# yjh0410/YOLO-Nano

Measured on NVIDIA B200. Metric: images/sec YOLO-Nano-1.0x 416 bs256 fp32-parity e2e (backbone+neck+head+decode+NMS), higher is better.
Workload: dtype f32 (tcgen05 3xTF32 split, fp32 accumulate)

## Files before the change

yolo_nano_b200/csrc/gemm_tc.cuh:

```cuda
#pragma once
#include <cuda.h>

#include <cstring>

#include "common.cuh"
#include "ptx_sm100.cuh"

namespace ynb {

constexpr int kTcThreads = 512;
constexpr int kTcSplitWarp0 = 8, kTcProducerWarp = 12, kTcMmaWarp = 13;
constexpr int kTcProducers = 3;
constexpr int kTcBM = 128;
constexpr int kTcBK = 32;
constexpr int kTcAStageBytes = kTcBM * 128;
constexpr int kTcMaxStages = 8;
constexpr int kTcSmemBudget = 232448;
constexpr int kTcMaxMain = 4;

struct TcGemmParams {
  int num_steps;
  int chunks_per_tap;
  int is3x3;
  int mode;
  int bf16_in;
  int out_bf16;
  int num_stages;
  int w_resident;
  int64_t M;
  int64_t num_tiles;
  int H, W, TH, TW, tiles_x, tiles_y;
  int N, Npad;
  int nmain;
  int nacc;
  int merge_corr;
  int ksub;
  int presplit;
  int a2_step;
  int stack_b;
  int acc_stages;
  uint32_t tmem_cols;
  uint32_t a_box_bytes;
  float* out;
  int out_ld, out_off, out_step;
  ChanMap omap;
  const float* bias;
  int act;
  const float* pass;
  int pass_ld;
  int tma_store;
  struct Decode {
    float* boxes;
    float* scores;
    int32_t* cls;
    int G, HW;
    float stride, input_size;
    float aw[3], ah[3];
    int64_t Ntot, level_off;
  } dec;
  int* err_flag;
  long long* trace;
  int trace_cap;
};

#define YNB_TRACE(role, a, b)                                                                        \
  do {                                                                                               \
    if (p.trace != nullptr && blockIdx.x == 0) {                                                     \
      const int _lt = (int)(((long long)(a) - (long long)blockIdx.x) / (long long)gridDim.x) & 63;   \
      long long* _e = p.trace + 1 + (long long)((((role) * 64 + _lt) * 32) + ((int)(b) & 31)) * 4;   \
      _e[0] = (role); _e[1] = (a); _e[2] = (b); _e[3] = clock64();                                   \
    }                                                                                                \
  } while (0)

struct TcSmemLayout {
  uint32_t stage_bytes;
  uint32_t w_chunk_bytes;
  uint32_t w_res_off;
  uint32_t bias_off;
  uint32_t stg_off;
  uint32_t bar_off;
  uint32_t total;
};
constexpr int kTcStgBytes = 8 * 4096;

__host__ __device__ inline TcSmemLayout tc_smem_layout(int Npad, int num_steps, int num_stages, bool w_resident,
                                                       bool split) {
  TcSmemLayout L;
  L.w_chunk_bytes = (uint32_t)Npad * 128;
  uint32_t a_bytes = kTcAStageBytes * (split ? 2 : 1);
  uint32_t w_bytes = w_resident ? 0 : L.w_chunk_bytes * (split ? 2 : 1);
  L.stage_bytes = a_bytes + w_bytes;
  L.w_res_off = L.stage_bytes * num_stages;
  uint32_t w_res = w_resident ? L.w_chunk_bytes * (split ? 2 : 1) * num_steps : 0;
  L.bias_off = L.w_res_off + w_res;
  L.stg_off = L.bias_off + 1024;
  L.bar_off = L.stg_off + kTcStgBytes;
  L.total = L.bar_off + 256 + 1024;
  return L;
}

__host__ __device__ __forceinline__ uint32_t rn_tf32_bits(uint32_t u) { return (u + 0x1000u) & 0xffffe000u; }

template <bool kPass, int kDecC>
__global__ void __launch_bounds__(kTcThreads, 1)
tc_gemm_kernel(const __grid_constant__ CUtensorMap tmA, const __grid_constant__ CUtensorMap tmAlo,
               const __grid_constant__ CUtensorMap tmWhi, const __grid_constant__ CUtensorMap tmWlo,
               const __grid_constant__ CUtensorMap tmOut, const TcGemmParams p) {
  extern __shared__ __align__(16) uint8_t smem_raw[];
  uint8_t* smem = smem_raw + ((1024u - (ptx::smem_u32(smem_raw) & 1023u)) & 1023u);

  const bool split = p.mode == YNB_GEMM_TC_3XTF32;
  const int kchunk = p.bf16_in ? 64 : kTcBK;
  const int box_alo = p.presplit ? 1 : -1;
  const int box_whi = p.w_resident ? -1 : 1 + (p.presplit ? 1 : 0);
  const int box_wlo = (p.w_resident || !split) ? -1 : box_whi + 1;
  const int nboxes = 1 + (box_alo >= 0) + (box_whi >= 0) + (box_wlo >= 0);
  const int nprod = nboxes < kTcProducers ? nboxes : kTcProducers;
  const TcSmemLayout lay = tc_smem_layout(p.Npad, p.num_steps, p.num_stages, p.w_resident != 0, split);
  const uint32_t w_chunk_bytes = lay.w_chunk_bytes;
  const uint32_t a_bytes = kTcAStageBytes * (split ? 2 : 1);
  const uint32_t stage_bytes = lay.stage_bytes;
  const uint32_t w_res_bytes = lay.bias_off - lay.w_res_off;
  float* s_bias = reinterpret_cast<float*>(smem + lay.bias_off);
  uint64_t* bars = reinterpret_cast<uint64_t*>(smem + lay.bar_off);
  uint64_t* full = bars;
  uint64_t* ready = bars + kTcMaxStages;
  uint64_t* empty = bars + 2 * kTcMaxStages;
  uint64_t* tmem_full = bars + 3 * kTcMaxStages;
  uint64_t* tmem_empty = bars + 3 * kTcMaxStages + 2;
  uint64_t* w_full = bars + 3 * kTcMaxStages + 4;
  uint32_t* tmem_ptr = reinterpret_cast<uint32_t*>(bars + 3 * kTcMaxStages + 5);

  const int warp = threadIdx.x >> 5, lane = threadIdx.x & 31;
  pdl_trigger();

  if (warp == kTcProducerWarp && lane == 0) {
    ptx::prefetch_tmap(&tmA);
    if (p.presplit || p.a2_step > 0) ptx::prefetch_tmap(&tmAlo);
    ptx::prefetch_tmap(&tmWhi);
    if (split) ptx::prefetch_tmap(&tmWlo);
    if (p.tma_store) ptx::prefetch_tmap(&tmOut);
    for (int s = 0; s < p.num_stages; ++s) {
      ptx::mbar_init(&full[s], nprod);
      ptx::mbar_init(&ready[s], 4);
      ptx::mbar_init(&empty[s], 1);
    }
    for (int a = 0; a < 2; ++a) {
      ptx::mbar_init(&tmem_full[a], 1);
      ptx::mbar_init(&tmem_empty[a], 4);
    }
    ptx::mbar_init(w_full, 1);
    ptx::fence_barrier_init();
  }
  if (warp == kTcMmaWarp) {
    ptx::tmem_alloc(tmem_ptr, p.tmem_cols);
    ptx::tmem_relinquish();
  }
  if (warp < 4) {
    for (int i = threadIdx.x; i < p.Npad; i += 128) s_bias[i] = i < p.N ? __ldg(p.bias + i) : 0.0f;
  }
  ptx::tc_fence_before_sync();
  __syncthreads();
  ptx::tc_fence_after_sync();
  const uint32_t tmem_base = *tmem_ptr;

  auto stage_a = [&](int s) { return smem + (size_t)s * stage_bytes; };
  auto stage_alo = [&](int s) { return smem + (size_t)s * stage_bytes + kTcAStageBytes; };
  auto w_hi_ptr = [&](int s, int step) {
    return p.w_resident ? smem + lay.w_res_off + (size_t)step * w_chunk_bytes * (split ? 2 : 1)
                        : smem + (size_t)s * stage_bytes + a_bytes;
  };
  auto w_lo_ptr = [&](int s, int step) { return w_hi_ptr(s, step) + w_chunk_bytes; };

  const int acc_cols = p.Npad * p.nacc;
  const uint32_t step_tx = p.a_box_bytes * (p.presplit ? 2 : 1) + (p.w_resident ? 0 : w_chunk_bytes * (split ? 2 : 1));
  const bool splitters_on = split && !p.presplit;

  if (warp == kTcProducerWarp && p.w_resident && ptx::elect_one()) {
    ptx::mbar_arrive_expect_tx(w_full, w_res_bytes);
    for (int st = 0; st < p.num_steps; ++st) {
      ptx::tma_load_2d(w_hi_ptr(0, st), &tmWhi, w_full, st * kchunk, 0);
      if (split) ptx::tma_load_2d(w_lo_ptr(0, st), &tmWlo, w_full, st * kchunk, 0);
    }
  }
  pdl_wait();

  const int prole = warp == kTcProducerWarp ? 0 : (warp == 14 ? 1 : (warp == 15 ? 2 : -1));
  if (prole >= 0) {
    if (prole < nprod && ptx::elect_one()) {
      const bool do_a = 0 % nprod == prole;
      const bool do_alo = box_alo >= 0 && box_alo % nprod == prole;
      const bool do_whi = box_whi >= 0 && box_whi % nprod == prole;
      const bool do_wlo = box_wlo >= 0 && box_wlo % nprod == prole;
      const uint32_t my_tx = (do_a ? p.a_box_bytes : 0u) + (do_alo ? p.a_box_bytes : 0u) +
                             (do_whi ? w_chunk_bytes : 0u) + (do_wlo ? w_chunk_bytes : 0u);
      int s = 0;
      uint32_t ph = 0;
      bool ok = true;
      for (int64_t tile = blockIdx.x; tile < p.num_tiles && ok; tile += gridDim.x) {
        int b = 0, y0 = 0, x0 = 0;
        if (p.is3x3) {
          int per_img = p.tiles_x * p.tiles_y;
          b = (int)(tile / per_img);
          int r = (int)(tile - (int64_t)b * per_img);
          y0 = (r / p.tiles_x) * p.TH;
          x0 = (r % p.tiles_x) * p.TW;
        }
        for (int st = 0; st < p.num_steps; ++st) {
          ok = ptx::mbar_wait(&empty[s], ph ^ 1, p.err_flag, 1);
          if (!ok) break;
          ptx::mbar_arrive_expect_tx(&full[s], my_tx);
          if (p.is3x3) {
            int tap = st / p.chunks_per_tap, kc = st - tap * p.chunks_per_tap;
            int dy = tap / 3, dx = tap - dy * 3;
            if (do_a) ptx::tma_load_4d(stage_a(s), &tmA, &full[s], kc * kchunk, x0 + dx - 1, y0 + dy - 1, b);
            if (do_alo) ptx::tma_load_4d(stage_alo(s), &tmAlo, &full[s], kc * kchunk, x0 + dx - 1, y0 + dy - 1, b);
          } else {
            if (do_a) {
              const bool second = p.a2_step > 0 && st >= p.a2_step;
              ptx::tma_load_2d(stage_a(s), second ? &tmAlo : &tmA, &full[s], (second ? st - p.a2_step : st) * kchunk,
                               (int)(tile * kTcBM));
            }
          }
          if (do_whi) ptx::tma_load_2d(w_hi_ptr(s, st), &tmWhi, &full[s], st * kchunk, 0);
          if (do_wlo) ptx::tma_load_2d(w_lo_ptr(s, st), &tmWlo, &full[s], st * kchunk, 0);
          if (prole == 0) YNB_TRACE(1, tile, st);
          if (++s == p.num_stages) { s = 0; ph ^= 1; }
        }
      }
    }
  } else if (warp == kTcMmaWarp) {
    if (ptx::elect_one()) {
      const uint32_t idesc = ptx::make_idesc(2 , kTcBM, p.Npad);
      const uint32_t idesc2 = ptx::make_idesc(2, kTcBM, 2 * p.Npad);
      const uint32_t idesc_bf = ptx::make_idesc(1 , kTcBM, p.Npad);
      int s = 0;
      uint32_t ph = 0;
      int acc = 0;
      uint32_t acc_ph = 0;
      bool ok = true;
      if (p.w_resident) ok = ptx::mbar_wait(w_full, 0, p.err_flag, 2);
      for (int64_t tile = blockIdx.x; tile < p.num_tiles && ok; tile += gridDim.x) {
        ok = ptx::mbar_wait(&tmem_empty[acc], acc_ph ^ 1, p.err_flag, 3);
        if (!ok) break;
        ptx::tc_fence_after_sync();
        const uint32_t d_tmem = tmem_base + (uint32_t)(acc * acc_cols);
        const uint32_t c_tmem = p.merge_corr ? d_tmem : d_tmem + (uint32_t)(p.nmain * p.Npad);
        int t = 0;
        for (int st = 0; st < p.num_steps; ++st) {
          ok = ptx::mbar_wait(splitters_on ? &ready[s] : &full[s], ph, p.err_flag, 4);
          if (!ok) break;
          ptx::tc_fence_after_sync();
          const uint32_t a_hi = ptx::smem_u32(stage_a(s));
          const uint32_t a_lo = ptx::smem_u32(stage_alo(s));
          const uint32_t b_hi = ptx::smem_u32(w_hi_ptr(s, st));
          const uint32_t b_lo = ptx::smem_u32(w_lo_ptr(s, st));
          const int nk = p.ksub > 0 ? min(kTcBK / 8, p.ksub - st * (kTcBK / 8)) : kTcBK / 8;
          if (p.bf16_in) {
#pragma unroll
            for (int k = 0; k < kTcBK / 8; ++k, ++t) {
              if (k >= nk) break;
              ptx::mma_bf16_ss(d_tmem, ptx::make_sw128_kmajor_desc(a_hi + k * 32), ptx::make_sw128_kmajor_desc(b_hi + k * 32),
                               idesc_bf, t != 0);
            }
          } else if (p.stack_b) {
#pragma unroll
            for (int k = 0; k < kTcBK / 8; ++k, ++t) {
              if (k >= nk) break;
              const uint64_t db = ptx::make_sw128_kmajor_desc(b_hi + k * 32);
              ptx::mma_tf32_ss(d_tmem, ptx::make_sw128_kmajor_desc(a_hi + k * 32), db, idesc2, t != 0);
              ptx::mma_tf32_ss(c_tmem, ptx::make_sw128_kmajor_desc(a_lo + k * 32), db, idesc, 1);
            }
          } else {
#pragma unroll
            for (int k = 0; k < kTcBK / 8; ++k, ++t) {
              if (k >= nk) break;
              const uint32_t ko = k * 32;
              const uint64_t da = ptx::make_sw128_kmajor_desc(a_hi + ko);
              const uint64_t db = ptx::make_sw128_kmajor_desc(b_hi + ko);
              const int slot = t % p.nmain;
              if (split) {
                ptx::mma_tf32_ss(c_tmem, ptx::make_sw128_kmajor_desc(a_lo + ko), db, idesc, t != 0);
                ptx::mma_tf32_ss(c_tmem, da, ptx::make_sw128_kmajor_desc(b_lo + ko), idesc, 1);
              }
              ptx::mma_tf32_ss(d_tmem + (uint32_t)(slot * p.Npad), da, db, idesc,
                               (split && p.merge_corr) ? 1 : (t >= p.nmain));
            }
          }
          YNB_TRACE(3, tile, st);
          ptx::mma_commit(&empty[s]);
          if (st == p.num_steps - 1) ptx::mma_commit(&tmem_full[acc]);
          if (++s == p.num_stages) { s = 0; ph ^= 1; }
        }
        if (++acc == p.acc_stages) { acc = 0; acc_ph ^= 1; }
      }
    }
  } else if (warp >= kTcSplitWarp0 && warp < kTcSplitWarp0 + 4) {
    if (splitters_on) {
      const int t = threadIdx.x - kTcSplitWarp0 * 32;
      int s = 0;
      uint32_t ph = 0;
      bool ok = true;
      for (int64_t tile = blockIdx.x; tile < p.num_tiles && ok; tile += gridDim.x) {
        for (int st = 0; st < p.num_steps; ++st) {
          ok = ptx::mbar_wait(&full[s], ph, p.err_flag, 5);
          if (!ok) break;
          uint4* a = reinterpret_cast<uint4*>(stage_a(s));
          uint4* lo = reinterpret_cast<uint4*>(stage_alo(s));
#pragma unroll
          for (int i = 0; i < kTcAStageBytes / 16 / 128; ++i) {
            const uint4 v = a[t + i * 128];
            uint4 h, l;
            h.x = rn_tf32_bits(v.x); h.y = rn_tf32_bits(v.y); h.z = rn_tf32_bits(v.z); h.w = rn_tf32_bits(v.w);
            l.x = rn_tf32_bits(__float_as_uint(__uint_as_float(v.x) - __uint_as_float(h.x)));
            l.y = rn_tf32_bits(__float_as_uint(__uint_as_float(v.y) - __uint_as_float(h.y)));
            l.z = rn_tf32_bits(__float_as_uint(__uint_as_float(v.z) - __uint_as_float(h.z)));
            l.w = rn_tf32_bits(__float_as_uint(__uint_as_float(v.w) - __uint_as_float(h.w)));
            a[t + i * 128] = h;
            lo[t + i * 128] = l;
          }
          ptx::fence_proxy_async_smem();
          __syncwarp();
          if (lane == 0) ptx::mbar_arrive(&ready[s]);
          if (t == 0) YNB_TRACE(2, tile, st);
          if (++s == p.num_stages) { s = 0; ph ^= 1; }
        }
      }
    }
  } else if (warp < 8) {
    const int group = warp >> 2;
    const int q = warp & 3;
    const int row = q * 32 + lane;
    const bool vec = p.out_step == 1 && p.omap.gap == 0;
    const float slope = p.act == YNB_ACT_RELU ? 0.0f : (p.act == YNB_ACT_LEAKY ? 0.1f : 1.0f);
    uint8_t* sbox = smem + lay.stg_off + warp * 4096;
    const int sw = lane & 7;
    const int nloc = (int64_t)blockIdx.x < p.num_tiles
                         ? (int)((p.num_tiles - blockIdx.x + gridDim.x - 1) / gridDim.x) : 0;
    const bool share_last = kDecC == 0;
    const int col_split = min(p.Npad, ((p.Npad / 2 + 31) / 32) * 32);
    bool ok = true;
    for (int lt = 0; lt < nloc && ok; ++lt) {
      const int64_t tile = blockIdx.x + (int64_t)lt * gridDim.x;
      const int acc = p.acc_stages == 2 ? (lt & 1) : 0;
      const bool shared = share_last && lt == nloc - 1 && col_split < p.Npad;
      if (!shared && group != acc) {
        if (p.acc_stages == 1 && share_last) ok = ptx::mbar_wait(&tmem_full[0], (uint32_t)(lt & 1), p.err_flag, 7);
        continue;
      }
      const int col_begin = shared && group == 1 ? col_split : 0;
      const int col_end = shared && group == 0 ? col_split : p.Npad;
      const uint32_t acc_ph = (uint32_t)((lt / p.acc_stages) & 1);
      int64_t m;
      bool valid;
      if (p.is3x3) {
        int per_img = p.tiles_x * p.tiles_y;
        int b = (int)(tile / per_img);
        int r = (int)(tile - (int64_t)b * per_img);
        int y = (r / p.tiles_x) * p.TH + row / p.TW;
        int x = (r % p.tiles_x) * p.TW + row % p.TW;
        valid = row < p.TH * p.TW && y < p.H && x < p.W;
        m = ((int64_t)b * p.H + y) * p.W + x;
      } else {
        m = tile * kTcBM + row;
        valid = m < p.M;
      }
      const int64_t m_base = tile * kTcBM + q * 32;
      float xa[16], xb[16];
      const int rows_left = (int)min((int64_t)32, p.M - m_base);
      auto fetch_x1 = [&](int c0, int r0, float (&x)[16]) {
        const int i = c0 + lane;
        const bool col_ok = kPass && i < p.N;
        const float* src = p.pass + (m_base + r0) * (int64_t)p.pass_ld + i;
        const int nr = col_ok ? rows_left - r0 : 0;
#pragma unroll
        for (int r = 0; r < 16; ++r) x[r] = r < nr ? __ldg(src + r * p.pass_ld) : 0.0f;
      };
      if (kPass) {
        fetch_x1(col_begin, 0, xa);
        fetch_x1(col_begin, 16, xb);
      }
      if (lane == 0 && q == 0) YNB_TRACE(4, tile, group);
      ok = ptx::mbar_wait(&tmem_full[acc], acc_ph, p.err_flag, 6);
      if (!ok) break;
      ptx::tc_fence_after_sync();
      if (lane == 0 && q == 0) YNB_TRACE(6, tile, group);
      const uint32_t t_base = tmem_base + ((uint32_t)(q * 32) << 16) + (uint32_t)(acc * acc_cols);
      if constexpr (kDecC > 0) {
        constexpr int A = 3, C = kDecC, CB = (C + 15) / 16;
        auto ld16 = [&](int c0, float (&v)[16]) {
          uint32_t r[16];
          ptx::tmem_ld_32x16(t_base + c0, r);
          if (p.nacc > 1) {
            for (int a2 = 1; a2 < p.nacc; ++a2) {
              uint32_t r2[16];
              ptx::tmem_ld_32x16(t_base + (uint32_t)(a2 * p.Npad) + c0, r2);
              ptx::tmem_ld_wait();
#pragma unroll
              for (int jj = 0; jj < 16; ++jj) r[jj] = __float_as_uint(__uint_as_float(r[jj]) + __uint_as_float(r2[jj]));
            }
          }
          ptx::tmem_ld_wait();
#pragma unroll
          for (int jj = 0; jj < 16; ++jj) v[jj] = __uint_as_float(r[jj]);
        };
        float objl[A], mx[A], sum[A], tb[4 * A];
        int am[A];
        {
          float v[16];
          ld16(0, v);
#pragma unroll
          for (int a = 0; a < A; ++a) objl[a] = v[a] + s_bias[a];
          constexpr int NPADC = (A * (1 + C + 4) + 15) / 16 * 16;
          constexpr int B0 = (A + A * C) < (NPADC - 16) ? (A + A * C) : (NPADC - 16);
          constexpr int BOFF = A + A * C - B0;
          ld16(B0, v);
#pragma unroll
          for (int k = 0; k < 4 * A; ++k) tb[k] = v[BOFF + k] + s_bias[A + A * C + k];
        }
#pragma unroll
        for (int a = 0; a < A; ++a) {
          const int cbase = A + a * C;
          float m = -INFINITY;
          int arg = 0;
#pragma unroll 1
          for (int blk = 0; blk < CB; ++blk) {
            float v[16];
            ld16(cbase + blk * 16, v);
            const float* bb = s_bias + cbase + blk * 16;
#pragma unroll
            for (int jj = 0; jj < 16; ++jj) {
              const int c = blk * 16 + jj;
              const float x = v[jj] + bb[jj];
              if ((C % 16 == 0 || c < C) && x > m) { m = x; arg = c; }
            }
          }
          float sm = 0.0f;
#pragma unroll 1
          for (int blk = 0; blk < CB; ++blk) {
            float v[16];
            ld16(cbase + blk * 16, v);
            const float* bb = s_bias + cbase + blk * 16;
#pragma unroll
            for (int jj = 0; jj < 16; ++jj) {
              const int c = blk * 16 + jj;
              if (C % 16 == 0 || c < C) sm += softmax_exp((v[jj] + bb[jj]) - m);
            }
          }
          mx[a] = m; am[a] = arg; sum[a] = sm;
        }
        (void)mx;
        {
          ptx::tc_fence_before_sync();
          __syncwarp();
          if (lane == 0) ptx::mbar_arrive(&tmem_empty[acc]);
        }
        if (valid) {
          const int b = (int)(m / p.dec.HW);
          const int pix = (int)(m - (int64_t)b * p.dec.HW);
          const int gy = pix / p.dec.G, gx = pix - gy * p.dec.G;
          const int64_t o0 = (int64_t)b * p.dec.Ntot + p.dec.level_off + (int64_t)pix * A;
#pragma unroll
          for (int a = 0; a < A; ++a) {
            const float obj = 1.0f / (1.0f + expf(-objl[a]));
            const float score = class_score(sum[a], obj);
            const float tx = tb[4 * a], ty = tb[4 * a + 1], tw = tb[4 * a + 2], th = tb[4 * a + 3];
            float cx = __fmul_rn(__fadd_rn(1.0f / (1.0f + expf(-tx)), (float)gx), p.dec.stride);
            float cy = __fmul_rn(__fadd_rn(1.0f / (1.0f + expf(-ty)), (float)gy), p.dec.stride);
            float w = __fmul_rn(expf(tw), p.dec.aw[a]);
            float h = __fmul_rn(expf(th), p.dec.ah[a]);
            float hw = __fmul_rn(w, 0.5f), hh = __fmul_rn(h, 0.5f);
            float x1 = __fdiv_rn(__fsub_rn(cx, hw), p.dec.input_size);
            float y1 = __fdiv_rn(__fsub_rn(cy, hh), p.dec.input_size);
            float x2 = __fdiv_rn(__fadd_rn(cx, hw), p.dec.input_size);
            float y2 = __fdiv_rn(__fadd_rn(cy, hh), p.dec.input_size);
            reinterpret_cast<float4*>(p.dec.boxes)[o0 + a] =
                make_float4(fminf(fmaxf(x1, 0.f), 1.f), fminf(fmaxf(y1, 0.f), 1.f), fminf(fmaxf(x2, 0.f), 1.f),
                            fminf(fmaxf(y2, 0.f), 1.f));
            p.dec.scores[o0 + a] = score;
            p.dec.cls[o0 + a] = am[a];
          }
        }
        if (lane == 0 && q == 0) YNB_TRACE(5, tile, group);
        continue;
      }
      auto box_free = [&]() {
        if (p.tma_store) {
          if (ptx::elect_one()) ptx::bulk_wait_read<0>();
          __syncwarp();
        }
      };
      auto drain16 = [&](int c0, int jc) {
        uint32_t r[16];
        ptx::tmem_ld_32x16(t_base + c0, r);
        if (p.nacc == 2) {
          uint32_t r2[16];
          ptx::tmem_ld_32x16(t_base + (uint32_t)p.Npad + c0, r2);
          ptx::tmem_ld_wait();
#pragma unroll
          for (int j = 0; j < 16; ++j) r[j] = __float_as_uint(__uint_as_float(r[j]) + __uint_as_float(r2[j]));
        } else if (p.nacc > 2) {
          for (int a = 1; a < p.nacc; ++a) {
            uint32_t r2[16];
            ptx::tmem_ld_32x16(t_base + (uint32_t)(a * p.Npad) + c0, r2);
            ptx::tmem_ld_wait();
#pragma unroll
            for (int j = 0; j < 16; ++j) r[j] = __float_as_uint(__uint_as_float(r[j]) + __uint_as_float(r2[j]));
          }
        } else {
          ptx::tmem_ld_wait();
        }
        if (jc == 0) box_free();
#pragma unroll
        for (int j = 0; j < 4; ++j) {
          const float4 b4 = *reinterpret_cast<const float4*>(s_bias + c0 + 4 * j);
          float x0 = __uint_as_float(r[4 * j]) + b4.x, x1 = __uint_as_float(r[4 * j + 1]) + b4.y;
          float x2 = __uint_as_float(r[4 * j + 2]) + b4.z, x3 = __uint_as_float(r[4 * j + 3]) + b4.w;
          *reinterpret_cast<float4*>(sbox + lane * 128 + (((jc + j) ^ sw) << 4)) =
              make_float4(fmaxf(x0, x0 * slope), fmaxf(x1, x1 * slope), fmaxf(x2, x2 * slope), fmaxf(x3, x3 * slope));
        }
      };
      auto staged = [&](int r, int l) {
        return *reinterpret_cast<const float*>(sbox + r * 128 + ((((l >> 2) ^ (r & 7)) << 4) | ((l & 3) << 2)));
      };

      auto drain16_bf16 = [&](int c0, int half) {
        uint32_t r[16];
        ptx::tmem_ld_32x16(t_base + c0, r);
        ptx::tmem_ld_wait();
        if (half == 0) box_free();
        uint32_t w[8];
#pragma unroll
        for (int j = 0; j < 8; ++j) {
          float x0 = __uint_as_float(r[2 * j]) + s_bias[c0 + 2 * j], x1 = __uint_as_float(r[2 * j + 1]) + s_bias[c0 + 2 * j + 1];
          w[j] = pack_bf16x2(fmaxf(x0, x0 * slope), fmaxf(x1, x1 * slope));
        }
        uint4* dst = reinterpret_cast<uint4*>(sbox + lane * 64 + half * 32);
        dst[0] = make_uint4(w[0], w[1], w[2], w[3]);
        dst[1] = make_uint4(w[4], w[5], w[6], w[7]);
      };
      const bool bf16_box = p.out_bf16 && p.tma_store && !kPass;
      bf16* const out_bf = reinterpret_cast<bf16*>(p.out);

      for (int c0 = col_begin; c0 < col_end; c0 += 32) {
        if (bf16_box) {
          drain16_bf16(c0, 0);
          if (c0 + 16 < col_end) drain16_bf16(c0 + 16, 1);
        } else {
          drain16(c0, 0);
          if (c0 + 16 < col_end) drain16(c0 + 16, 4);
        }
        if (c0 + 32 >= col_end && !shared) {
          ptx::tc_fence_before_sync();
          __syncwarp();
          if (lane == 0) ptx::mbar_arrive(&tmem_empty[acc]);
        }
        if (!kPass && p.tma_store) {
          ptx::fence_proxy_async_smem();
          __syncwarp();
          if (ptx::elect_one()) {
            ptx::tma_store_2d(&tmOut, sbox, c0, (int)m_base);
            ptx::bulk_commit();
          }
          continue;
        }
        __syncwarp();
        const int i = c0 + lane;
        const bool col_ok = i < p.N;
        if (kPass) {
          const int nrow = col_ok ? (int)min((int64_t)32, p.M - m_base) : 0;
          float* o = p.out + m_base * p.out_ld + p.omap.slot(2 * (col_ok ? i : 0));
#pragma unroll
          for (int r = 0; r < 16; ++r, o += p.out_ld)
            if (r < nrow) *reinterpret_cast<float2*>(o) = make_float2(xa[r], staged(r, lane));
          if (c0 + 32 < col_end) fetch_x1(c0 + 32, 0, xa);
#pragma unroll
          for (int r = 16; r < 32; ++r, o += p.out_ld)
            if (r < nrow) *reinterpret_cast<float2*>(o) = make_float2(xb[r - 16], staged(r, lane));
          if (c0 + 32 < col_end) fetch_x1(c0 + 32, 16, xb);
        } else {
          const int col = vec ? p.out_off + i : p.omap.slot(p.out_off + (col_ok ? i : 0) * p.out_step);
          if (!p.is3x3) {
            const int nrow = col_ok ? (int)min((int64_t)32, p.M - m_base) : 0;
            if (p.out_bf16) {
              bf16* o = out_bf + m_base * p.out_ld + col;
#pragma unroll 8
              for (int r = 0; r < 32; ++r, o += p.out_ld)
                if (r < nrow) *o = __float2bfloat16_rn(staged(r, lane));
            } else {
              float* o = p.out + m_base * p.out_ld + col;
#pragma unroll 8
              for (int r = 0; r < 32; ++r, o += p.out_ld)
                if (r < nrow) *o = staged(r, lane);
            }
          } else {
            const int64_t off = valid ? m * p.out_ld : -1;
#pragma unroll 8
            for (int r = 0; r < 32; ++r) {
              const int64_t offr = __shfl_sync(0xffffffffu, off, r);
              if (col_ok && offr >= 0) {
                if (p.out_bf16) out_bf[offr + col] = __float2bfloat16_rn(staged(r, lane));
                else p.out[offr + col] = staged(r, lane);
              }
            }
          }
        }
        __syncwarp();
      }
      if (lane == 0 && q == 0) YNB_TRACE(5, tile, group);
    }
    __syncwarp();
    if (p.tma_store && ptx::elect_one()) ptx::bulk_wait<0>();
  }

  ptx::tc_fence_before_sync();
  __syncthreads();
  if (warp == kTcMmaWarp) {
    ptx::tc_fence_after_sync();
    ptx::tmem_dealloc(tmem_base, p.tmem_cols);
  }
}

typedef CUresult (*PFN_encodeTiled)(CUtensorMap*, CUtensorMapDataType, cuuint32_t, void*, const cuuint64_t*,
                                    const cuuint64_t*, const cuuint32_t*, const cuuint32_t*,
                                    CUtensorMapInterleave, CUtensorMapSwizzle, CUtensorMapL2promotion,
                                    CUtensorMapFloatOOBfill);

inline PFN_encodeTiled get_encode_tiled() {
  static PFN_encodeTiled fn = nullptr;
  if (!fn) {
    void* p = nullptr;
    cudaDriverEntryPointQueryResult qres;
    if (cudaGetDriverEntryPoint("cuTensorMapEncodeTiled", &p, cudaEnableDefault, &qres) == cudaSuccess &&
        qres == cudaDriverEntryPointSuccess)
      fn = reinterpret_cast<PFN_encodeTiled>(p);
  }
  return fn;
}

inline bool make_tmap_2d(CUtensorMap* m, const void* base, uint64_t k, uint64_t rows, uint64_t row_stride_elems,
                         uint32_t box_rows, bool bf16 = false) {
  PFN_encodeTiled enc = get_encode_tiled();
  if (!enc) return false;
  const uint64_t es = bf16 ? 2 : 4;
  cuuint64_t dims[2] = {k, rows};
  cuuint64_t strides[1] = {row_stride_elems * es};
  cuuint32_t box[2] = {(cuuint32_t)(128 / es), box_rows};
  cuuint32_t estr[2] = {1, 1};
  return enc(m, bf16 ? CU_TENSOR_MAP_DATA_TYPE_BFLOAT16 : CU_TENSOR_MAP_DATA_TYPE_FLOAT32, 2, const_cast<void*>(base), dims,
             strides, box, estr, CU_TENSOR_MAP_INTERLEAVE_NONE, CU_TENSOR_MAP_SWIZZLE_128B,
             CU_TENSOR_MAP_L2_PROMOTION_L2_128B, CU_TENSOR_MAP_FLOAT_OOB_FILL_NONE) == CUDA_SUCCESS;
}

inline bool make_tmap_nhwc(CUtensorMap* m, const void* base, int C, int W, int H, int B, int ld, int box_w,
                           int box_h, bool bf16 = false, bool swizzle = true) {
  PFN_encodeTiled enc = get_encode_tiled();
  if (!enc) return false;
  const uint64_t es = bf16 ? 2 : 4;
  cuuint64_t dims[4] = {(cuuint64_t)C, (cuuint64_t)W, (cuuint64_t)H, (cuuint64_t)B};
  cuuint64_t strides[3] = {(cuuint64_t)ld * es, (cuuint64_t)ld * es * W, (cuuint64_t)ld * es * W * H};
  cuuint32_t box[4] = {(cuuint32_t)(128 / es), (cuuint32_t)box_w, (cuuint32_t)box_h, 1};
  cuuint32_t estr[4] = {1, 1, 1, 1};
  return enc(m, bf16 ? CU_TENSOR_MAP_DATA_TYPE_BFLOAT16 : CU_TENSOR_MAP_DATA_TYPE_FLOAT32, 4, const_cast<void*>(base), dims,
             strides, box, estr, CU_TENSOR_MAP_INTERLEAVE_NONE,
             swizzle ? CU_TENSOR_MAP_SWIZZLE_128B : CU_TENSOR_MAP_SWIZZLE_NONE,
             CU_TENSOR_MAP_L2_PROMOTION_L2_128B, CU_TENSOR_MAP_FLOAT_OOB_FILL_NONE) == CUDA_SUCCESS;
}

inline bool make_tmap_stem_input(CUtensorMap* m, const float* x, int S, int B) {
  PFN_encodeTiled enc = get_encode_tiled();
  if (!enc || (reinterpret_cast<uintptr_t>(x) & 15u) || (S & 3)) return false;
  cuuint64_t dims[4] = {(cuuint64_t)S, (cuuint64_t)S, 3, (cuuint64_t)B};
  cuuint64_t strides[3] = {(cuuint64_t)S * 4, (cuuint64_t)S * S * 4, (cuuint64_t)S * S * 12};
  cuuint32_t box[4] = {40, 35, 3, 1};
  cuuint32_t estr[4] = {1, 1, 1, 1};
  return enc(m, CU_TENSOR_MAP_DATA_TYPE_FLOAT32, 4, const_cast<float*>(x), dims, strides, box, estr,
             CU_TENSOR_MAP_INTERLEAVE_NONE, CU_TENSOR_MAP_SWIZZLE_NONE, CU_TENSOR_MAP_L2_PROMOTION_L2_128B,
             CU_TENSOR_MAP_FLOAT_OOB_FILL_NONE) == CUDA_SUCCESS;
}

inline bool make_tmap_out(CUtensorMap* m, void* base, uint64_t cols, uint64_t rows, uint64_t ld, bool bf16 = false) {
  PFN_encodeTiled enc = get_encode_tiled();
  if (!enc) return false;
  const uint64_t es = bf16 ? 2 : 4;
  cuuint64_t dims[2] = {cols, rows};
  cuuint64_t strides[1] = {ld * es};
  cuuint32_t box[2] = {32, 32};
  cuuint32_t estr[2] = {1, 1};
  return enc(m, bf16 ? CU_TENSOR_MAP_DATA_TYPE_BFLOAT16 : CU_TENSOR_MAP_DATA_TYPE_FLOAT32, 2, base, dims, strides, box,
             estr, CU_TENSOR_MAP_INTERLEAVE_NONE, bf16 ? CU_TENSOR_MAP_SWIZZLE_NONE : CU_TENSOR_MAP_SWIZZLE_128B,
             CU_TENSOR_MAP_L2_PROMOTION_NONE, CU_TENSOR_MAP_FLOAT_OOB_FILL_NONE) == CUDA_SUCCESS;
}

struct TcWeights {
  float* hi = nullptr;
  float* lo = nullptr;
  bf16* bw = nullptr;
  int N = 0, Npad = 0, Kpad = 0;
  CUtensorMap tm_hi, tm_lo;
};

inline void split_tf32_host(float v, float* hi, float* lo) {
  uint32_t u;
  memcpy(&u, &v, 4);
  uint32_t h = rn_tf32_bits(u);
  float hf;
  memcpy(&hf, &h, 4);
  float l = v - hf;
  uint32_t lu;
  memcpy(&lu, &l, 4);
  lu = rn_tf32_bits(lu);
  memcpy(lo, &lu, 4);
  *hi = hf;
}

struct TcGemmLaunch {
  CUtensorMap tmA;
  CUtensorMap tmOut;
  const TcWeights* w = nullptr;
  CUtensorMap tmAlo;
  TcGemmParams p;
  uint32_t smem = 0;
  unsigned grid = 0;
  int dec_classes = 0;
};

inline void tc_plan_tmem(TcGemmParams& p, bool allow_merge = false) {
  const bool split = p.mode == YNB_GEMM_TC_3XTF32;
  p.merge_corr = 0;
  static const bool merge_all = getenv("YNB_TC_MERGE_ALL") != nullptr;
  if (split && ((allow_merge && p.num_steps * (kTcBK / 8) <= 16) || merge_all) && 2 * p.Npad <= 512) {
    p.merge_corr = 1;
    p.stack_b = 0;
    p.nmain = 1; p.nacc = 1; p.acc_stages = 2;
    p.tmem_cols = 32;
    while ((int)p.tmem_cols < 2 * p.Npad) p.tmem_cols <<= 1;
    return;
  }
  const int corr = split ? 1 : 0;
  int want = 1;
  if (split) {
    const int ksteps = p.num_steps * (kTcBK / 8);
    want = ksteps >= 64 ? 4 : (ksteps >= 24 ? 3 : (ksteps >= 12 ? 2 : 1));
    static const int nmain_cap = getenv("YNB_TC_NMAIN_MAX") ? atoi(getenv("YNB_TC_NMAIN_MAX")) : 1;
    if (want > nmain_cap) want = nmain_cap;
  }
  p.nmain = want;
  while (p.nmain > 1 && (p.nmain + corr) * p.Npad > 512) p.nmain--;
  p.nacc = p.nmain + corr;
  p.acc_stages = 2 * p.nacc * p.Npad <= 512 ? 2 : 1;
  if (p.acc_stages == 1 && want <= 2 && p.nmain > 1 && 2 * (p.nmain - 1 + corr) * p.Npad <= 512) {
    p.nmain--;
    p.nacc--;
    p.acc_stages = 2;
  }
  p.tmem_cols = 32;
  while ((int)p.tmem_cols < p.acc_stages * p.nacc * p.Npad) p.tmem_cols <<= 1;
  static const bool no_stack = getenv("YNB_TC_NO_STACK") != nullptr;
  p.stack_b = (split && !no_stack && p.nmain == 1 && p.nacc == 2 && 2 * p.Npad <= 256 && (2 * p.Npad) % 16 == 0) ? 1 : 0;
}

inline bool tc_plan_smem(TcGemmLaunch& L) {
  TcGemmParams& p = L.p;
  const bool split = p.mode == YNB_GEMM_TC_3XTF32;
  for (int resident = 1; resident >= 0; --resident) {
    for (int stages = kTcMaxStages; stages >= 2; --stages) {
      if (stages > p.num_steps * 4 && stages > 2) continue;
      TcSmemLayout lay = tc_smem_layout(p.Npad, p.num_steps, stages, resident != 0, split);
      static const bool res2 = getenv("YNB_TC_RES2") != nullptr;
      if (lay.total <= (uint32_t)kTcSmemBudget && (resident == 0 || stages >= 3 || p.num_steps <= 2 || res2)) {
        p.num_stages = stages;
        p.w_resident = resident;
        L.smem = lay.total;
        return true;
      }
    }
  }
  return false;
}

inline cudaError_t launch_tc_gemm(const TcGemmLaunch& L, cudaStream_t st) {
  using KernelT = void (*)(CUtensorMap, CUtensorMap, CUtensorMap, CUtensorMap, CUtensorMap, TcGemmParams);
  static const KernelT kernels[4] = {tc_gemm_kernel<false, 0>, tc_gemm_kernel<true, 0>, tc_gemm_kernel<false, 80>,
                                     tc_gemm_kernel<false, 20>};
  static bool attr_set = false;
  if (!attr_set) {
    for (KernelT k : kernels) {
      cudaError_t e = cudaFuncSetAttribute(k, cudaFuncAttributeMaxDynamicSharedMemorySize, kTcSmemBudget);
      if (e != cudaSuccess) return e;
    }
    attr_set = true;
  }
  const CUtensorMap& tmo = L.p.tma_store ? L.tmOut : L.tmA;
  KernelT kern = L.dec_classes == 80 ? kernels[2] : (L.dec_classes == 20 ? kernels[3] : kernels[L.p.pass != nullptr ? 1 : 0]);
  const CUtensorMap& tmalo = (L.p.presplit || L.p.a2_step > 0) ? L.tmAlo : L.tmA;
  cudaError_t r = launch_pdl(kern, dim3(L.grid), dim3(kTcThreads), (size_t)L.smem, st, L.tmA, tmalo, L.w->tm_hi,
                             L.w->tm_lo, tmo, L.p);
  YNB_COUNT_LAUNCH();
  return r;
}

inline void tc_pick_tile(int H, int W, int* TH, int* TW) {
  double best = -1;
  for (int tw = 4; tw <= 64 && tw <= W + 3; ++tw) {
    int th = 128 / tw;
    if (th < 1) continue;
    if (th > H) th = H;
    double eff = (double)H * W / ((double)((W + tw - 1) / tw) * ((H + th - 1) / th) * 128.0);
    if (eff > best + 1e-9) { best = eff; *TH = th; *TW = tw; }
  }
}

}
```

yolo_nano_b200/csrc/unit_tc.cuh:

```cuda
#pragma once
#include "gemm_tc.cuh"

namespace ynb {

constexpr int kDpThreads = 640;
constexpr int kDpEpiWarps = 8;
constexpr int kDpDwWarp0 = 8, kDpDwWarps = 8;
constexpr int kDpRawWarp = 16, kDpMmaWarp = 17, kDpWWarp = 18;
constexpr int kDpMaxAStages = 4, kDpMaxRawStages = 4;
constexpr int kDpStgBytes = kDpEpiWarps * 4096;

struct DwPwParams {
  int H, W, lgTW, tiles_x, tiles_y;
  int64_t num_tiles;
  int C4;
  int num_chunks;
  int ksub;
  int N, Npad;
  int mode;
  int w_resident, a_stages, raw_stages;
  int prefetch_tiles;
  int pass_blocks;
  int tma_out;
  uint32_t tmem_cols;
  const float* dw_w;
  const float* dw_b;
  int dw_act;
  float* out;
  int out_ld, out_off;
  ChanMap omap;
  const float* bias;
  int act;
  const float* pass;
  int pass_ld;
  int* err_flag;
  long long* trace;
};

#define YNB_DP_TRACE(role, lt, kc)                                                              \
  do {                                                                                           \
    if (p.trace != nullptr && blockIdx.x == 0 && (lt) < 16)                                      \
      p.trace[((role) * 16 + (lt)) * 8 + ((kc) & 7)] = clock64();                               \
  } while (0)

struct DpSmemLayout {
  uint32_t raw_stride, a_off, a_stride, w_chunk_bytes, w_res_off, dww_off, bias_off, stg_off, bar_off, total;
};

__host__ __device__ inline DpSmemLayout dp_smem_layout(int Npad, int num_chunks, int lgTW, int a_stages, int raw_stages,
                                                       bool w_resident, bool split, int chunk_ch = 32) {
  DpSmemLayout L;
  const int TW = 1 << lgTW, TH = kTcBM >> lgTW;
  L.w_chunk_bytes = (uint32_t)Npad * 128;
  L.raw_stride = ((uint32_t)((TW + 2) * (TH + 2) * 128) + 1023u) & ~1023u;
  L.a_off = L.raw_stride * raw_stages;
  L.a_stride = kTcAStageBytes * (split ? 2 : 1) + (w_resident ? 0 : L.w_chunk_bytes * (split ? 2 : 1));
  L.w_res_off = L.a_off + L.a_stride * a_stages;
  const uint32_t w_res = w_resident ? L.w_chunk_bytes * (split ? 2 : 1) * num_chunks : 0;
  L.dww_off = L.w_res_off + w_res;
  L.bias_off = L.dww_off + (((uint32_t)(10 * num_chunks * chunk_ch * 4) + 1023u) & ~1023u);
  L.stg_off = L.bias_off + 1024;
  L.bar_off = L.stg_off + kDpStgBytes;
  L.total = L.bar_off + 256 + 1024;
  return L;
}

__device__ __forceinline__ float cvt_rna_tf32(float x) {
  uint32_t r;
  asm("cvt.rna.tf32.f32 %0, %1;" : "=r"(r) : "f"(x));
  return __uint_as_float(r);
}

template <bool kPass, typename E>
__global__ void __launch_bounds__(kDpThreads, 1)
dwpw_tc_kernel(const __grid_constant__ CUtensorMap tmIn, const __grid_constant__ CUtensorMap tmWhi,
               const __grid_constant__ CUtensorMap tmWlo, const __grid_constant__ CUtensorMap tmPass,
               const __grid_constant__ CUtensorMap tmOut, const DwPwParams p) {
  extern __shared__ __align__(16) uint8_t smem_raw[];
  uint8_t* smem = smem_raw + ((1024u - (ptx::smem_u32(smem_raw) & 1023u)) & 1023u);

  constexpr bool kBf16 = sizeof(E) == 2;
  constexpr int CH = 128 / (int)sizeof(E);
  constexpr int CGS = CH / 4;
  const bool split = !kBf16 && p.mode == YNB_GEMM_TC_3XTF32;
  const DpSmemLayout lay = dp_smem_layout(p.Npad, p.num_chunks, p.lgTW, p.a_stages, p.raw_stages, p.w_resident != 0, split, CH);
  const uint32_t w_chunk_bytes = lay.w_chunk_bytes;
  const int KC = p.num_chunks * CH;
  const int TW = 1 << p.lgTW, TH = kTcBM >> p.lgTW;
  float* s_dww = reinterpret_cast<float*>(smem + lay.dww_off);
  float* s_bias = reinterpret_cast<float*>(smem + lay.bias_off);
  uint64_t* bars = reinterpret_cast<uint64_t*>(smem + lay.bar_off);
  uint64_t* raw_full = bars;
  uint64_t* raw_empty = bars + 4;
  uint64_t* a_ready = bars + 8;
  uint64_t* a_empty = bars + 12;
  uint64_t* w_full = bars + 16;
  uint64_t* tmem_full = bars + 20;
  uint64_t* tmem_empty = bars + 22;
  uint32_t* tmem_ptr = reinterpret_cast<uint32_t*>(bars + 24);

  const int warp = threadIdx.x >> 5, lane = threadIdx.x & 31;
  pdl_trigger();

  if (warp == kDpRawWarp && lane == 0) {
    ptx::prefetch_tmap(&tmIn);
    ptx::prefetch_tmap(&tmWhi);
    if (split) ptx::prefetch_tmap(&tmWlo);
    if (p.pass_blocks) ptx::prefetch_tmap(&tmPass);
    if (p.tma_out) ptx::prefetch_tmap(&tmOut);
    for (int s = 0; s < kDpMaxRawStages; ++s) {
      ptx::mbar_init(&raw_full[s], 1);
      ptx::mbar_init(&raw_empty[s], kBf16 ? kDpDwWarps : kDpDwWarps / 2);
    }
    for (int s = 0; s < kDpMaxAStages; ++s) {
      ptx::mbar_init(&a_ready[s], kBf16 ? kDpDwWarps : kDpDwWarps / 2);
      ptx::mbar_init(&a_empty[s], 1);
      ptx::mbar_init(&w_full[s], 1);
    }
    for (int a = 0; a < 2; ++a) {
      ptx::mbar_init(&tmem_full[a], 1);
      ptx::mbar_init(&tmem_empty[a], 4);
    }
    ptx::fence_barrier_init();
  }
  if (warp == kDpMmaWarp) {
    ptx::tmem_alloc(tmem_ptr, p.tmem_cols);
    ptx::tmem_relinquish();
  }
  for (int i = threadIdx.x; i < 10 * KC; i += kDpThreads) {
    const int tap = i / KC, c = i - tap * KC;
    float v = 0.0f;
    if (c < p.C4) v = tap < 9 ? __ldg(p.dw_w + tap * p.C4 + c) : __ldg(p.dw_b + c);
    s_dww[i] = v;
  }
  for (int i = threadIdx.x; i < p.Npad; i += kDpThreads) s_bias[i] = i < p.N ? __ldg(p.bias + i) : 0.0f;
  ptx::tc_fence_before_sync();
  __syncthreads();
  ptx::tc_fence_after_sync();
  const uint32_t tmem_base = *tmem_ptr;

  const int nacc = split ? 2 : 1;
  const int acc_cols = p.Npad * nacc;
  const int per_img = p.tiles_x * p.tiles_y;
  auto a_stage = [&](int s) { return smem + lay.a_off + (size_t)s * lay.a_stride; };
  auto w_hi_ptr = [&](int s, int kc) {
    return p.w_resident ? smem + lay.w_res_off + (size_t)kc * w_chunk_bytes * (split ? 2 : 1)
                        : a_stage(s) + kTcAStageBytes * (split ? 2 : 1);
  };

  if (warp == kDpRawWarp && p.w_resident && ptx::elect_one()) {
    ptx::mbar_arrive_expect_tx(&w_full[0], w_chunk_bytes * (split ? 2 : 1) * p.num_chunks);
    for (int kc = 0; kc < p.num_chunks; ++kc) {
      ptx::tma_load_2d(w_hi_ptr(0, kc), &tmWhi, &w_full[0], kc * CH, 0);
      if (split) ptx::tma_load_2d(w_hi_ptr(0, kc) + w_chunk_bytes, &tmWlo, &w_full[0], kc * CH, 0);
    }
  }
  pdl_wait();

  if (warp == kDpRawWarp) {
    if (ptx::elect_one()) {
      const uint32_t raw_bytes = (uint32_t)((TW + 2) * (TH + 2) * 128);
      int r = 0;
      uint32_t ph = 0;
      bool ok = true;
      for (int64_t tile = blockIdx.x; tile < p.num_tiles && ok; tile += gridDim.x) {
        const int b = (int)(tile / per_img);
        const int rr = (int)(tile - (int64_t)b * per_img);
        const int y0 = (rr / p.tiles_x) * TH, x0 = (rr % p.tiles_x) * TW;
#pragma unroll 1
        for (int cb = 0; cb < p.pass_blocks; ++cb) ptx::tma_prefetch_4d(&tmPass, cb * CH, x0, y0, b);
        if (p.prefetch_tiles > 0) {
          const int64_t tp = tile + (int64_t)p.prefetch_tiles * gridDim.x;
          if (tp < p.num_tiles) {
            const int bp = (int)(tp / per_img);
            const int rp = (int)(tp - (int64_t)bp * per_img);
            const int yp = (rp / p.tiles_x) * TH, xp = (rp % p.tiles_x) * TW;
#pragma unroll 1
            for (int kc = 0; kc < p.num_chunks; ++kc) ptx::tma_prefetch_4d(&tmIn, kc * CH, xp - 1, yp - 1, bp);
          }
        }
        for (int kc = 0; kc < p.num_chunks; ++kc) {
          ok = ptx::mbar_wait(&raw_empty[r], ph ^ 1, p.err_flag, 1);
          if (!ok) break;
          ptx::mbar_arrive_expect_tx(&raw_full[r], raw_bytes);
          ptx::tma_load_4d(smem + (size_t)r * lay.raw_stride, &tmIn, &raw_full[r], kc * CH, x0 - 1, y0 - 1, b);
          YNB_DP_TRACE(0, (int)((tile - blockIdx.x) / gridDim.x), kc);
          if (++r == p.raw_stages) { r = 0; ph ^= 1; }
        }
      }
    }
  } else if (warp == kDpWWarp) {
    if (!p.w_resident && ptx::elect_one()) {
      int s = 0;
      uint32_t ph = 0;
      bool ok = true;
      for (int64_t tile = blockIdx.x; tile < p.num_tiles && ok; tile += gridDim.x) {
        for (int kc = 0; kc < p.num_chunks; ++kc) {
          ok = ptx::mbar_wait(&a_empty[s], ph ^ 1, p.err_flag, 2);
          if (!ok) break;
          ptx::mbar_arrive_expect_tx(&w_full[s], w_chunk_bytes * (split ? 2 : 1));
          ptx::tma_load_2d(w_hi_ptr(s, kc), &tmWhi, &w_full[s], kc * CH, 0);
          if (split) ptx::tma_load_2d(w_hi_ptr(s, kc) + w_chunk_bytes, &tmWlo, &w_full[s], kc * CH, 0);
          if (++s == p.a_stages) { s = 0; ph ^= 1; }
        }
      }
    }
  } else if (warp == kDpMmaWarp) {
    if (ptx::elect_one()) {
      const uint32_t idesc = ptx::make_idesc(kBf16 ? 1 : 2 , kTcBM, p.Npad);
      const uint32_t idesc2 = ptx::make_idesc(2, kTcBM, 2 * p.Npad);
      const bool stack_b = split && 2 * p.Npad <= 256;
      int s = 0, acc = 0;
      uint32_t ph = 0, acc_ph = 0;
      bool ok = true;
      if (p.w_resident) ok = ptx::mbar_wait(&w_full[0], 0, p.err_flag, 3);
      for (int64_t tile = blockIdx.x; tile < p.num_tiles && ok; tile += gridDim.x) {
        ok = ptx::mbar_wait(&tmem_empty[acc], acc_ph ^ 1, p.err_flag, 4);
        if (!ok) break;
        ptx::tc_fence_after_sync();
        const uint32_t d_tmem = tmem_base + (uint32_t)(acc * acc_cols);
        const uint32_t c_tmem = d_tmem + (uint32_t)p.Npad;
        for (int kc = 0; kc < p.num_chunks; ++kc) {
          ok = ptx::mbar_wait(&a_ready[s], ph, p.err_flag, 5);
          if (ok && !p.w_resident) ok = ptx::mbar_wait(&w_full[s], ph, p.err_flag, 6);
          if (!ok) break;
          ptx::tc_fence_after_sync();
          const uint32_t a_hi = ptx::smem_u32(a_stage(s));
          const uint32_t a_lo = a_hi + kTcAStageBytes;
          const uint32_t b_hi = ptx::smem_u32(w_hi_ptr(s, kc));
          const uint32_t b_lo = b_hi + w_chunk_bytes;
          const int nk = min(kTcBK / 8, p.ksub - kc * (kTcBK / 8));
#pragma unroll
          for (int k = 0; k < kTcBK / 8; ++k) {
            if (k >= nk) break;
            const uint32_t ko = k * 32;
            const uint32_t accum = (kc | k) != 0;
            const uint64_t da = ptx::make_sw128_kmajor_desc(a_hi + ko);
            const uint64_t db = ptx::make_sw128_kmajor_desc(b_hi + ko);
            if (kBf16) {
              ptx::mma_bf16_ss(d_tmem, da, db, idesc, accum);
            } else if (stack_b) {
              ptx::mma_tf32_ss(d_tmem, da, db, idesc2, accum);
              ptx::mma_tf32_ss(c_tmem, ptx::make_sw128_kmajor_desc(a_lo + ko), db, idesc, 1);
            } else if (split) {
              ptx::mma_tf32_ss(c_tmem, ptx::make_sw128_kmajor_desc(a_lo + ko), db, idesc, accum);
              ptx::mma_tf32_ss(c_tmem, da, ptx::make_sw128_kmajor_desc(b_lo + ko), idesc, 1);
              ptx::mma_tf32_ss(d_tmem, da, db, idesc, accum);
            } else {
              ptx::mma_tf32_ss(d_tmem, da, db, idesc, accum);
            }
          }
          YNB_DP_TRACE(3, (int)((tile - blockIdx.x) / gridDim.x), kc);
          ptx::mma_commit(&a_empty[s]);
          if (kc == p.num_chunks - 1) ptx::mma_commit(&tmem_full[acc]);
          if (++s == p.a_stages) { s = 0; ph ^= 1; }
        }
        if (++acc == 2) { acc = 0; acc_ph ^= 1; }
      }
    }
  } else if (warp >= kDpDwWarp0 && warp < kDpDwWarp0 + kDpDwWarps) {
    constexpr int NGROUPS = kBf16 ? 1 : 2;
    constexpr int GTHREADS = 256 / NGROUPS;
    const int t = (threadIdx.x - kDpDwWarp0 * 32) % GTHREADS;
    const int grp = (threadIdx.x - kDpDwWarp0 * 32) / GTHREADS;
    const int cg = t & (CGS - 1);
    const int IW = TW + 2;
    const bool has_act = p.dw_act != YNB_ACT_NONE;
    const float slope = p.dw_act == YNB_ACT_RELU ? 0.0f : 0.1f;
    const int nloc = (int64_t)blockIdx.x < p.num_tiles
                         ? (int)((p.num_tiles - blockIdx.x + gridDim.x - 1) / gridDim.x) : 0;
    const int total_chunks = nloc * p.num_chunks;
    bool ok = true;
    {
      for (int gc = grp; gc < total_chunks && ok; gc += NGROUPS) {
        const int lt_ = gc / p.num_chunks, kc = gc - lt_ * p.num_chunks;
        const int r = gc % p.raw_stages, s = gc % p.a_stages;
        const uint32_t rph = (uint32_t)((gc / p.raw_stages) & 1), sph = (uint32_t)((gc / p.a_stages) & 1);
        const float* wv = s_dww + kc * CH + cg * 4;
        const float4 bv = *reinterpret_cast<const float4*>(wv + 9 * KC);
        ok = ptx::mbar_wait(&raw_full[r], rph, p.err_flag, 7);
        if (ok) ok = ptx::mbar_wait(&a_empty[s], sph ^ 1, p.err_flag, 8);
        if (!ok) break;
        if (t == 0) YNB_DP_TRACE(1, lt_, kc);
        const uint8_t* raw = smem + (size_t)r * lay.raw_stride;
        uint8_t* a_hi = a_stage(s);
        uint8_t* a_lo = a_hi + kTcAStageBytes;
        constexpr int ROWS = 2;
        const int bidx = t / CGS;
        const int nsx = TW >> 2;
        const int sx = bidx % nsx, sy = (bidx / nsx) * ROWS;
        float4 acc[ROWS][4];
#pragma unroll
        for (int o = 0; o < ROWS; ++o)
#pragma unroll
          for (int q = 0; q < 4; ++q) acc[o][q] = bv;
#pragma unroll
        for (int ir = 0; ir < ROWS + 2; ++ir) {
          const int r0 = (sy + ir) * IW + sx * 4;
          float4 v[6];
#pragma unroll
          for (int j = 0; j < 6; ++j) {
            const int rr = r0 + j;
            if (!kBf16) v[j] = load4(reinterpret_cast<const E*>(raw + rr * 128 + (cg << 4)));
            else v[j] = load4(reinterpret_cast<const E*>(raw + rr * 128 + (cg << 3)));
          }
#pragma unroll
          for (int o = 0; o < ROWS; ++o) {
            const int ky = ir - o;
            if (ky < 0 || ky > 2) continue;
#pragma unroll
            for (int kx = 0; kx < 3; ++kx) {
              const float4 k = *reinterpret_cast<const float4*>(wv + (ky * 3 + kx) * KC);
#pragma unroll
              for (int q = 0; q < 4; ++q) {
                const float4 u = v[q + kx];
                const float2 lo = __ffma2_rn(make_float2(u.x, u.y), make_float2(k.x, k.y), make_float2(acc[o][q].x, acc[o][q].y));
                const float2 hi = __ffma2_rn(make_float2(u.z, u.w), make_float2(k.z, k.w), make_float2(acc[o][q].z, acc[o][q].w));
                acc[o][q] = make_float4(lo.x, lo.y, hi.x, hi.y);
              }
            }
          }
        }
        __syncwarp();
        if (lane == 0) ptx::mbar_arrive(&raw_empty[r]);
#pragma unroll
        for (int o = 0; o < ROWS; ++o) {
          const int row0 = (sy + o) * TW + sx * 4;
#pragma unroll
          for (int q = 0; q < 4; ++q) {
            const int row = row0 + q;
            float4 a = acc[o][q];
            if (has_act) {
              a.x = fmaxf(a.x, a.x * slope); a.y = fmaxf(a.y, a.y * slope);
              a.z = fmaxf(a.z, a.z * slope); a.w = fmaxf(a.w, a.w * slope);
            }
            if (kBf16) {
              const uint32_t o2 = (uint32_t)row * 128 + ((uint32_t)((cg >> 1) ^ (row & 7)) << 4) + ((uint32_t)(cg & 1) << 3);
              *reinterpret_cast<uint2*>(a_hi + o2) = make_uint2(pack_bf16x2(a.x, a.y), pack_bf16x2(a.z, a.w));
            } else {
              const uint32_t o2 = (uint32_t)row * 128 + ((uint32_t)(cg ^ (row & 7)) << 4);
              if (split) {
                float4 h, l;
                h.x = cvt_rna_tf32(a.x); h.y = cvt_rna_tf32(a.y); h.z = cvt_rna_tf32(a.z); h.w = cvt_rna_tf32(a.w);
                l.x = cvt_rna_tf32(a.x - h.x); l.y = cvt_rna_tf32(a.y - h.y);
                l.z = cvt_rna_tf32(a.z - h.z); l.w = cvt_rna_tf32(a.w - h.w);
                *reinterpret_cast<float4*>(a_hi + o2) = h;
                *reinterpret_cast<float4*>(a_lo + o2) = l;
              } else {
                *reinterpret_cast<float4*>(a_hi + o2) = a;
              }
            }
          }
        }
        ptx::fence_proxy_async_smem();
        __syncwarp();
        if (lane == 0) ptx::mbar_arrive(&a_ready[s]);
        if (t == 0) YNB_DP_TRACE(2, lt_, kc);
      }
    }
  } else if (warp < kDpEpiWarps) {
    const int group = warp >> 2, q = warp & 3;
    const int row = q * 32 + lane;
    const float slope = p.act == YNB_ACT_RELU ? 0.0f : (p.act == YNB_ACT_LEAKY ? 0.1f : 1.0f);
    uint8_t* sbox = smem + lay.stg_off + warp * 4096;
    const int sw = lane & 7;
    const int yy = row >> p.lgTW, xx = row & (TW - 1);
    const bool gap = p.omap.gap != 0;
    constexpr int BOX = 128 / (int)sizeof(E);
    constexpr int CPB = kPass ? BOX / 2 : BOX;
    constexpr int EPC = 16 / (int)sizeof(E);
    const int nbox = (p.Npad + CPB - 1) / CPB;
    const int out_cols = kPass ? 2 * p.N : ((p.N + EPC - 1) / EPC) * EPC;
    E* const outp = reinterpret_cast<E*>(p.out);
    const E* const passp = reinterpret_cast<const E*>(p.pass);
    const int acc = group;
    bool ok = true;
    int lt = group;
    for (int64_t tile = blockIdx.x + (int64_t)group * gridDim.x; tile < p.num_tiles && ok; tile += 2 * (int64_t)gridDim.x, lt += 2) {
      const uint32_t acc_ph = (uint32_t)((lt >> 1) & 1);
      const int b = (int)(tile / per_img);
      const int rr = (int)(tile - (int64_t)b * per_img);
      const int y = (rr / p.tiles_x) * TH + yy, x = (rr % p.tiles_x) * TW + xx;
      const bool valid = y < p.H && x < p.W;
      const int pix = (b * p.H + y) * p.W + x;
      const int ooff = valid ? pix * p.out_ld : -1;
      const E* prow = passp + (valid ? (size_t)pix * p.pass_ld : 0);
      uint4 x1v[4];
      auto fetch_x1 = [&](int c0) {
#pragma unroll
        for (int j = 0; j < 4; ++j)
          x1v[j] = (kPass && valid && c0 + EPC * j < p.N) ? __ldg(reinterpret_cast<const uint4*>(prow + c0) + j)
                                                         : make_uint4(0u, 0u, 0u, 0u);
      };
      if (kPass) fetch_x1(0);
      ok = ptx::mbar_wait(&tmem_full[acc], acc_ph, p.err_flag, 9);
      if (!ok) break;
      ptx::tc_fence_after_sync();
      if (q == 0 && lane == 0) YNB_DP_TRACE(4, lt, 0);
      const uint32_t t_base = tmem_base + ((uint32_t)(q * 32) << 16) + (uint32_t)(acc * acc_cols);
      auto drain16 = [&](int c0, float (&v)[16]) {
        uint32_t r1[16];
        ptx::tmem_ld_32x16(t_base + c0, r1);
        if (nacc == 2) {
          uint32_t r2[16];
          ptx::tmem_ld_32x16(t_base + (uint32_t)p.Npad + c0, r2);
          ptx::tmem_ld_wait();
#pragma unroll
          for (int j = 0; j < 16; ++j) v[j] = __uint_as_float(r1[j]) + __uint_as_float(r2[j]);
        } else {
          ptx::tmem_ld_wait();
#pragma unroll
          for (int j = 0; j < 16; ++j) v[j] = __uint_as_float(r1[j]);
        }
#pragma unroll
        for (int j = 0; j < 4; ++j) {
          const float4 b4 = *reinterpret_cast<const float4*>(s_bias + c0 + 4 * j);
          v[4 * j] += b4.x; v[4 * j + 1] += b4.y; v[4 * j + 2] += b4.z; v[4 * j + 3] += b4.w;
        }
        if (p.act == YNB_ACT_RELU) {
#pragma unroll
          for (int j = 0; j < 16; ++j) v[j] = fmaxf(v[j], 0.0f);
        } else {
#pragma unroll
          for (int j = 0; j < 16; ++j) v[j] = fmaxf(v[j], v[j] * slope);
        }
      };
      auto put_chunk = [&](int j, uint4 val) {
        *reinterpret_cast<uint4*>(sbox + lane * 128 + ((j ^ sw) << 4)) = val;
      };
      const bool tma_out = p.tma_out != 0;
      for (int bx = 0; bx < nbox; ++bx) {
        const int c0 = bx * CPB;
        auto box_free = [&]() {
          if (tma_out) {
            if (ptx::elect_one()) ptx::bulk_wait_read<0>();
            __syncwarp();
          }
        };
        if (!kBf16 && kPass) {
          float v[16];
          drain16(c0, v);
          box_free();
          const uint32_t xw[16] = {x1v[0].x, x1v[0].y, x1v[0].z, x1v[0].w, x1v[1].x, x1v[1].y, x1v[1].z, x1v[1].w,
                                   x1v[2].x, x1v[2].y, x1v[2].z, x1v[2].w, x1v[3].x, x1v[3].y, x1v[3].z, x1v[3].w};
#pragma unroll
          for (int j = 0; j < 8; ++j)
            put_chunk(j, make_uint4(xw[2 * j], __float_as_uint(v[2 * j]), xw[2 * j + 1], __float_as_uint(v[2 * j + 1])));
        } else if (!kBf16) {
          float v[16];
          drain16(c0, v);
          box_free();
#pragma unroll
          for (int j = 0; j < 4; ++j)
            put_chunk(j, make_uint4(__float_as_uint(v[4 * j]), __float_as_uint(v[4 * j + 1]), __float_as_uint(v[4 * j + 2]),
                                    __float_as_uint(v[4 * j + 3])));
          if (c0 + 16 < p.Npad) {
            drain16(c0 + 16, v);
#pragma unroll
            for (int j = 0; j < 4; ++j)
              put_chunk(4 + j, make_uint4(__float_as_uint(v[4 * j]), __float_as_uint(v[4 * j + 1]),
                                          __float_as_uint(v[4 * j + 2]), __float_as_uint(v[4 * j + 3])));
          }
        } else if (kPass) {
          box_free();
          const uint32_t xw[16] = {x1v[0].x, x1v[0].y, x1v[0].z, x1v[0].w, x1v[1].x, x1v[1].y, x1v[1].z, x1v[1].w,
                                   x1v[2].x, x1v[2].y, x1v[2].z, x1v[2].w, x1v[3].x, x1v[3].y, x1v[3].z, x1v[3].w};
#pragma unroll
          for (int h = 0; h < 2; ++h) {
            if (h == 0 || c0 + 16 < p.Npad) {
              float v[16];
              drain16(c0 + 16 * h, v);
              uint32_t w[16];
#pragma unroll
              for (int i = 0; i < 16; ++i) {
                const uint32_t xs = xw[8 * h + (i >> 1)];
                const uint32_t x1bits = (i & 1) ? (xs >> 16) : (xs & 0xffffu);
                w[i] = x1bits | (pack_bf16x2(0.0f, v[i]) & 0xffff0000u);
              }
#pragma unroll
              for (int j = 0; j < 4; ++j) put_chunk(4 * h + j, make_uint4(w[4 * j], w[4 * j + 1], w[4 * j + 2], w[4 * j + 3]));
            }
          }
        } else {
          box_free();
#pragma unroll
          for (int h = 0; h < 4; ++h) {
            if (h == 0 || c0 + 16 * h < p.Npad) {
              float v[16];
              drain16(c0 + 16 * h, v);
              put_chunk(2 * h, make_uint4(pack_bf16x2(v[0], v[1]), pack_bf16x2(v[2], v[3]), pack_bf16x2(v[4], v[5]),
                                          pack_bf16x2(v[6], v[7])));
              put_chunk(2 * h + 1, make_uint4(pack_bf16x2(v[8], v[9]), pack_bf16x2(v[10], v[11]), pack_bf16x2(v[12], v[13]),
                                              pack_bf16x2(v[14], v[15])));
            }
          }
        }
        if (kPass && bx + 1 < nbox) fetch_x1((bx + 1) * CPB);
        if (bx == nbox - 1) {
          ptx::tc_fence_before_sync();
          __syncwarp();
          if (lane == 0) ptx::mbar_arrive(&tmem_empty[acc]);
        }
        __syncwarp();
        const int j0 = bx * BOX;
        if (tma_out) {
          ptx::fence_proxy_async_smem();
          __syncwarp();
          if (ptx::elect_one()) {
            ptx::tma_store_4d(&tmOut, sbox, j0, (rr % p.tiles_x) * TW, (rr / p.tiles_x) * TH + q * (32 >> p.lgTW), b);
            ptx::bulk_commit();
          }
          continue;
        }
        if (!gap) {
          const int ch = lane & 7;
          const int jc = j0 + EPC * ch;
#pragma unroll
          for (int k = 0; k < 8; ++k) {
            const int r = (lane >> 3) + 4 * k;
            const int oo = __shfl_sync(0xffffffffu, ooff, r);
            const uint4 val = *reinterpret_cast<const uint4*>(sbox + r * 128 + ((ch ^ (r & 7)) << 4));
            if (oo >= 0 && jc < out_cols) *reinterpret_cast<uint4*>(outp + oo + p.out_off + jc) = val;
          }
        } else if (!kBf16) {
          const int pr = lane & 15;
          const int jc = j0 + 2 * pr;
          const int col = p.omap.slot(p.out_off + jc);
#pragma unroll
          for (int k = 0; k < 16; ++k) {
            const int r = (lane >> 4) + 2 * k;
            const int oo = __shfl_sync(0xffffffffu, ooff, r);
            const uint2 val =
                *reinterpret_cast<const uint2*>(sbox + r * 128 + ((((pr >> 1) ^ (r & 7)) << 4) | ((pr & 1) << 3)));
            if (oo >= 0 && jc < out_cols) *reinterpret_cast<uint2*>(outp + oo + col) = val;
          }
        } else {
          const int jc = j0 + 2 * lane;
          const int col = p.omap.slot(p.out_off + jc);
#pragma unroll 8
          for (int r = 0; r < 32; ++r) {
            const int oo = __shfl_sync(0xffffffffu, ooff, r);
            const uint32_t val =
                *reinterpret_cast<const uint32_t*>(sbox + r * 128 + ((((lane >> 2) ^ (r & 7)) << 4) | ((lane & 3) << 2)));
            if (oo >= 0 && jc < out_cols) *reinterpret_cast<uint32_t*>(outp + oo + col) = val;
          }
        }
        __syncwarp();
      }
      if (q == 0 && lane == 0) YNB_DP_TRACE(5, lt, 0);
    }
    if (p.tma_out && ptx::elect_one()) ptx::bulk_wait<0>();
  }

  ptx::tc_fence_before_sync();
  __syncthreads();
  if (warp == kDpMmaWarp) {
    ptx::tc_fence_after_sync();
    ptx::tmem_dealloc(tmem_base, p.tmem_cols);
  }
}

struct DwPwLaunch {
  CUtensorMap tmIn;
  CUtensorMap tmOut;
  CUtensorMap tmPass;
  const TcWeights* w = nullptr;
  DwPwParams p;
  uint32_t smem = 0;
  unsigned grid = 0;
};

inline bool plan_dwpw(DwPwLaunch& L, const void* in, int in_ld, int B, int H, int W, int C, int C4, const TcWeights* w,
                      int mode) {
  DwPwParams& p = L.p;
  const bool split = mode == YNB_GEMM_TC_3XTF32;
  const bool is_bf16 = mode == YNB_GEMM_TC_BF16;
  const int es = is_bf16 ? 2 : 4, chunk_ch = 128 / es;
  if (2 * (split ? 2 : 1) * w->Npad > 512 || (reinterpret_cast<uintptr_t>(in) & 15u) || ((in_ld * es) & 15)) return false;
  if ((int64_t)B * H * W * std::max(p.out_ld, std::max(p.pass_ld, 1)) >= (1LL << 31)) return false;
  p.H = H; p.W = W;
  {
    const int t16 = ((W + 15) / 16) * ((H + 7) / 8), t32 = ((W + 31) / 32) * ((H + 3) / 4);
    p.lgTW = t32 < t16 ? 5 : 4;
    static const int force = getenv("YNB_DP_LGTW") ? atoi(getenv("YNB_DP_LGTW")) : 0;
    if (force == 4 || force == 5) p.lgTW = force;
  }
  const int TW = 1 << p.lgTW, TH = kTcBM >> p.lgTW;
  p.tiles_x = (W + TW - 1) / TW;
  p.tiles_y = (H + TH - 1) / TH;
  p.num_tiles = (int64_t)B * p.tiles_x * p.tiles_y;
  p.C4 = C4;
  p.num_chunks = w->Kpad / chunk_ch;
  p.ksub = (C * es + 31) / 32;
  p.N = w->N; p.Npad = w->Npad;
  p.mode = mode;
  p.tmem_cols = 32;
  while ((int)p.tmem_cols < 2 * (split ? 2 : 1) * p.Npad) p.tmem_cols <<= 1;
  bool found = false;
  static const int wres = getenv("YNB_DP_WRES") ? atoi(getenv("YNB_DP_WRES")) : -1;
  for (int raw = kDpMaxRawStages; raw >= 2 && !found; --raw)
    for (int resident = 1; resident >= 0 && !found; --resident) {
      if (wres >= 0 && resident != wres) continue;
      DpSmemLayout lay = dp_smem_layout(p.Npad, p.num_chunks, p.lgTW, 2, raw, resident != 0, split, chunk_ch);
      if (lay.total <= (uint32_t)kTcSmemBudget) {
        p.a_stages = 2; p.raw_stages = raw; p.w_resident = resident; L.smem = lay.total;
        found = true;
      }
    }
  if (!found) return false;
  {
    static const int pf = getenv("YNB_DP_PREFETCH") ? atoi(getenv("YNB_DP_PREFETCH")) : 0;
    p.prefetch_tiles = pf;
  }
  const int epc = 16 / es;
  if ((reinterpret_cast<uintptr_t>(p.out) & 15u) || (p.out_ld % epc) || (p.out_off % epc)) return false;
  p.pass_blocks = 0;
  if (p.pass) {
    if ((reinterpret_cast<uintptr_t>(p.pass) & 15u) || (p.pass_ld % epc)) return false;
    if (make_tmap_nhwc(&L.tmPass, p.pass, (p.N + epc - 1) / epc * epc, W, H, B, p.pass_ld, TW, TH, is_bf16))
      p.pass_blocks = (p.N + chunk_ch - 1) / chunk_ch;
  }
  if (!make_tmap_nhwc(&L.tmIn, in, C4, W, H, B, in_ld, TW + 2, TH + 2, is_bf16, false)) return false;
  p.tma_out = 0;
  {
    static const bool no_ts = getenv("YNB_DP_NO_TMA_STORE") != nullptr;
    const int out_cols = p.pass ? 2 * p.N : (p.N + epc - 1) / epc * epc;
    if (!no_ts && p.omap.gap == 0 && p.out_off == 0 &&
        make_tmap_nhwc(&L.tmOut, p.out, out_cols, W, H, B, p.out_ld, TW, 32 / TW, is_bf16))
      p.tma_out = 1;
  }
  L.w = w;
  L.grid = (unsigned)std::min<int64_t>(p.num_tiles, kNumSMs);
  return true;
}

inline cudaError_t launch_dwpw_tc(const DwPwLaunch& L, cudaStream_t st) {
  using KernelT = void (*)(CUtensorMap, CUtensorMap, CUtensorMap, CUtensorMap, CUtensorMap, DwPwParams);
  static const KernelT kernels[4] = {dwpw_tc_kernel<false, float>, dwpw_tc_kernel<true, float>,
                                     dwpw_tc_kernel<false, bf16>, dwpw_tc_kernel<true, bf16>};
  static bool attr_set = false;
  if (!attr_set) {
    for (KernelT k : kernels) {
      cudaError_t e = cudaFuncSetAttribute(k, cudaFuncAttributeMaxDynamicSharedMemorySize, kTcSmemBudget);
      if (e != cudaSuccess) return e;
    }
    attr_set = true;
  }
  const int ki = (L.p.mode == YNB_GEMM_TC_BF16 ? 2 : 0) + (L.p.pass != nullptr ? 1 : 0);
  cudaError_t r = launch_pdl(kernels[ki], dim3(L.grid), dim3(kDpThreads), (size_t)L.smem, st,
                             L.tmIn, L.w->tm_hi, L.w->tm_lo, L.p.pass_blocks ? L.tmPass : L.tmIn,
                             L.p.tma_out ? L.tmOut : L.tmIn, L.p);
  YNB_COUNT_LAUNCH();
  return r;
}

}
```

yolo_nano_b200/csrc/ynb_api.cu:

```cuda
#include <cuda.h>
#include <cuda_runtime.h>

#include <cmath>
#include <cstdio>
#include <cstdlib>
#include <cstring>
#include <deque>
#include <functional>
#include <map>
#include <memory>
#include <string>
#include <tuple>
#include <vector>

#include "yolonano_b200.h"

#include "common.cuh"
#include "decode_nms.cuh"
#include "nms_grid.cuh"
#include "gemm_ffma.cuh"
#include "gemm_tc.cuh"
#include "unit_tc.cuh"
#include "kernels_basic.cuh"
#include "train_ops.cuh"
#include "wgrad_tc.cuh"
#include "topology.h"

#define YNB_EXPORT extern "C" __attribute__((visibility("default")))

namespace ynb {

thread_local LaunchCounter* g_counter = nullptr;
static thread_local std::string g_create_error;

struct Tensor {
  float* p = nullptr;
  int es = 4;
  int C = 0;
  int ld = 0;
  int H = 0, W = 0;
  ChanMap map = {INT_MAX, 0};
  size_t floats_per_image() const { return (size_t)H * W * ld; }
  void* at(int off = 0) const { return reinterpret_cast<char*>(p) + (size_t)off * es; }
};

struct InLayout {
  int ktot;
  ChanMap map;
};

struct PackedConv {
  bool loaded = false;
  std::vector<float> w_host, b_host;
  float* w_dev = nullptr;
  float* b_dev = nullptr;
  int n = 0, ktot = 0;
  TcWeights tc;
};

struct Op {
  std::string name, kind;
  double bytes = 0, flops = 0;
  std::function<cudaError_t(cudaStream_t)> fn;
  bool mark = false;
  bool side = false;
  bool join = false;
};

struct ProfEntry {
  std::string name, kind;
  double bytes, flops;
  float ms;
};

struct Plan {
  int batch = 0;
  std::vector<Op> net;
  std::vector<Op> raw_tail;
  std::vector<Op> decode;
  std::vector<Op> fused_tail;
  bool fused = false;
};

}

using namespace ynb;

struct ynb_engine {
  ynb_config cfg;
  int S = 0;
  std::string err;
  std::vector<ConvSpec> table;
  std::map<std::string, int> index;
  std::vector<PackedConv> convs;
  struct CatConv { PackedConv pc; int n0 = 0, k1p = 0, k2p = 0; };
  std::vector<CatConv> cat[3];
  StemWeights stem_w;
  PreLut prelut;
  PreLut* d_prelut = nullptr;
  struct StemMap { CUtensorMap tm; int ok; };
  std::map<std::tuple<const float*, int, int>, StemMap> stem_maps;
  bool committed = false;

  char* ws = nullptr;
  size_t ws_bytes = 0;
  int ws_batch = 0, ws_S = 0;
  std::map<std::string, Tensor> taps;
  Tensor raw[3];
  float* d_boxes = nullptr;
  float* d_scores = nullptr;
  int32_t* d_cls = nullptr;
  void* d_nms_ws = nullptr;
  int64_t nms_ws_bytes = 0;
  float* d_x = nullptr;
  struct HostSlot {
    float* x = nullptr; float* boxes = nullptr; float* scores = nullptr; int32_t* cls = nullptr;
    int32_t* counts = nullptr;
    uint8_t* img_u8 = nullptr;
    int32_t* rects = nullptr;
    cudaEvent_t h2d = nullptr, done = nullptr;
    bool busy = false;
    int batch = 0;
    float* ob = nullptr; float* os = nullptr; int32_t* oc = nullptr; int32_t* on = nullptr;
    int* flag_host = nullptr;
  } slot[2];
  cudaStream_t s_copy = nullptr;
  cudaStream_t s_copy2 = nullptr;
  cudaEvent_t ev_copy2 = nullptr;
  cudaStream_t s_d2h = nullptr;
  const float* d_x_bound = nullptr;
  float* d_out_boxes = nullptr;
  float* d_out_scores = nullptr;
  int32_t* d_out_cls = nullptr;
  int32_t* d_out_counts = nullptr;
  int* d_err = nullptr;

  std::map<int, std::unique_ptr<Plan>> plans;
  std::deque<std::deque<TcGemmLaunch>> tc_store;
  std::deque<std::deque<DwPwLaunch>> dp_store;
  std::deque<CUtensorMap> dw_maps;

  cudaStream_t s_main = nullptr, s_side = nullptr;
  std::vector<cudaEvent_t> events;
  size_t ev_next = 0;
  cudaEvent_t ev_in = nullptr, ev_out = nullptr;
  struct GraphKey {
    int batch; const void* x; const void* ob; const void* os; const void* oc; const void* on;
    float conf, thr; int diou, mode, S;
    bool operator<(const GraphKey& o) const {
      return std::tie(batch, x, ob, os, oc, on, conf, thr, diou, mode, S) <
             std::tie(o.batch, o.x, o.ob, o.os, o.oc, o.on, o.conf, o.thr, o.diou, o.mode, o.S);
    }
  };
  std::map<GraphKey, cudaGraphExec_t> graphs;
  std::map<GraphKey, int> graph_seen;
  bool use_graphs = true;
  std::map<int, int64_t> graph_launches;
  LaunchCounter counter;
  bool profiling = false;
  std::vector<ProfEntry> prof;

  int64_t N() const {
    int64_t n = 0;
    for (int s : {8, 16, 32}) n += (int64_t)cfg.num_anchors * (S / s) * (S / s);
    return n;
  }
};

namespace ynb {
inline bool is_bf16(const ynb_engine* e) { return e->cfg.gemm_mode == YNB_GEMM_TC_BF16; }
}

namespace {

int fail(ynb_engine* e, int code, const std::string& msg) {
  if (e) e->err = msg; else g_create_error = msg;
  return code;
}
#define CUDA_TRY(e, call)                                                                 \
  do {                                                                                    \
    cudaError_t _st = (call);                                                             \
    if (_st != cudaSuccess)                                                               \
      return fail(e, YNB_ERR_CUDA, std::string(#call) + ": " + cudaGetErrorString(_st));  \
  } while (0)

struct CounterScope {
  explicit CounterScope(ynb_engine* e) { g_counter = &e->counter; }
  ~CounterScope() { g_counter = nullptr; }
};

struct StageLayout { int ld; ChanMap map; };
static bool dense_stage2() {
  static const bool off = getenv("YNB_GAP_STAGE2") != nullptr;
  return !off;
}
StageLayout stage_layout(bool bf, int si) {
  const int cout = stage_channels()[si + 1], h = cout / 2, a = bf ? 8 : 4;
  const int hp = round_up(h, a);
  if (hp == h) return {cout, dense_map()};
  if (dense_stage2()) return {round_up(cout, a), dense_map()};
  return {2 * hp, ChanMap{h, hp - h}};
}
struct X2Window { int off, shift; };
X2Window x2_window(const StageLayout& sl, int h, int a) {
  if (sl.map.gap != 0) return {sl.map.slot(h), 0};
  return {h - h % a, h % a};
}

InLayout in_layout(const ConvSpec& c, bool bf) {
  const std::string& n = c.name;
  if (c.kind == kDense3x3) return {c.cin == 3 ? 27 : 9 * c.cin, dense_map()};
  bool reads_c3 = n == "backbone.stage3.0.branch1.0" || n == "backbone.stage3.0.branch1.2" ||
                  n == "backbone.stage3.0.branch2.0" || n == "conv1x1_0.convs.0";
  bool reads_c4 = n == "backbone.stage4.0.branch1.0" || n == "backbone.stage4.0.branch1.2" ||
                  n == "backbone.stage4.0.branch2.0" || n == "conv1x1_1.convs.0";
  if (reads_c3) { StageLayout L = stage_layout(bf, 0); return {L.ld, L.map}; }
  if (reads_c4) { StageLayout L = stage_layout(bf, 1); return {L.ld, L.map}; }
  for (int si = 0; si < 3; ++si) {
    const std::string pre = "backbone.stage" + std::to_string(si + 2) + ".";
    if (n.compare(0, pre.size(), pre) == 0 && n.size() > pre.size() + 2 && n[pre.size()] != '0' &&
        n.compare(n.size() - 10, 10, ".branch2.0") == 0) {
      const int a = bf ? 8 : 4;
      const X2Window w = x2_window(stage_layout(bf, si), c.cin, a);
      if (w.shift) return {round_up(c.cin + w.shift, a), ChanMap{0, w.shift}};
    }
  }
  return {round_up(c.cin, bf ? 8 : 4), dense_map()};
}

int pack_tc_matrix(ynb_engine* e, TcWeights& t, const float* w, int n, int ktot, int taps, const std::string& name) {
  const bool bf = is_bf16(e);
  t.N = n;
  t.Npad = round_up(n, 16);
  if (t.hi) cudaFree(t.hi);
  if (t.lo) cudaFree(t.lo);
  if (t.bw) cudaFree(t.bw);
  t.hi = t.lo = nullptr; t.bw = nullptr;
  if (bf) {
    const int kin = ktot / taps, kin_pad = round_up(kin, 64);
    t.Kpad = taps * kin_pad;
    std::vector<bf16> bw((size_t)t.Npad * t.Kpad, __float2bfloat16(0.0f));
    for (int r = 0; r < n; ++r)
      for (int tp = 0; tp < taps; ++tp)
        for (int k = 0; k < kin; ++k)
          bw[(size_t)r * t.Kpad + (size_t)tp * kin_pad + k] = __float2bfloat16_rn(w[(size_t)r * ktot + (size_t)tp * kin + k]);
    CUDA_TRY(e, cudaMalloc(&t.bw, bw.size() * 2));
    CUDA_TRY(e, cudaMemcpy(t.bw, bw.data(), bw.size() * 2, cudaMemcpyHostToDevice));
    if (!make_tmap_2d(&t.tm_hi, t.bw, t.Kpad, t.Npad, t.Kpad, t.Npad, true))
      return fail(e, YNB_ERR_CUDA, "cuTensorMapEncodeTiled failed for weights of " + name);
    t.tm_lo = t.tm_hi;
    return YNB_OK;
  }
  t.Kpad = round_up(ktot, kTcBK);
  std::vector<float> hi((size_t)t.Npad * t.Kpad, 0.f), lo((size_t)t.Npad * t.Kpad, 0.f);
  for (int r = 0; r < n; ++r)
    for (int k = 0; k < ktot; ++k)
      split_tf32_host(w[(size_t)r * ktot + k], &hi[(size_t)r * t.Kpad + k], &lo[(size_t)r * t.Kpad + k]);
  CUDA_TRY(e, cudaMalloc(&t.hi, hi.size() * 4));
  CUDA_TRY(e, cudaMalloc(&t.lo, lo.size() * 4));
  CUDA_TRY(e, cudaMemcpy(t.hi, hi.data(), hi.size() * 4, cudaMemcpyHostToDevice));
  CUDA_TRY(e, cudaMemcpy(t.lo, lo.data(), lo.size() * 4, cudaMemcpyHostToDevice));
  if (!make_tmap_2d(&t.tm_hi, t.hi, t.Kpad, t.Npad, t.Kpad, t.Npad) ||
      !make_tmap_2d(&t.tm_lo, t.lo, t.Kpad, t.Npad, t.Kpad, t.Npad))
    return fail(e, YNB_ERR_CUDA, "cuTensorMapEncodeTiled failed for weights of " + name);
  return YNB_OK;
}

int pack_cat(ynb_engine* e, int si) {
  const bool bf = is_bf16(e);
  const std::string bk = "backbone.stage" + std::to_string(si + 2) + ".0.";
  const int i1 = e->index.at(bk + "branch1.2"), i2 = e->index.at(bk + "branch2.5");
  const ConvSpec& c1 = e->table[i1];
  const ConvSpec& c2 = e->table[i2];
  const PackedConv& p1 = e->convs[i1];
  const PackedConv& p2 = e->convs[i2];
  const InLayout il1 = in_layout(c1, bf), il2 = in_layout(c2, bf);
  const StageLayout sl = stage_layout(bf, si);
  const int ch = bf ? 64 : kTcBK;
  const int k1p = round_up(il1.ktot, ch), k2p = round_up(il2.ktot, ch), ktot = k1p + k2p;
  const int h = c1.cout;
  std::vector<float> w((size_t)sl.ld * ktot, 0.f), b((size_t)sl.ld, 0.f);
  for (int i = 0; i < h; ++i) {
    const int r1 = sl.map.slot(2 * i), r2 = sl.map.slot(2 * i + 1);
    for (int k = 0; k < c1.cin; ++k) w[(size_t)r1 * ktot + il1.map.slot(k)] = p1.w_host[(size_t)i * c1.cin + k];
    for (int k = 0; k < c2.cin; ++k) w[(size_t)r2 * ktot + k1p + il2.map.slot(k)] = p2.w_host[(size_t)i * c2.cin + k];
    b[r1] = p1.b_host[i];
    b[r2] = p2.b_host[i];
  }
  const int parts = (sl.ld + 239) / 240;
  const int npart = round_up((sl.ld + parts - 1) / parts, bf ? 8 : 4);
  for (auto& cc : e->cat[si]) {
    if (cc.pc.b_dev) cudaFree(cc.pc.b_dev);
    if (cc.pc.tc.hi) cudaFree(cc.pc.tc.hi);
    if (cc.pc.tc.lo) cudaFree(cc.pc.tc.lo);
    if (cc.pc.tc.bw) cudaFree(cc.pc.tc.bw);
  }
  e->cat[si].clear();
  e->cat[si].resize(parts);
  for (int pi = 0; pi < parts; ++pi) {
    ynb_engine::CatConv& cc = e->cat[si][pi];
    cc.n0 = pi * npart;
    const int n = std::min(npart, sl.ld - cc.n0);
    cc.k1p = k1p; cc.k2p = k2p;
    cc.pc.n = n; cc.pc.ktot = ktot; cc.pc.loaded = true;
    CUDA_TRY(e, cudaMalloc(&cc.pc.b_dev, round_up(n, 4) * 4));
    CUDA_TRY(e, cudaMemset(cc.pc.b_dev, 0, round_up(n, 4) * 4));
    CUDA_TRY(e, cudaMemcpy(cc.pc.b_dev, b.data() + cc.n0, n * 4, cudaMemcpyHostToDevice));
    int rc = pack_tc_matrix(e, cc.pc.tc, w.data() + (size_t)cc.n0 * ktot, n, ktot, 1, bk + "cat");
    if (rc) return rc;
  }
  return YNB_OK;
}

int pack_conv(ynb_engine* e, int i) {
  const ConvSpec& c = e->table[i];
  PackedConv& pc = e->convs[i];
  const bool bf = is_bf16(e);
  InLayout il = in_layout(c, bf);
  std::vector<float> w, b;
  if (c.kind == kDense3x3 && c.cin == 3) {
    w.assign(27 * 24, 0.f);
    for (int co = 0; co < 24; ++co)
      for (int ci = 0; ci < 3; ++ci)
        for (int t = 0; t < 9; ++t) w[(ci * 9 + t) * 24 + co] = pc.w_host[(co * 3 + ci) * 9 + t];
    b = pc.b_host;
    pc.n = 24; pc.ktot = 27;
    memcpy(e->stem_w.w, w.data(), sizeof(e->stem_w.w));
    memcpy(e->stem_w.b, b.data(), sizeof(e->stem_w.b));
  } else if (c.kind == kDw3x3) {
    int c4 = il.ktot;
    w.assign(9 * c4, 0.f);
    b.assign(c4, 0.f);
    for (int ch = 0; ch < c.cin; ++ch) {
      int s = il.map.slot(ch);
      for (int t = 0; t < 9; ++t) w[t * c4 + s] = pc.w_host[ch * 9 + t];
      b[s] = pc.b_host[ch];
    }
    pc.n = c4; pc.ktot = 9;
  } else if (c.kind == kPw1x1) {
    w.assign((size_t)c.cout * il.ktot, 0.f);
    for (int n = 0; n < c.cout; ++n)
      for (int k = 0; k < c.cin; ++k) w[(size_t)n * il.ktot + il.map.slot(k)] = pc.w_host[(size_t)n * c.cin + k];
    b = pc.b_host;
    pc.n = c.cout; pc.ktot = il.ktot;
  } else {
    w.assign((size_t)c.cout * 9 * c.cin, 0.f);
    for (int n = 0; n < c.cout; ++n)
      for (int ci = 0; ci < c.cin; ++ci)
        for (int t = 0; t < 9; ++t)
          w[((size_t)n * 9 + t) * c.cin + ci] = pc.w_host[((size_t)n * c.cin + ci) * 9 + t];
    b = pc.b_host;
    pc.n = c.cout; pc.ktot = 9 * c.cin;
  }
  if (pc.w_dev) cudaFree(pc.w_dev);
  if (pc.b_dev) cudaFree(pc.b_dev);
  pc.w_dev = pc.b_dev = nullptr;
  CUDA_TRY(e, cudaMalloc(&pc.w_dev, w.size() * 4));
  CUDA_TRY(e, cudaMalloc(&pc.b_dev, round_up((int)b.size(), 4) * 4));
  CUDA_TRY(e, cudaMemcpy(pc.w_dev, w.data(), w.size() * 4, cudaMemcpyHostToDevice));
  CUDA_TRY(e, cudaMemset(pc.b_dev, 0, round_up((int)b.size(), 4) * 4));
  CUDA_TRY(e, cudaMemcpy(pc.b_dev, b.data(), b.size() * 4, cudaMemcpyHostToDevice));

  if ((c.kind == kPw1x1) || (c.kind == kDense3x3 && c.cin != 3)) {
    int rc = pack_tc_matrix(e, pc.tc, w.data(), pc.n, pc.ktot, c.kind == kDense3x3 ? 9 : 1, c.name);
    if (rc) return rc;
  }
  return YNB_OK;
}

struct Bump {
  size_t off = 0;
  size_t take(size_t bytes) {
    size_t o = off;
    off += (bytes + 1023) & ~(size_t)1023;
    return o;
  }
};

size_t layout_workspace(ynb_engine* e, int batch, int S, char* base) {
  Bump bump;
  const bool bf = is_bf16(e);
  const int es_act = bf ? 2 : 4, al = bf ? 8 : 4;
  auto tensor = [&](const std::string& name, int C, int ld, int H, ChanMap map = dense_map(), int es = 0) {
    Tensor t;
    t.es = es ? es : es_act;
    t.C = C; t.ld = ld; t.H = H; t.W = H; t.map = map;
    size_t o = bump.take((size_t)batch * H * H * ld * t.es);
    t.p = base ? reinterpret_cast<float*>(base + o) : nullptr;
    e->taps[name] = t;
    return t;
  };
  e->taps.clear();
  const int H1 = S / 4;
  tensor("pool", 24, 24, H1);
  int hin = H1;
  int ld_in = 24;
  ChanMap map_in = dense_map();
  for (int si = 0; si < 3; ++si) {
    int cout = stage_channels()[si + 1], h = cout / 2, cin = stage_channels()[si];
    int hout = hin / 2;
    std::string st = "stage" + std::to_string(si + 2);
    const StageLayout sl = stage_layout(bf, si);
    int ld_h = round_up(h, al);
    tensor(st + ".b1dw", cin, ld_in, hout, map_in);
    tensor(st + ".b2pw", h, ld_h, hin);
    tensor(st + ".mid1", h, ld_h, hout);
    tensor(st + ".mid2", h, ld_h, hout);
    for (int bi = 0; bi < stage_repeats()[si]; ++bi) tensor(st + "." + std::to_string(bi), cout, sl.ld, hout, sl.map);
    hin = hout;
    ld_in = sl.ld;
    map_in = sl.map;
  }
  const int H3 = S / 8, H4 = S / 16, H5 = S / 32;
  const int hs[3] = {H3, H4, H5};
  for (int l = 0; l < 3; ++l) tensor("lat" + std::to_string(l + 3), 96, 96, hs[l]);
  tensor("sum4", 96, 96, H4); tensor("sum4.lo", 96, 96, H4); tensor("fpn4", 96, 96, H4);
  tensor("sum3", 96, 96, H3); tensor("sum3.lo", 96, 96, H3); tensor("p3", 96, 96, H3);
  tensor("sum4b", 96, 96, H4); tensor("sum4b.lo", 96, 96, H4); tensor("p4", 96, 96, H4);
  tensor("sum5", 96, 96, H5); tensor("sum5.lo", 96, 96, H5); tensor("p5", 96, 96, H5);
  const int ch = e->cfg.num_anchors * (1 + e->cfg.num_classes + 4);
  const char* pn[3] = {"pred_s", "pred_m", "pred_l"};
  for (int l = 0; l < 3; ++l) {
    tensor("head" + std::to_string(l) + ".a", 96, 96, hs[l]);
    tensor("head" + std::to_string(l) + ".b", 96, 96, hs[l]);
    tensor("head" + std::to_string(l) + ".c", 96, 96, hs[l]);
    e->raw[l] = tensor(pn[l], ch, round_up(ch, 4), hs[l], dense_map(), 4);
  }
  e->taps["c3"] = e->taps["stage2.3"];
  e->taps["c4"] = e->taps["stage3.7"];
  e->taps["c5"] = e->taps["stage4.3"];

  int64_t n = 0;
  for (int s : {8, 16, 32}) n += (int64_t)e->cfg.num_anchors * (S / s) * (S / s);
  auto raw = [&](size_t bytes) { size_t o = bump.take(bytes); return base ? base + o : nullptr; };
  e->d_boxes = (float*)raw((size_t)batch * n * 16);
  e->d_scores = (float*)raw((size_t)batch * n * 4);
  e->d_cls = (int32_t*)raw((size_t)batch * n * 4);
  e->nms_ws_bytes = std::max(nms_workspace_bytes(batch, n), grid_nms_workspace_bytes(batch, n));
  e->d_nms_ws = raw((size_t)e->nms_ws_bytes);
  for (int k = 0; k < 2; ++k) {
    e->slot[k].x = (float*)raw((size_t)batch * 3 * S * S * 4);
    e->slot[k].boxes = (float*)raw((size_t)batch * n * 16);
    e->slot[k].scores = (float*)raw((size_t)batch * n * 4);
    e->slot[k].cls = (int32_t*)raw((size_t)batch * n * 4);
    e->slot[k].counts = (int32_t*)raw((size_t)batch * 4);
    e->slot[k].img_u8 = (uint8_t*)raw((size_t)batch * 3 * S * S);
    e->slot[k].rects = (int32_t*)raw((size_t)batch * 16);
  }
  e->d_x = e->slot[0].x;
  e->d_out_boxes = e->slot[0].boxes;
  e->d_out_scores = e->slot[0].scores;
  e->d_out_cls = e->slot[0].cls;
  e->d_out_counts = e->slot[0].counts;
  e->d_err = (int*)raw(256);
  return bump.off;
}

int ensure_workspace(ynb_engine* e, int batch) {
  if (e->ws && e->ws_batch >= batch && e->ws_S == e->S) return YNB_OK;
  int nb = std::max(batch, std::max(e->ws_batch, (int)e->cfg.max_batch));
  CUDA_TRY(e, cudaDeviceSynchronize());
  e->plans.clear();
  e->tc_store.clear(); e->dp_store.clear(); e->dw_maps.clear(); e->stem_maps.clear();
  for (auto& kv : e->graphs) cudaGraphExecDestroy(kv.second);
  e->graphs.clear();
  e->graph_seen.clear();
  if (e->ws) { cudaFree(e->ws); e->ws = nullptr; }
  size_t bytes = layout_workspace(e, nb, e->S, nullptr);
  CUDA_TRY(e, cudaMalloc(&e->ws, bytes));
  CUDA_TRY(e, cudaMemset(e->ws, 0, bytes));
  layout_workspace(e, nb, e->S, e->ws);
  e->ws_bytes = bytes;
  e->ws_batch = nb;
  e->ws_S = e->S;
  return YNB_OK;
}

struct Planner {
  ynb_engine* e;
  int B;
  Plan* plan;
  std::deque<TcGemmLaunch>* tc;
  std::deque<DwPwLaunch>* dp;
  std::string error;
  std::vector<Op>* dst = nullptr;
  std::vector<Op>& ops() { return dst ? *dst : plan->net; }

  const PackedConv& conv(const std::string& name) const { return e->convs[e->index.at(name)]; }
  const ConvSpec& spec(const std::string& name) const { return e->table[e->index.at(name)]; }
  Tensor T(const std::string& name) const { return e->taps.at(name); }

  void dw(const std::string& name, const Tensor& in, int in_off, const Tensor& out) {
    const PackedConv& pc = conv(name);
    const ConvSpec& c = spec(name);
    int B_ = B, c4 = pc.n, stride = c.stride, act = c.act;
    const float *w = pc.w_dev, *b = pc.b_dev;
    double px_in = (double)B * in.H * in.W, px_out = (double)B * out.H * out.W;
    const bool bf = is_bf16(e);
    const double bytes = (double)in.es * c.cin * (px_in + px_out) + 40.0 * c.cin, flops = 18.0 * c.cin * px_out;
    static const bool no_tma = getenv("YNB_DW_NO_TMA") != nullptr;
    e->dw_maps.emplace_back();
    CUtensorMap* tm = &e->dw_maps.back();
    if ((!no_tma || bf) && make_tmap_dw(tm, in.p, in.ld, in_off, B, in.H, in.W, c4, stride, bf)) {
      plan->net.push_back({name, "dwconv3x3", bytes, flops, [=](cudaStream_t st) {
        return launch_dwconv3x3_tma(*tm, out.p, out.ld, 0, w, b, B_, in.H, in.W, c4, stride, act, st, false, bf);
      }});
      return;
    }
    if (bf) { error = "bf16 depthwise conv needs a 16-byte aligned view: " + name; return; }
    plan->net.push_back({name, "dwconv3x3", bytes, flops, [=](cudaStream_t st) {
      return launch_dwconv3x3(in.p, in.ld, in_off, out.p, out.ld, 0, w, b, B_, in.H, in.W, c4, stride, act, st);
    }});
  }

  void passthrough(const std::string& name, const Tensor& x, const Tensor& out, int half) {
    int64_t M = (int64_t)B * x.H * x.W;
    Tensor ps = x, o = out;
    Op op{name + "+passthrough", "interleave_copy", 8.0 * M * half, 0.0, [=](cudaStream_t st) {
      return launch_interleave_copy(ps.p, ps.ld, o.p, o.ld, o.map, M, half, st);
    }};
    op.side = true;
    plan->net.push_back(op);
  }

  void pw(const std::string& name, const Tensor& in, int in_off, const Tensor& out, int out_off, int out_step,
          bool join = false, const Tensor* pass = nullptr, const TcGemmParams::Decode* dec = nullptr) {
    const PackedConv& pc = conv(name);
    const ConvSpec& c = spec(name);
    int64_t M = (int64_t)B * in.H * in.W;
    const bool tc_mode = e->cfg.gemm_mode != YNB_GEMM_FP32_FFMA;
    const bool bf = is_bf16(e);
    const double abytes = (double)in.es * M * c.cin + (double)out.es * M * (c.cout + (pass && tc_mode ? 2.0 * c.cout : 0.0)) +
                          (bf ? 2.0 : 4.0) * c.cin * c.cout + 4.0 * c.cout;
    const double aflops = 2.0 * M * c.cin * c.cout;
    if (e->cfg.gemm_mode == YNB_GEMM_FP32_FFMA) {
      GemmParams g{};
      g.a = in.p; g.a_ld = in.ld; g.a_off = in_off; g.a2 = nullptr; g.a2_mode = 0;
      g.w = pc.w_dev; g.bias = pc.b_dev; g.out = out.p; g.out_ld = out.ld;
      g.out_off = out_off; g.out_step = out_step; g.omap = out.map;
      g.M = M; g.N = pc.n; g.Ktot = pc.ktot; g.act = c.act;
      if (pass) { g.out_off = 1; g.out_step = 2; }
      Op op{name, "pw_ffma", abytes, aflops, [=](cudaStream_t st) { return launch_gemm_ffma(g, false, st); }};
      op.join = join;
      ops().push_back(op);
      return;
    }
    tc->emplace_back();
    TcGemmLaunch& L = tc->back();
    L.w = &pc.tc;
    TcGemmParams& p = L.p;
    memset(&p, 0, sizeof(p));
    p.mode = e->cfg.gemm_mode;
    p.is3x3 = 0;
    p.bf16_in = bf ? 1 : 0;
    p.out_bf16 = out.es == 2 ? 1 : 0;
    if (bf && pass) { error = "bf16 mode: the pass-through GEMM epilogue is not built (unit tails go through dwpw): " + name; return; }
    p.num_steps = pc.tc.Kpad / (bf ? 64 : kTcBK);
    p.chunks_per_tap = p.num_steps;
    p.ksub = bf ? (pc.ktot + 15) / 16 : (pc.ktot + 7) / 8;
    p.M = M;
    p.num_tiles = (M + kTcBM - 1) / kTcBM;
    p.N = pc.n; p.Npad = pc.tc.Npad;
    tc_plan_tmem(p, name.size() > 2 && name.compare(0, 8, "head_det") == 0 && name.compare(name.size() - 2, 2, ".4") == 0);
    p.a_box_bytes = kTcAStageBytes;
    p.out = out.p; p.out_ld = out.ld; p.out_off = out_off; p.out_step = out_step; p.omap = out.map;
    p.bias = pc.b_dev; p.act = c.act;
    p.pass = pass ? pass->p : nullptr; p.pass_ld = pass ? pass->ld : 0;
    p.err_flag = e->d_err;
    if (dec) {
      p.dec = *dec;
      L.dec_classes = e->cfg.num_classes;
    }
    const int oal = 16 / out.es;
    p.tma_store = (!dec && !pass && out_step == 1 && out.map.gap == 0 && out_off % oal == 0 && out.ld % oal == 0) ? 1 : 0;
    if (p.tma_store && !make_tmap_out(&L.tmOut, out.at(out_off), (uint64_t)round_up(pc.n, oal), (uint64_t)M,
                                      (uint64_t)out.ld, out.es == 2)) {
      error = "cuTensorMapEncodeTiled failed for output of " + name;
      return;
    }
    if (!make_tmap_2d(&L.tmA, in.at(in_off), (uint64_t)pc.ktot, (uint64_t)M, (uint64_t)in.ld, kTcBM, bf)) {
      error = "cuTensorMapEncodeTiled failed for input of " + name;
      return;
    }
    if (!tc_plan_smem(L)) { error = "no smem configuration for " + name; return; }
    L.grid = (unsigned)std::min<int64_t>(p.num_tiles, kNumSMs);
    const TcGemmLaunch* Lp = &L;
    const double obytes = dec ? abytes - (double)out.es * M * c.cout + 24.0 * M * 3 : abytes;
    Op op{dec ? name + "+decode" : name, dec ? "pw_decode_tcgen05" : "pw_tcgen05", obytes, aflops,
          [=](cudaStream_t st) { return launch_tc_gemm(*Lp, st); }};
    op.join = join;
    ops().push_back(op);
  }

  bool catpw(int si, const std::string& unit, const Tensor& b1dw, const Tensor& mid2, const Tensor& out) {
    static const bool off = getenv("YNB_NO_CAT_GEMM") != nullptr;
    if (off || e->cfg.gemm_mode == YNB_GEMM_FP32_FFMA || e->cat[si].empty()) return false;
    const bool bf = is_bf16(e);
// ... 194 lines not shown
      std::string u = bk + std::to_string(bi);
      Tensor o = P.T(st + "." + std::to_string(bi));
      const int x2_off = x2_window(stage_layout(is_bf16(e), si), h, is_bf16(e) ? 8 : 4).off;
      const bool ffma = e->cfg.gemm_mode == YNB_GEMM_FP32_FFMA;
      P.pw(u + ".branch2.0", x, x2_off, mid1, 0, 1, ffma && bi > 1);
      if (ffma) {
        plan->net.back().mark = true;
        P.passthrough(u, x, o, h);
      }
      if (!P.dwpw(u + ".branch2.3", u + ".branch2.5", mid1, o, &x)) {
        P.dw(u + ".branch2.3", mid1, 0, mid2);
        P.pw(u + ".branch2.5", mid2, 0, o, 1, 2, false, &x);
      }
      x = o;
    }
  }
  Tensor c3 = P.T("c3"), c4 = P.T("c4"), c5 = P.T("c5");
  Tensor lat3 = P.T("lat3"), lat4 = P.T("lat4"), lat5 = P.T("lat5");
  P.pw("conv1x1_0.convs.0", c3, 0, lat3, 0, 1, true);
  P.pw("conv1x1_1.convs.0", c4, 0, lat4, 0, 1);
  P.pw("conv1x1_2.convs.0", c5, 0, lat5, 0, 1);
  Tensor fpn4 = P.T("fpn4"), p3 = P.T("p3"), p4 = P.T("p4"), p5 = P.T("p5");
  P.conv3("smooth_0.convs.0", lat4, &lat5, 1, P.T("sum4"), P.T("sum4.lo"), fpn4);
  P.conv3("smooth_1.convs.0", lat3, &fpn4, 1, P.T("sum3"), P.T("sum3.lo"), p3);
  P.conv3("smooth_2.convs.0", fpn4, &p3, 2, P.T("sum4b"), P.T("sum4b.lo"), p4);
  P.conv3("smooth_3.convs.0", lat5, &p4, 2, P.T("sum5"), P.T("sum5.lo"), p5);
  Tensor feats[3] = {p3, p4, p5};
  Tensor head_in[3];
  for (int l = 0; l < 3; ++l) {
    std::string hd = "head_det_" + std::to_string(l + 1);
    Tensor ta = P.T("head" + std::to_string(l) + ".a"), tb = P.T("head" + std::to_string(l) + ".b");
    if (!P.dwpw(hd + ".0.convs.0", hd + ".1.convs.0", feats[l], ta, nullptr)) {
      P.dw(hd + ".0.convs.0", feats[l], 0, tb);
      P.pw(hd + ".1.convs.0", tb, 0, ta, 0, 1);
    }
    if (!P.dwpw(hd + ".2.convs.0", hd + ".3.convs.0", ta, tb, nullptr)) {
      Tensor tc2 = P.T("head" + std::to_string(l) + ".c");
      P.dw(hd + ".2.convs.0", ta, 0, tc2);
      P.pw(hd + ".3.convs.0", tc2, 0, tb, 0, 1);
    }
    head_in[l] = tb;
  }
  P.dst = &plan->raw_tail;
  for (int l = 0; l < 3; ++l) P.pw("head_det_" + std::to_string(l + 1) + ".4", head_in[l], 0, e->raw[l], 0, 1);
  plan->fused = e->cfg.gemm_mode != YNB_GEMM_FP32_FFMA && e->cfg.num_anchors == 3 &&
                (e->cfg.num_classes == 80 || e->cfg.num_classes == 20) && !getenv("YNB_NO_FUSED_DECODE");
  if (plan->fused) {
    P.dst = &plan->fused_tail;
    int64_t off = 0;
    for (int l = 0; l < 3; ++l) {
      TcGemmParams::Decode d{};
      const int stride = 8 << l;
      d.boxes = e->d_boxes; d.scores = e->d_scores; d.cls = e->d_cls;
      d.G = S / stride; d.HW = d.G * d.G;
      d.stride = (float)stride; d.input_size = (float)S;
      for (int a = 0; a < 3; ++a) {
        d.aw[a] = e->cfg.anchors[(l * 3 + a) * 2];
        d.ah[a] = e->cfg.anchors[(l * 3 + a) * 2 + 1];
      }
      d.Ntot = e->N(); d.level_off = off;
      off += (int64_t)d.HW * 3;
      P.pw("head_det_" + std::to_string(l + 1) + ".4", head_in[l], 0, e->raw[l], 0, 1, false, nullptr, &d);
    }
  }
  P.dst = nullptr;
  if (!P.error.empty()) return fail(e, YNB_ERR_CUDA, P.error);
  int64_t N = e->N(), off = 0;
  for (int l = 0; l < 3; ++l) {
    DecodeParams d{};
    int stride = 8 << l;
    d.raw = e->raw[l].p; d.ld = e->raw[l].ld;
    d.boxes = e->d_boxes; d.scores = e->d_scores; d.cls = e->d_cls;
    d.batch = B; d.G = S / stride; d.A = e->cfg.num_anchors; d.C = e->cfg.num_classes;
    d.stride = (float)stride; d.input_size = (float)S;
    for (int a = 0; a < d.A; ++a) {
      d.anchor_w[a] = e->cfg.anchors[(l * d.A + a) * 2];
      d.anchor_h[a] = e->cfg.anchors[(l * d.A + a) * 2 + 1];
    }
    d.N = N; d.level_off = off;
    off += (int64_t)d.G * d.G * d.A;
    double cells = (double)B * d.G * d.G;
    plan->decode.push_back({"decode.level" + std::to_string(l), "decode",
                            4.0 * cells * d.A * (1 + d.C + 4) + 24.0 * cells * d.A, 0.0,
                            [=](cudaStream_t st) { return launch_decode_level(d, st); }});
  }
  *out = plan.get();
  e->plans[B] = std::move(plan);
  return YNB_OK;
}

int check_ready(ynb_engine* e, int batch) {
  if (!e) return YNB_ERR_INVALID;
  if (!e->committed) return fail(e, YNB_ERR_STATE, "weights not committed (ynb_load_conv x77, ynb_commit_weights)");
  if (batch <= 0) return fail(e, YNB_ERR_INVALID, "batch must be positive");
  return YNB_OK;
}

cudaEvent_t next_event(ynb_engine* e) {
  cudaEvent_t ev = e->events[e->ev_next];
  e->ev_next = (e->ev_next + 1) % e->events.size();
  return ev;
}

struct SideState {
  cudaEvent_t mark = nullptr, done = nullptr;
};

int run_ops(ynb_engine* e, const std::vector<Op>& ops, SideState* ss = nullptr) {
  cudaStream_t st = e->s_main;
  SideState local;
  if (!ss) ss = &local;
  if (!e->profiling) {
    for (const Op& op : ops) {
      if (op.mark) {
        ss->mark = next_event(e);
        CUDA_TRY(e, cudaEventRecord(ss->mark, st));
      }
      if (op.join && ss->done) {
        CUDA_TRY(e, cudaStreamWaitEvent(st, ss->done, 0));
        ss->done = nullptr;
      }
      cudaError_t r;
      if (op.side) {
        if (!ss->mark) {
          ss->mark = next_event(e);
          CUDA_TRY(e, cudaEventRecord(ss->mark, st));
        }
        CUDA_TRY(e, cudaStreamWaitEvent(e->s_side, ss->mark, 0));
        r = op.fn(e->s_side);
        ss->done = next_event(e);
        CUDA_TRY(e, cudaEventRecord(ss->done, e->s_side));
      } else {
        r = op.fn(st);
      }
      if (r != cudaSuccess)
        return fail(e, YNB_ERR_CUDA, "kernel launch (" + op.name + "): " + cudaGetErrorString(r));
    }
    if (ss == &local && ss->done) CUDA_TRY(e, cudaStreamWaitEvent(st, ss->done, 0));
    return YNB_OK;
  }
  std::vector<cudaEvent_t> ev(ops.size() + 1);
  for (auto& x : ev) CUDA_TRY(e, cudaEventCreate(&x));
  CUDA_TRY(e, cudaEventRecord(ev[0], st));
  for (size_t i = 0; i < ops.size(); ++i) {
    cudaError_t r = ops[i].fn(st);
    if (r != cudaSuccess)
      return fail(e, YNB_ERR_CUDA, "kernel launch (" + ops[i].name + "): " + cudaGetErrorString(r));
    CUDA_TRY(e, cudaEventRecord(ev[i + 1], st));
  }
  CUDA_TRY(e, cudaEventSynchronize(ev.back()));
  for (size_t i = 0; i < ops.size(); ++i) {
    float ms = 0;
    CUDA_TRY(e, cudaEventElapsedTime(&ms, ev[i], ev[i + 1]));
    e->prof.push_back({ops[i].name, ops[i].kind, ops[i].bytes, ops[i].flops, ms});
  }
  for (auto& x : ev) cudaEventDestroy(x);
  return YNB_OK;
}

int enter(ynb_engine* e, cudaStream_t user) {
  CUDA_TRY(e, cudaEventRecord(e->ev_in, user));
  CUDA_TRY(e, cudaStreamWaitEvent(e->s_main, e->ev_in, 0));
  return YNB_OK;
}
int leave(ynb_engine* e, cudaStream_t user) {
  CUDA_TRY(e, cudaEventRecord(e->ev_out, e->s_main));
  CUDA_TRY(e, cudaStreamWaitEvent(user, e->ev_out, 0));
  return YNB_OK;
}

int prepare(ynb_engine* e, int batch, Plan** plan_out) {
  int rc = check_ready(e, batch);
  if (rc) return rc;
  CUDA_TRY(e, cudaSetDevice(e->cfg.device));
  if ((rc = ensure_workspace(e, batch))) return rc;
  return build_plan(e, batch, plan_out);
}

int run_network(ynb_engine* e, const float* x_dev, Plan* plan) {
  e->d_x_bound = x_dev;
  e->prof.clear();
  int rc = run_ops(e, plan->net);
  return rc ? rc : run_ops(e, plan->raw_tail);
}

int run_decoded(ynb_engine* e, const float* x_dev, Plan* plan) {
  if (!plan->fused) {
    int rc = run_network(e, x_dev, plan);
    return rc ? rc : run_ops(e, plan->decode);
  }
  e->d_x_bound = x_dev;
  e->prof.clear();
  int rc = run_ops(e, plan->net);
  return rc ? rc : run_ops(e, plan->fused_tail);
}

int check_device_error(ynb_engine* e) {
  cudaStream_t st = e->s_main;
  int flag = 0;
  CUDA_TRY(e, cudaMemcpyAsync(&flag, e->d_err, 4, cudaMemcpyDeviceToHost, st));
  CUDA_TRY(e, cudaStreamSynchronize(st));
  if (flag != 0) {
    cudaMemsetAsync(e->d_err, 0, 4, st);
    return fail(e, YNB_ERR_CUDA, "tensor-core pipeline timed out waiting on mbarrier (code " +
                                     std::to_string(flag) + ")");
  }
  return YNB_OK;
}

}

static void drop_graphs(ynb_engine* e);

YNB_EXPORT int ynb_abi_version(void) { return YNB_ABI_VERSION; }

YNB_EXPORT const char* ynb_last_error(const ynb_engine* e) { return e ? e->err.c_str() : g_create_error.c_str(); }

YNB_EXPORT int ynb_create(const ynb_config* cfg, ynb_engine** out) {
  if (!cfg || !out) return fail(nullptr, YNB_ERR_INVALID, "null argument");
  *out = nullptr;
  if (cfg->abi_version != YNB_ABI_VERSION) return fail(nullptr, YNB_ERR_INVALID, "ABI version mismatch");
  if (cfg->num_anchors != 3) return fail(nullptr, YNB_ERR_UNSUPPORTED, "num_anchors must be 3");
  if (cfg->num_classes < 1 || cfg->num_classes > 255) return fail(nullptr, YNB_ERR_INVALID, "num_classes out of range");
  if (cfg->input_size < 32 || cfg->input_size % 32 || cfg->input_size > 1024)
    return fail(nullptr, YNB_ERR_INVALID, "input_size must be a multiple of 32 in [32, 1024]");
  if (cfg->gemm_mode < 0 || cfg->gemm_mode > YNB_GEMM_TC_BF16) return fail(nullptr, YNB_ERR_INVALID, "bad gemm_mode");
  int ndev = 0;
  cudaError_t st = cudaGetDeviceCount(&ndev);
  if (st != cudaSuccess || ndev == 0)
    return fail(nullptr, YNB_ERR_NO_DEVICE,
                std::string("no CUDA device: ") + (st != cudaSuccess ? cudaGetErrorString(st) : "count is 0") +
                    " (this library has no CPU path)");
  if (cfg->device < 0 || cfg->device >= ndev) return fail(nullptr, YNB_ERR_INVALID, "device ordinal out of range");
  cudaDeviceProp prop;
  if (cudaGetDeviceProperties(&prop, cfg->device) != cudaSuccess || prop.major != 10)
    return fail(nullptr, YNB_ERR_NO_DEVICE, "device is not compute capability 10.x (built for sm_100a only)");
  if (cudaSetDevice(cfg->device) != cudaSuccess) return fail(nullptr, YNB_ERR_CUDA, "cudaSetDevice failed");
  ynb_engine* e = new ynb_engine();
  e->cfg = *cfg;
  if (e->cfg.max_batch < 1) e->cfg.max_batch = 1;
  e->S = cfg->input_size;
  {
    const float mean[3] = {0.406f, 0.456f, 0.485f}, stdv[3] = {0.225f, 0.224f, 0.229f};
    make_prelut(&e->prelut, mean, stdv);
  }
  e->table = conv_table(cfg->num_classes, cfg->num_anchors);
  e->convs.resize(e->table.size());
  for (size_t i = 0; i < e->table.size(); ++i) e->index[e->table[i].name] = (int)i;
  bool ok = cudaStreamCreateWithFlags(&e->s_main, cudaStreamNonBlocking) == cudaSuccess &&
            cudaStreamCreateWithFlags(&e->s_side, cudaStreamNonBlocking) == cudaSuccess &&
            cudaEventCreateWithFlags(&e->ev_in, cudaEventDisableTiming) == cudaSuccess &&
            cudaEventCreateWithFlags(&e->ev_out, cudaEventDisableTiming) == cudaSuccess;
  ok = ok && cudaStreamCreateWithFlags(&e->s_copy, cudaStreamNonBlocking) == cudaSuccess;
  ok = ok && cudaStreamCreateWithFlags(&e->s_copy2, cudaStreamNonBlocking) == cudaSuccess;
  ok = ok && cudaEventCreateWithFlags(&e->ev_copy2, cudaEventDisableTiming) == cudaSuccess;
  ok = ok && cudaStreamCreateWithFlags(&e->s_d2h, cudaStreamNonBlocking) == cudaSuccess;
  ok = ok && cudaMalloc(&e->d_prelut, sizeof(PreLut)) == cudaSuccess &&
       cudaMemcpy(e->d_prelut, &e->prelut, sizeof(PreLut), cudaMemcpyHostToDevice) == cudaSuccess;
  for (int k = 0; k < 2 && ok; ++k)
    ok = cudaEventCreateWithFlags(&e->slot[k].h2d, cudaEventDisableTiming) == cudaSuccess &&
         cudaEventCreateWithFlags(&e->slot[k].done, cudaEventDisableTiming) == cudaSuccess &&
         cudaHostAlloc(&e->slot[k].flag_host, 64, cudaHostAllocDefault) == cudaSuccess;
  e->events.resize(64);
  for (auto& ev : e->events) ok = ok && cudaEventCreateWithFlags(&ev, cudaEventDisableTiming) == cudaSuccess;
  if (!ok) {
    delete e;
    return fail(nullptr, YNB_ERR_CUDA, "stream / event creation failed");
  }
  *out = e;
  return YNB_OK;
}

static void drop_graphs(ynb_engine* e) {
  for (auto& kv : e->graphs) cudaGraphExecDestroy(kv.second);
  e->graphs.clear();
  e->graph_seen.clear();
}

YNB_EXPORT void ynb_destroy(ynb_engine* e) {
  if (!e) return;
  cudaSetDevice(e->cfg.device);
  cudaDeviceSynchronize();
  drop_graphs(e);
  for (auto ev : e->events) cudaEventDestroy(ev);
  if (e->ev_in) cudaEventDestroy(e->ev_in);
  if (e->ev_out) cudaEventDestroy(e->ev_out);
  for (int k = 0; k < 2; ++k) {
    if (e->slot[k].h2d) cudaEventDestroy(e->slot[k].h2d);
    if (e->slot[k].done) cudaEventDestroy(e->slot[k].done);
    if (e->slot[k].flag_host) cudaFreeHost(e->slot[k].flag_host);
  }
  if (e->s_copy) cudaStreamDestroy(e->s_copy);
  if (e->s_copy2) cudaStreamDestroy(e->s_copy2);
  if (e->ev_copy2) cudaEventDestroy(e->ev_copy2);
  if (e->s_d2h) cudaStreamDestroy(e->s_d2h);
  if (e->d_prelut) cudaFree(e->d_prelut);
  if (e->s_main) cudaStreamDestroy(e->s_main);
  if (e->s_side) cudaStreamDestroy(e->s_side);
  for (PackedConv& pc : e->convs) {
    if (pc.w_dev) cudaFree(pc.w_dev);
    if (pc.b_dev) cudaFree(pc.b_dev);
    if (pc.tc.hi) cudaFree(pc.tc.hi);
    if (pc.tc.lo) cudaFree(pc.tc.lo);
    if (pc.tc.bw) cudaFree(pc.tc.bw);
  }
  for (int si = 0; si < 3; ++si)
    for (auto& cc : e->cat[si]) {
      if (cc.pc.b_dev) cudaFree(cc.pc.b_dev);
      if (cc.pc.tc.hi) cudaFree(cc.pc.tc.hi);
      if (cc.pc.tc.lo) cudaFree(cc.pc.tc.lo);
      if (cc.pc.tc.bw) cudaFree(cc.pc.tc.bw);
    }
  if (e->ws) cudaFree(e->ws);
  delete e;
}

YNB_EXPORT int ynb_set_grid(ynb_engine* e, int32_t input_size) {
  if (!e) return YNB_ERR_INVALID;
  if (input_size < 32 || input_size % 32 || input_size > 1024)
    return fail(e, YNB_ERR_INVALID, "input_size must be a multiple of 32 in [32, 1024]");
  if (input_size != e->S) e->stem_maps.clear();
  e->S = input_size;
  return YNB_OK;
}

YNB_EXPORT int ynb_set_thresholds(ynb_engine* e, float conf, float nms, int32_t diou) {
  if (!e) return YNB_ERR_INVALID;
  e->cfg.conf_thresh = conf; e->cfg.nms_thresh = nms; e->cfg.diou_nms = diou;
  return YNB_OK;
}

YNB_EXPORT int ynb_set_gemm_mode(ynb_engine* e, int32_t mode) {
  if (!e) return YNB_ERR_INVALID;
  if (mode < 0 || mode > YNB_GEMM_TC_BF16) return fail(e, YNB_ERR_INVALID, "bad gemm_mode");
  if ((mode == YNB_GEMM_TC_BF16) != (e->cfg.gemm_mode == YNB_GEMM_TC_BF16))
    return fail(e, YNB_ERR_UNSUPPORTED, "bf16 mode changes the activation storage and the weight packing: create the "
                                        "engine with gemm_mode = YNB_GEMM_TC_BF16 instead of switching");
  if (mode != e->cfg.gemm_mode) {
    cudaDeviceSynchronize();
    e->cfg.gemm_mode = mode; e->plans.clear(); e->tc_store.clear(); e->dp_store.clear(); e->dw_maps.clear(); drop_graphs(e);
  }
  return YNB_OK;
}

YNB_EXPORT int64_t ynb_num_boxes(const ynb_engine* e) { return e ? e->N() : 0; }

YNB_EXPORT int64_t ynb_workspace_bytes(const ynb_engine* e, int32_t batch) {
  if (!e || batch < 1) return 0;
  ynb_engine tmp;
  tmp.cfg = e->cfg;
  return (int64_t)layout_workspace(&tmp, batch, e->S, nullptr);
}

YNB_EXPORT int32_t ynb_num_convs(void) { return 77; }

YNB_EXPORT const char* ynb_conv_name(int32_t i) {
  static const std::vector<ConvSpec> t = conv_table(80, 3);
  return (i >= 0 && i < (int)t.size()) ? t[i].name.c_str() : nullptr;
}

YNB_EXPORT int ynb_conv_shape(int32_t i, int32_t num_classes, int32_t num_anchors, int32_t* cout,
                              int32_t* cin_per_group, int32_t* ksize) {
  std::vector<ConvSpec> t = conv_table(num_classes, num_anchors);
  if (i < 0 || i >= (int)t.size() || !cout || !cin_per_group || !ksize) return YNB_ERR_INVALID;
  *cout = t[i].cout;
  *cin_per_group = t[i].kind == kDw3x3 ? 1 : t[i].cin;
  *ksize = t[i].kind == kPw1x1 ? 1 : 3;
  return YNB_OK;
}

YNB_EXPORT int ynb_load_conv(ynb_engine* e, const char* name, const float* w, int64_t w_elems, const float* b,
                             int64_t b_elems) {
  if (!e || !name || !w || !b) return fail(e, YNB_ERR_INVALID, "null argument");
  auto it = e->index.find(name);
  if (it == e->index.end()) return fail(e, YNB_ERR_INVALID, std::string("unknown conv ") + name);
  const ConvSpec& c = e->table[it->second];
  int64_t expect = (int64_t)c.cout * (c.kind == kDw3x3 ? 1 : c.cin) * (c.kind == kPw1x1 ? 1 : 9);
  if (w_elems != expect || b_elems != c.cout)
    return fail(e, YNB_ERR_INVALID, std::string("shape mismatch for ") + name);
  PackedConv& pc = e->convs[it->second];
  pc.w_host.assign(w, w + w_elems);
  pc.b_host.assign(b, b + b_elems);
  pc.loaded = true;
  e->committed = false;
  return YNB_OK;
}

YNB_EXPORT int ynb_commit_weights(ynb_engine* e) {
  if (!e) return YNB_ERR_INVALID;
  CUDA_TRY(e, cudaSetDevice(e->cfg.device));
  for (size_t i = 0; i < e->convs.size(); ++i)
    if (!e->convs[i].loaded) return fail(e, YNB_ERR_STATE, "conv not loaded: " + e->table[i].name);
  CUDA_TRY(e, cudaDeviceSynchronize());
  e->plans.clear();
  e->tc_store.clear(); e->dp_store.clear(); e->dw_maps.clear();
  drop_graphs(e);
  for (size_t i = 0; i < e->convs.size(); ++i) {
    int rc = pack_conv(e, (int)i);
    if (rc) return rc;
  }
  for (int si = 0; si < 3; ++si) {
    int rc = pack_cat(e, si);
    if (rc) return rc;
  }
  e->committed = true;
  return YNB_OK;
}

YNB_EXPORT int ynb_forward_raw(ynb_engine* e, const float* x_dev, int32_t batch, float* ps, float* pm, float* pl,
                               void* stream) {
  if (!e || !x_dev || !ps || !pm || !pl) return fail(e, YNB_ERR_INVALID, "null argument");
  cudaStream_t user = (cudaStream_t)stream;
  CounterScope cs(e);
  Plan* plan = nullptr;
  int rc = prepare(e, batch, &plan);
  if (rc || (rc = enter(e, user)) || (rc = run_network(e, x_dev, plan))) return rc;
  float* outs[3] = {ps, pm, pl};
  for (int l = 0; l < 3; ++l) {
    const Tensor& t = e->raw[l];
    CUDA_TRY(e, launch_nhwc_to_nchw(t.p, t.ld, t.map, outs[l], batch, t.C, t.H * t.W, e->s_main, t.es == 2));
  }
  if ((rc = leave(e, user))) return rc;
  return e->cfg.gemm_mode == YNB_GEMM_FP32_FFMA ? YNB_OK : check_device_error(e);
}

YNB_EXPORT int ynb_forward_decode(ynb_engine* e, const float* x_dev, int32_t batch, float* boxes, float* scores,
                                  int32_t* cls, void* stream) {
  if (!e || !x_dev || !boxes || !scores || !cls) return fail(e, YNB_ERR_INVALID, "null argument");
  cudaStream_t user = (cudaStream_t)stream;
  CounterScope cs(e);
  Plan* plan = nullptr;
  int rc = prepare(e, batch, &plan);
  if (rc || (rc = enter(e, user)) || (rc = run_decoded(e, x_dev, plan))) return rc;
  int64_t n = e->N();
  cudaStream_t st = e->s_main;
  CUDA_TRY(e, cudaMemcpyAsync(boxes, e->d_boxes, (size_t)batch * n * 16, cudaMemcpyDeviceToDevice, st));
  CUDA_TRY(e, cudaMemcpyAsync(scores, e->d_scores, (size_t)batch * n * 4, cudaMemcpyDeviceToDevice, st));
  CUDA_TRY(e, cudaMemcpyAsync(cls, e->d_cls, (size_t)batch * n * 4, cudaMemcpyDeviceToDevice, st));
  if ((rc = leave(e, user))) return rc;
  return e->cfg.gemm_mode == YNB_GEMM_FP32_FFMA ? YNB_OK : check_device_error(e);
}

static int detect_ops(ynb_engine* e, Plan* plan, const float* x_dev, int batch, float* ob, float* os, int32_t* oc,
                      int32_t* on) {
  int rc = run_decoded(e, x_dev, plan);
  if (rc) return rc;
  const int64_t n = e->N();
  std::vector<Op> nms_ops(1);
  static const bool sorted_nms = getenv("YNB_NMS_SORTED") != nullptr;
  if (!sorted_nms && e->cfg.num_anchors == 3 && n <= 65535 && e->S % 32 == 0) {
    GridNmsWorkspace gw = grid_nms_carve(e->d_nms_ws, batch, n);
    const int S = e->S;
    nms_ops[0] = {"nms(prep+build+resolve+compact)", "nms", 24.0 * batch * n * 2, 0.0, [=](cudaStream_t s2) {
      return launch_nms_grid(e->d_boxes, e->d_scores, e->d_cls, batch, S, e->cfg.num_classes, e->cfg.conf_thresh,
                             e->cfg.nms_thresh, e->cfg.diou_nms, ob, os, oc, on, nullptr, gw, s2);
    }};
    return run_ops(e, nms_ops);
  }
  NmsWorkspace w = nms_carve(e->d_nms_ws, batch, e->N());
  nms_ops[0] = {"nms(keys+sort+greedy+compact)", "nms", 24.0 * batch * n * 2, 0.0, [=](cudaStream_t s2) {
    return launch_nms(e->d_boxes, e->d_scores, e->d_cls, batch, n, e->cfg.num_classes, e->cfg.conf_thresh,
                      e->cfg.nms_thresh, e->cfg.diou_nms, ob, os, oc, on, nullptr, w, s2);
  }};
  return run_ops(e, nms_ops);
}

static int detect_device(ynb_engine* e, const float* x_dev, int batch, float* ob, float* os, int32_t* oc,
                         int32_t* on) {
  Plan* plan = nullptr;
  int rc = prepare(e, batch, &plan);
  if (rc) return rc;
  if (!e->use_graphs || e->profiling) return detect_ops(e, plan, x_dev, batch, ob, os, oc, on);
  ynb_engine::GraphKey key{batch, x_dev, ob, os, oc, on, e->cfg.conf_thresh, e->cfg.nms_thresh,
                           e->cfg.diou_nms, e->cfg.gemm_mode, e->S};
  auto it = e->graphs.find(key);
  if (it == e->graphs.end()) {
    if (e->graph_seen.size() > 256) e->graph_seen.clear();
    if (e->graph_seen[key]++ == 0) return detect_ops(e, plan, x_dev, batch, ob, os, oc, on);
    if (e->graphs.size() >= 32) drop_graphs(e);
    cudaGraph_t graph = nullptr;
    CUDA_TRY(e, cudaStreamBeginCapture(e->s_main, cudaStreamCaptureModeThreadLocal));
    const int64_t l0 = e->counter.n;
    rc = detect_ops(e, plan, x_dev, batch, ob, os, oc, on);
    e->graph_launches[batch] = e->counter.n - l0;
    e->counter.n = l0;
    cudaError_t ce = cudaStreamEndCapture(e->s_main, &graph);
    if (rc) { if (graph) cudaGraphDestroy(graph); return rc; }
    if (ce != cudaSuccess) return fail(e, YNB_ERR_CUDA, std::string("cudaStreamEndCapture: ") + cudaGetErrorString(ce));
    cudaGraphExec_t exec = nullptr;
    ce = cudaGraphInstantiate(&exec, graph, 0);
    cudaGraphDestroy(graph);
    if (ce != cudaSuccess) return fail(e, YNB_ERR_CUDA, std::string("cudaGraphInstantiate: ") + cudaGetErrorString(ce));
    it = e->graphs.emplace(key, exec).first;
  }
  CUDA_TRY(e, cudaGraphLaunch(it->second, e->s_main));
  e->counter.n += e->graph_launches[batch];
  return YNB_OK;
}

YNB_EXPORT int ynb_forward_detect(ynb_engine* e, const float* x_dev, int32_t batch, float* ob, float* os,
                                  int32_t* oc, int32_t* on, void* stream) {
  if (!e || !x_dev || !ob || !os || !oc || !on) return fail(e, YNB_ERR_INVALID, "null argument");
  cudaStream_t user = (cudaStream_t)stream;
  CounterScope cs(e);
  int rc = check_ready(e, batch);
  if (rc || (rc = enter(e, user)) || (rc = detect_device(e, x_dev, batch, ob, os, oc, on))) return rc;
  return leave(e, user);
}

static int submit_host_common(ynb_engine* e, int32_t slot_id, const float* x_host, const uint8_t* img_host,
                              const int32_t* rects_host, int32_t batch, float* ob, float* os, int32_t* oc,
                              int32_t* on, void* stream) {
  if (!e || (!x_host && !img_host) || !ob || !os || !oc || !on) return fail(e, YNB_ERR_INVALID, "null argument");
  if (slot_id < 0 || slot_id > 1) return fail(e, YNB_ERR_INVALID, "slot must be 0 or 1");
  cudaStream_t user = (cudaStream_t)stream;
  CounterScope cs(e);
  Plan* plan = nullptr;
  int rc = prepare(e, batch, &plan);
  if (rc) return rc;
  ynb_engine::HostSlot& sl = e->slot[slot_id];
  if (sl.busy) return fail(e, YNB_ERR_STATE, "slot still in flight: call ynb_wait_host first");
  const size_t px = (size_t)3 * e->S * e->S;
  CUDA_TRY(e, cudaEventRecord(e->ev_in, user));
  CUDA_TRY(e, cudaStreamWaitEvent(e->s_copy, e->ev_in, 0));
  if (x_host) {
    const size_t total = px * 4 * batch, half = (total / 2) & ~(size_t)255;
    CUDA_TRY(e, cudaStreamWaitEvent(e->s_copy2, e->ev_in, 0));
    CUDA_TRY(e, cudaMemcpyAsync(sl.x, x_host, half, cudaMemcpyHostToDevice, e->s_copy));
    CUDA_TRY(e, cudaMemcpyAsync(reinterpret_cast<char*>(sl.x) + half, reinterpret_cast<const char*>(x_host) + half,
                                total - half, cudaMemcpyHostToDevice, e->s_copy2));
    CUDA_TRY(e, cudaEventRecord(e->ev_copy2, e->s_copy2));
    CUDA_TRY(e, cudaStreamWaitEvent(e->s_copy, e->ev_copy2, 0));
  } else {
    CUDA_TRY(e, cudaMemcpyAsync(sl.img_u8, img_host, px * batch, cudaMemcpyHostToDevice, e->s_copy));
    if (rects_host)
      CUDA_TRY(e, cudaMemcpyAsync(sl.rects, rects_host, (size_t)batch * 16, cudaMemcpyHostToDevice, e->s_copy));
  }
  CUDA_TRY(e, cudaEventRecord(sl.h2d, e->s_copy));
  CUDA_TRY(e, cudaStreamWaitEvent(e->s_main, sl.h2d, 0));
  if (!x_host)
    CUDA_TRY(e, launch_preprocess_u8(sl.img_u8, rects_host ? sl.rects : nullptr, sl.x, e->d_prelut, batch, e->S,
                                     e->s_main));
  if ((rc = detect_device(e, sl.x, batch, sl.boxes, sl.scores, sl.cls, sl.counts))) return rc;
  CUDA_TRY(e, cudaMemcpyAsync(on, sl.counts, (size_t)batch * 4, cudaMemcpyDeviceToHost, e->s_main));
  CUDA_TRY(e, cudaMemcpyAsync(sl.flag_host, e->d_err, 4, cudaMemcpyDeviceToHost, e->s_main));
  CUDA_TRY(e, cudaEventRecord(sl.done, e->s_main));
  sl.busy = true; sl.batch = batch; sl.ob = ob; sl.os = os; sl.oc = oc; sl.on = on;
  return YNB_OK;
}

YNB_EXPORT int ynb_submit_host(ynb_engine* e, int32_t slot_id, const float* x_host, int32_t batch, float* ob,
                               float* os, int32_t* oc, int32_t* on, void* stream) {
  if (!x_host) return fail(e, YNB_ERR_INVALID, "null argument");
  return submit_host_common(e, slot_id, x_host, nullptr, nullptr, batch, ob, os, oc, on, stream);
}

YNB_EXPORT int ynb_submit_host_u8(ynb_engine* e, int32_t slot_id, const uint8_t* img_host, const int32_t* rects_host,
                                  int32_t batch, float* ob, float* os, int32_t* oc, int32_t* on, void* stream) {
  if (!img_host) return fail(e, YNB_ERR_INVALID, "null argument");
  return submit_host_common(e, slot_id, nullptr, img_host, rects_host, batch, ob, os, oc, on, stream);
}

YNB_EXPORT int ynb_set_normalization(ynb_engine* e, const float* mean_bgr, const float* std_bgr) {
  if (!e || !mean_bgr || !std_bgr) return fail(e, YNB_ERR_INVALID, "null argument");
  for (int c = 0; c < 3; ++c)
    if (!(std_bgr[c] > 0.0f)) return fail(e, YNB_ERR_INVALID, "std must be positive");
  make_prelut(&e->prelut, mean_bgr, std_bgr);
  CUDA_TRY(e, cudaSetDevice(e->cfg.device));
  CUDA_TRY(e, cudaDeviceSynchronize());
  CUDA_TRY(e, cudaMemcpy(e->d_prelut, &e->prelut, sizeof(PreLut), cudaMemcpyHostToDevice));
  return YNB_OK;
}

YNB_EXPORT int ynb_preprocess_u8(ynb_engine* e, const uint8_t* img_dev, const int32_t* rects_dev, int32_t batch,
                                 float* x_dev, void* stream) {
  if (!e || !img_dev || !x_dev || batch <= 0) return fail(e, YNB_ERR_INVALID, "null argument");
  CUDA_TRY(e, cudaSetDevice(e->cfg.device));
  cudaError_t r = launch_preprocess_u8(img_dev, rects_dev, x_dev, e->d_prelut, batch, e->S, (cudaStream_t)stream);
  if (r != cudaSuccess) return fail(e, YNB_ERR_CUDA, std::string("preprocess_u8: ") + cudaGetErrorString(r));
  return YNB_OK;
}

static_assert(sizeof(ynb_image_desc) == sizeof(ImageDesc), "ynb_image_desc and the kernel's ImageDesc must agree");

YNB_EXPORT int ynb_preprocess_letterbox_u8(ynb_engine* e, const uint8_t* src_dev, const ynb_image_desc* descs_dev,
                                           int32_t batch, float* x_dev, void* stream) {
  if (!e || !src_dev || !descs_dev || !x_dev || batch <= 0) return fail(e, YNB_ERR_INVALID, "null argument");
  CUDA_TRY(e, cudaSetDevice(e->cfg.device));
  cudaError_t r = launch_letterbox_preprocess(src_dev, reinterpret_cast<const ImageDesc*>(descs_dev), x_dev, e->d_prelut,
                                              batch, e->S, (cudaStream_t)stream);
  if (r != cudaSuccess) return fail(e, YNB_ERR_CUDA, std::string("letterbox_preprocess: ") + cudaGetErrorString(r));
  return YNB_OK;
}

YNB_EXPORT int ynb_map_boxes(float* boxes_dev, const int32_t* counts_dev, const double* maps_dev, int32_t batch,
                             int64_t n_per_image, void* stream) {
  if (!boxes_dev || !counts_dev || !maps_dev || batch <= 0 || n_per_image <= 0)
    return fail(nullptr, YNB_ERR_INVALID, "ynb_map_boxes: bad arguments");
  cudaError_t r = launch_map_boxes(boxes_dev, counts_dev, maps_dev, batch, n_per_image, (cudaStream_t)stream);
  if (r != cudaSuccess) return fail(nullptr, YNB_ERR_CUDA, std::string("map_boxes: ") + cudaGetErrorString(r));
  return YNB_OK;
}

YNB_EXPORT int ynb_wait_host(ynb_engine* e, int32_t slot_id) {
  if (!e || slot_id < 0 || slot_id > 1) return fail(e, YNB_ERR_INVALID, "bad slot");
  ynb_engine::HostSlot& sl = e->slot[slot_id];
  if (!sl.busy) return fail(e, YNB_ERR_STATE, "nothing submitted on this slot");
  CUDA_TRY(e, cudaSetDevice(e->cfg.device));
  CUDA_TRY(e, cudaEventSynchronize(sl.done));
  sl.busy = false;
  if (*sl.flag_host != 0) {
    int code = *sl.flag_host;
    cudaMemsetAsync(e->d_err, 0, 4, e->s_main);
    return fail(e, YNB_ERR_CUDA, "tensor-core pipeline timed out waiting on mbarrier (code " + std::to_string(code) + ")");
  }
  const int64_t n = e->N();
  size_t kmax = 0;
  for (int b = 0; b < sl.batch; ++b) kmax = std::max(kmax, (size_t)sl.on[b]);
  if (kmax > 0) {
    CUDA_TRY(e, cudaMemcpy2DAsync(sl.ob, (size_t)n * 16, sl.boxes, (size_t)n * 16, kmax * 16, sl.batch,
                                  cudaMemcpyDeviceToHost, e->s_d2h));
    CUDA_TRY(e, cudaMemcpy2DAsync(sl.os, (size_t)n * 4, sl.scores, (size_t)n * 4, kmax * 4, sl.batch,
                                  cudaMemcpyDeviceToHost, e->s_d2h));
    CUDA_TRY(e, cudaMemcpy2DAsync(sl.oc, (size_t)n * 4, sl.cls, (size_t)n * 4, kmax * 4, sl.batch,
                                  cudaMemcpyDeviceToHost, e->s_d2h));
    CUDA_TRY(e, cudaStreamSynchronize(e->s_d2h));
  }
  return YNB_OK;
}

YNB_EXPORT int ynb_detect_host(ynb_engine* e, const float* x_host, int32_t batch, float* ob, float* os,
                               int32_t* oc, int32_t* on, void* stream) {
  if (!e) return YNB_ERR_INVALID;
  if (e->slot[0].busy) return fail(e, YNB_ERR_STATE, "slot 0 in flight (ynb_submit_host without ynb_wait_host)");
  int rc = ynb_submit_host(e, 0, x_host, batch, ob, os, oc, on, stream);
  return rc ? rc : ynb_wait_host(e, 0);
}

YNB_EXPORT int ynb_tap_shape(const ynb_engine* e, const char* tap, int32_t* c, int32_t* h, int32_t* w) {
  if (!e || !tap || !c || !h || !w) return YNB_ERR_INVALID;
  ynb_engine* me = const_cast<ynb_engine*>(e);
  if (me->taps.empty()) {
    ynb_engine tmp;
    tmp.cfg = e->cfg;
    layout_workspace(&tmp, 1, e->S, nullptr);
    me->taps = tmp.taps;
  }
  auto it = me->taps.find(tap);
  if (it == me->taps.end()) return fail(me, YNB_ERR_INVALID, std::string("unknown tap ") + tap);
  int hh = it->second.H;
  if (me->ws_S != me->S) {
    ynb_engine tmp;
    tmp.cfg = e->cfg;
    layout_workspace(&tmp, 1, e->S, nullptr);
    hh = tmp.taps.at(tap).H;
  }
  *c = it->second.C; *h = hh; *w = hh;
  return YNB_OK;
}

YNB_EXPORT int ynb_read_tap(ynb_engine* e, const char* tap, int32_t batch, float* out_dev, void* stream) {
  if (!e || !tap || !out_dev) return fail(e, YNB_ERR_INVALID, "null argument");
  if (!e->ws || e->ws_S != e->S || batch > e->ws_batch) return fail(e, YNB_ERR_STATE, "run a forward first");
  auto it = e->taps.find(tap);
  if (it == e->taps.end() || !it->second.p) return fail(e, YNB_ERR_INVALID, std::string("unknown tap ") + tap);
  const Tensor& t = it->second;
  CounterScope cs(e);
  int rc = enter(e, (cudaStream_t)stream);
  if (rc) return rc;
  CUDA_TRY(e, launch_nhwc_to_nchw(t.p, t.ld, t.map, out_dev, batch, t.C, t.H * t.W, e->s_main, t.es == 2));
  return leave(e, (cudaStream_t)stream);
}

YNB_EXPORT int64_t ynb_launch_count(const ynb_engine* e) { return e ? e->counter.n : 0; }

YNB_EXPORT int ynb_set_profiling(ynb_engine* e, int32_t on) {
  if (!e) return YNB_ERR_INVALID;
  e->profiling = on != 0;
  return YNB_OK;
}

YNB_EXPORT int32_t ynb_profile_count(const ynb_engine* e) { return e ? (int32_t)e->prof.size() : 0; }

YNB_EXPORT int ynb_profile_entry(const ynb_engine* e, int32_t i, const char** name, const char** kind, float* ms,
                                 double* bytes, double* flops) {
  if (!e || i < 0 || i >= (int32_t)e->prof.size() || !name || !kind || !ms || !bytes || !flops) return YNB_ERR_INVALID;
  const ProfEntry& p = e->prof[i];
  *name = p.name.c_str(); *kind = p.kind.c_str(); *ms = p.ms; *bytes = p.bytes; *flops = p.flops;
  return YNB_OK;
}

static thread_local std::string g_unit_error;
#define UNIT_TRY(call)                                                       \
  do {                                                                       \
    cudaError_t _st = (call);                                                \
    if (_st != cudaSuccess) {                                                \
      g_create_error = std::string(#call) + ": " + cudaGetErrorString(_st);  \
      return YNB_ERR_CUDA;                                                   \
    }                                                                        \
  } while (0)

YNB_EXPORT int ynb_dwconv3x3(const float* in, int32_t in_ld, int32_t in_off, float* out, int32_t out_ld,
                             int32_t out_off, int32_t out_step, const float* w, const float* b, int32_t batch,
                             int32_t h_in, int32_t w_in, int32_t channels, int32_t stride, int32_t act, void* stream) {
  if (!in || !out || !w || !b || channels % 4 || in_ld % 4 || in_off % 4 || out_ld % 4 || out_off % 4 ||
      out_step != 1 || (stride != 1 && stride != 2))
    return fail(nullptr, YNB_ERR_INVALID, "ynb_dwconv3x3: channels/ld/off must be multiples of 4, out_step 1");
  CUtensorMap tm;
  if (!getenv("YNB_DW_NO_TMA") && make_tmap_dw(&tm, in, in_ld, in_off, batch, h_in, w_in, channels, stride)) {
    UNIT_TRY(launch_dwconv3x3_tma(tm, out, out_ld, out_off, w, b, batch, h_in, w_in, channels, stride, act,
                                  (cudaStream_t)stream));
    return YNB_OK;
  }
  UNIT_TRY(launch_dwconv3x3(in, in_ld, in_off, out, out_ld, out_off, w, b, batch, h_in, w_in, channels, stride, act,
                            (cudaStream_t)stream));
  return YNB_OK;
}

YNB_EXPORT int ynb_resize_bilinear(const float* in_dev, int32_t batch, int32_t h_in, int32_t w_in, float* out_dev,
                                   int32_t s_out, int32_t with_flip, void* stream) {
  if (!in_dev || !out_dev || batch <= 0 || h_in <= 0 || w_in <= 0 || s_out <= 0)
    return fail(nullptr, YNB_ERR_INVALID, "ynb_resize_bilinear: bad arguments");
  UNIT_TRY(launch_resize_bilinear(in_dev, out_dev, batch, h_in, w_in, s_out, with_flip, (cudaStream_t)stream));
  return YNB_OK;
}

YNB_EXPORT int ynb_pwconv(const float* in, int32_t in_ld, int32_t in_off, float* out, int32_t out_ld,
                          int32_t out_off, int32_t out_step, const float* w, const float* b, int64_t pixels,
                          int32_t cin, int32_t cout, int32_t act, void* stream) {
  if (!in || !out || !w || !b || cin % 4 || in_ld % 4 || in_off % 4)
    return fail(nullptr, YNB_ERR_INVALID, "ynb_pwconv: cin / in_ld / in_off must be multiples of 4");
  GemmParams g{};
  g.a = in; g.a_ld = in_ld; g.a_off = in_off; g.w = w; g.bias = b; g.out = out; g.out_ld = out_ld;
  g.out_off = out_off; g.out_step = out_step; g.omap = dense_map(); g.M = pixels; g.N = cout; g.Ktot = cin;
  g.act = act;
  UNIT_TRY(launch_gemm_ffma(g, false, (cudaStream_t)stream));
  return YNB_OK;
}

YNB_EXPORT int ynb_pwconv_tc(const float* in, int32_t in_ld, int32_t in_off, float* out, int32_t out_ld,
                             int32_t out_off, int32_t out_step, const float* w_dev, const float* b_dev,
                             int64_t pixels, int32_t cin, int32_t cout, int32_t act, int32_t mode, void* stream) {
  if (!in || !out || !w_dev || !b_dev || cin % 4 || in_ld % 4 || in_off % 4 || out_ld % 4 ||
      (out_step == 1 && out_off % 4) || cout > 256 || (mode != YNB_GEMM_TC_3XTF32 && mode != YNB_GEMM_TC_TF32))
    return fail(nullptr, YNB_ERR_INVALID, "ynb_pwconv_tc: bad arguments");
  cudaStream_t st = (cudaStream_t)stream;
  std::vector<float> w((size_t)cout * cin);
  UNIT_TRY(cudaMemcpy(w.data(), w_dev, w.size() * 4, cudaMemcpyDeviceToHost));
  TcWeights t;
  t.N = cout; t.Npad = round_up(cout, 16); t.Kpad = round_up(cin, kTcBK);
  std::vector<float> hi((size_t)t.Npad * t.Kpad, 0.f), lo((size_t)t.Npad * t.Kpad, 0.f);
  for (int n = 0; n < cout; ++n)
    for (int k = 0; k < cin; ++k)
      split_tf32_host(w[(size_t)n * cin + k], &hi[(size_t)n * t.Kpad + k], &lo[(size_t)n * t.Kpad + k]);
  int* d_err = nullptr;
  UNIT_TRY(cudaMalloc(&t.hi, hi.size() * 4));
  UNIT_TRY(cudaMalloc(&t.lo, lo.size() * 4));
  UNIT_TRY(cudaMalloc(&d_err, 4));
  UNIT_TRY(cudaMemset(d_err, 0, 4));
  UNIT_TRY(cudaMemcpy(t.hi, hi.data(), hi.size() * 4, cudaMemcpyHostToDevice));
  UNIT_TRY(cudaMemcpy(t.lo, lo.data(), lo.size() * 4, cudaMemcpyHostToDevice));
  int rc = YNB_OK;
  TcGemmLaunch L;
  L.w = &t;
  TcGemmParams& p = L.p;
  memset(&p, 0, sizeof(p));
  p.mode = mode; p.num_steps = t.Kpad / kTcBK; p.chunks_per_tap = p.num_steps; p.ksub = (cin + 7) / 8;
  p.M = pixels; p.num_tiles = (pixels + kTcBM - 1) / kTcBM; p.N = cout; p.Npad = t.Npad;
  tc_plan_tmem(p);
  p.a_box_bytes = kTcAStageBytes;
  p.out = out; p.out_ld = out_ld; p.out_off = out_off; p.out_step = out_step; p.omap = dense_map();
  p.bias = b_dev; p.act = act; p.err_flag = d_err;
  long long* d_trace = nullptr;
  const int trace_cap = 8 * 64 * 32;
  const bool want_trace = getenv("YNB_TC_TRACE") != nullptr;
  if (want_trace) {
    UNIT_TRY(cudaMalloc(&d_trace, (1 + 4 * trace_cap) * 8));
    UNIT_TRY(cudaMemset(d_trace, 0, (1 + 4 * trace_cap) * 8));
    p.trace = d_trace; p.trace_cap = trace_cap;
  }
  p.tma_store = (out_step == 1 && out_off % 4 == 0 && getenv("YNB_TC_NO_TMA_STORE") == nullptr) ? 1 : 0;
  if (getenv("YNB_TC_PASS") != nullptr && cin >= cout && out_ld >= 2 * cout) {
    p.pass = in; p.pass_ld = in_ld; p.tma_store = 0; p.out_off = 1; p.out_step = 2;
  }
  if (!make_tmap_2d(&t.tm_hi, t.hi, t.Kpad, t.Npad, t.Kpad, t.Npad) ||
      !make_tmap_2d(&t.tm_lo, t.lo, t.Kpad, t.Npad, t.Kpad, t.Npad) ||
      (p.tma_store && !make_tmap_out(&L.tmOut, out + out_off, (uint64_t)round_up(cout, 4), (uint64_t)pixels,
                                     (uint64_t)out_ld)) ||
      !make_tmap_2d(&L.tmA, in + in_off, cin, pixels, in_ld, kTcBM) || !tc_plan_smem(L)) {
    rc = fail(nullptr, YNB_ERR_CUDA, "ynb_pwconv_tc: tensor map / smem planning failed");
  } else {
    L.grid = (unsigned)std::min<int64_t>(p.num_tiles, kNumSMs);
    cudaError_t r = launch_tc_gemm(L, st);
    if (r == cudaSuccess) r = cudaStreamSynchronize(st);
    int flag = 0;
    if (r == cudaSuccess) r = cudaMemcpy(&flag, d_err, 4, cudaMemcpyDeviceToHost);
    if (r != cudaSuccess) rc = fail(nullptr, YNB_ERR_CUDA, std::string("ynb_pwconv_tc: ") + cudaGetErrorString(r));
    else if (flag) rc = fail(nullptr, YNB_ERR_CUDA, "ynb_pwconv_tc: mbarrier timeout code " + std::to_string(flag));
    if (want_trace && r == cudaSuccess) {
      std::vector<long long> h(1 + 4 * trace_cap);
      cudaMemcpy(h.data(), d_trace, h.size() * 8, cudaMemcpyDeviceToHost);
      int n = 0;
      for (int i = 0; i < trace_cap; ++i) n += h[4 + 4 * i] != 0;
      fprintf(stderr, "YNB_TC_TRACE stages=%d resident=%d nmain=%d acc_stages=%d steps=%d grid=%u events=%d\n",
              p.num_stages, p.w_resident, p.nmain, p.acc_stages, p.num_steps, L.grid, n);
      for (int i = 0; i < trace_cap; ++i)
        if (h[4 + 4 * i] != 0)
          fprintf(stderr, "TRACE %lld %lld %lld %lld\n", h[1 + 4 * i], h[2 + 4 * i], h[3 + 4 * i], h[4 + 4 * i]);
    }
  }
  if (d_trace) cudaFree(d_trace);
  cudaFree(t.hi); cudaFree(t.lo); cudaFree(d_err);
  return rc;
}

YNB_EXPORT int ynb_dwpw_tc(const float* in, int32_t in_ld, const float* dw_w, const float* dw_b, int32_t dw_act,
                           const float* pw_w, const float* pw_b, int32_t act, float* out, int32_t out_ld,
                           const float* pass, int32_t pass_ld, int32_t batch, int32_t h, int32_t w_, int32_t channels,
                           int32_t cout, int32_t mode, void* stream) {
  const bool bfm = mode == YNB_GEMM_TC_BF16;
  const int al = bfm ? 8 : 4;
  if (!in || !dw_w || !dw_b || !pw_w || !pw_b || !out || channels % al || in_ld % al || out_ld % al || cout > (bfm ? 240 : 128) ||
      cout < 1 || batch < 1 || h < 1 || w_ < 1 ||
      (mode != YNB_GEMM_TC_3XTF32 && mode != YNB_GEMM_TC_TF32 && mode != YNB_GEMM_TC_BF16) ||
      (pass && (out_ld < 2 * cout || pass_ld < cout || pass_ld % 4 || ((uintptr_t)pass & 15u))) || (!pass && out_ld < cout) ||
      ((uintptr_t)out & 15u))
    return fail(nullptr, YNB_ERR_INVALID, "ynb_dwpw_tc: bad arguments");
  cudaStream_t st = (cudaStream_t)stream;
  std::vector<float> wv((size_t)cout * channels);
  UNIT_TRY(cudaMemcpy(wv.data(), pw_w, wv.size() * 4, cudaMemcpyDeviceToHost));
  TcWeights t;
  t.N = cout; t.Npad = round_up(cout, 16); t.Kpad = round_up(channels, bfm ? 64 : kTcBK);
  std::vector<float> hi((size_t)t.Npad * t.Kpad, 0.f), lo((size_t)t.Npad * t.Kpad, 0.f);
  std::vector<bf16> bwv((size_t)t.Npad * t.Kpad, __float2bfloat16(0.0f));
  for (int n = 0; n < cout; ++n)
    for (int k = 0; k < channels; ++k) {
      split_tf32_host(wv[(size_t)n * channels + k], &hi[(size_t)n * t.Kpad + k], &lo[(size_t)n * t.Kpad + k]);
      bwv[(size_t)n * t.Kpad + k] = __float2bfloat16_rn(wv[(size_t)n * channels + k]);
    }
  int* d_err = nullptr;
  UNIT_TRY(cudaMalloc(&t.hi, hi.size() * 4));
  UNIT_TRY(cudaMalloc(&t.lo, lo.size() * 4));
  UNIT_TRY(cudaMalloc(&d_err, 4));
  UNIT_TRY(cudaMemset(d_err, 0, 4));
  UNIT_TRY(cudaMemcpy(t.hi, hi.data(), hi.size() * 4, cudaMemcpyHostToDevice));
  UNIT_TRY(cudaMemcpy(t.lo, lo.data(), lo.size() * 4, cudaMemcpyHostToDevice));
  if (bfm) UNIT_TRY(cudaMemcpy(t.hi, bwv.data(), bwv.size() * 2, cudaMemcpyHostToDevice));
  int rc = YNB_OK;
  DwPwLaunch L;
  DwPwParams& p = L.p;
  memset(&p, 0, sizeof(p));
  p.dw_w = dw_w; p.dw_b = dw_b; p.dw_act = dw_act;
  p.out = out; p.out_ld = out_ld; p.out_off = 0; p.omap = dense_map();
  p.bias = pw_b; p.act = act; p.pass = pass; p.pass_ld = pass ? pass_ld : 0; p.err_flag = d_err;
  long long* d_trace = nullptr;
  const bool want_trace = getenv("YNB_DP_TRACE") != nullptr;
  if (want_trace) {
    UNIT_TRY(cudaMalloc(&d_trace, 6 * 16 * 8 * 8));
    UNIT_TRY(cudaMemset(d_trace, 0, 6 * 16 * 8 * 8));
    p.trace = d_trace;
  }
  if (!make_tmap_2d(&t.tm_hi, t.hi, t.Kpad, t.Npad, t.Kpad, t.Npad, bfm) ||
      !make_tmap_2d(&t.tm_lo, t.lo, t.Kpad, t.Npad, t.Kpad, t.Npad) ||
      !plan_dwpw(L, in, in_ld, batch, h, w_, channels, channels, &t, mode)) {
    rc = fail(nullptr, YNB_ERR_CUDA, "ynb_dwpw_tc: tensor map / smem planning failed");
  } else {
    cudaError_t r = launch_dwpw_tc(L, st);
    if (r == cudaSuccess) r = cudaStreamSynchronize(st);
    int flag = 0;
    if (r == cudaSuccess) r = cudaMemcpy(&flag, d_err, 4, cudaMemcpyDeviceToHost);
    if (r != cudaSuccess) rc = fail(nullptr, YNB_ERR_CUDA, std::string("ynb_dwpw_tc: ") + cudaGetErrorString(r));
    else if (flag) rc = fail(nullptr, YNB_ERR_CUDA, "ynb_dwpw_tc: mbarrier timeout code " + std::to_string(flag));
    if (want_trace && r == cudaSuccess) {
      std::vector<long long> h(6 * 16 * 8);
      cudaMemcpy(h.data(), d_trace, h.size() * 8, cudaMemcpyDeviceToHost);
      long long t0 = 0;
      for (long long v : h) if (v && (!t0 || v < t0)) t0 = v;
      fprintf(stderr, "YNB_DP_TRACE chunks=%d a_stages=%d raw_stages=%d resident=%d lgTW=%d tiles=%lld grid=%u\n", L.p.num_chunks,
              L.p.a_stages, L.p.raw_stages, L.p.w_resident, L.p.lgTW, (long long)L.p.num_tiles, L.grid);
      const char* names[6] = {"raw_issued", "raw_landed", "A_written", "mma_issued", "acc_ready", "epi_done"};
      for (int lt = 0; lt < 16; ++lt)
        for (int role = 0; role < 6; ++role) {
          std::string line;
          for (int kc = 0; kc < 8; ++kc)
            if (h[(role * 16 + lt) * 8 + kc]) line += " " + std::to_string(h[(role * 16 + lt) * 8 + kc] - t0);
          if (!line.empty()) fprintf(stderr, "TRACE tile %2d %-11s%s\n", lt, names[role], line.c_str());
        }
    }
  }
  if (d_trace) cudaFree(d_trace);
  cudaFree(t.hi); cudaFree(t.lo); cudaFree(d_err);
  return rc;
}

YNB_EXPORT int ynb_stem_pool(const float* x, float* out, const float* w, const float* b, int32_t batch,
                             int32_t input_size, void* stream) {
  if (!x || !out || !w || !b || input_size % 32) return fail(nullptr, YNB_ERR_INVALID, "ynb_stem_pool: bad arguments");
  StemWeights wt;
  UNIT_TRY(cudaMemcpy(wt.w, w, sizeof(wt.w), cudaMemcpyDeviceToHost));
  UNIT_TRY(cudaMemcpy(wt.b, b, sizeof(wt.b), cudaMemcpyDeviceToHost));
  CUtensorMap tmx{};
  const int use_tma = make_tmap_stem_input(&tmx, x, input_size, batch) ? 1 : 0;
  UNIT_TRY(launch_stem_pool(x, out, false, wt, tmx, use_tma, batch, input_size, (cudaStream_t)stream));
  return YNB_OK;
}

YNB_EXPORT int ynb_decode_level(const float* raw, int32_t raw_ld, float* boxes, float* scores, int32_t* cls,
                                int32_t batch, int32_t grid, int32_t stride_px, int32_t input_size,
                                const float* anchors_wh, int32_t num_anchors, int32_t num_classes,
                                int64_t boxes_per_image, int64_t level_off, void* stream) {
  if (!raw || !boxes || !scores || !cls || !anchors_wh || num_anchors > 4)
    return fail(nullptr, YNB_ERR_INVALID, "ynb_decode_level: bad arguments");
  DecodeParams d{};
  d.raw = raw; d.ld = raw_ld; d.boxes = boxes; d.scores = scores; d.cls = cls; d.batch = batch; d.G = grid;
  d.A = num_anchors; d.C = num_classes; d.stride = (float)stride_px; d.input_size = (float)input_size;
  for (int a = 0; a < num_anchors; ++a) { d.anchor_w[a] = anchors_wh[2 * a]; d.anchor_h[a] = anchors_wh[2 * a + 1]; }
  d.N = boxes_per_image; d.level_off = level_off;
  UNIT_TRY(launch_decode_level(d, (cudaStream_t)stream));
  return YNB_OK;
}

YNB_EXPORT int64_t ynb_nms_workspace_bytes(int32_t batch, int64_t n) { return nms_workspace_bytes(batch, n); }

YNB_EXPORT int64_t ynb_nms_grid_workspace_bytes(int32_t batch, int32_t input_size) {
  return grid_nms_workspace_bytes(batch, make_grid_geom(input_size).N);
}

YNB_EXPORT int ynb_nms_grid(const float* boxes, const float* scores, const int32_t* cls, int32_t batch,
                            int32_t input_size, int32_t num_classes, float conf, float thr, int32_t diou, float* ob,
                            float* os, int32_t* oc, int32_t* on, uint8_t* keep, void* ws, int64_t ws_bytes,
                            void* stream) {
  if (!boxes || !scores || !cls || !ob || !os || !oc || !on || !ws || input_size <= 0 || input_size % 32 ||
      ws_bytes < ynb_nms_grid_workspace_bytes(batch, input_size))
    return fail(nullptr, YNB_ERR_INVALID, "ynb_nms_grid: bad arguments / workspace too small");
  GridNmsWorkspace w = grid_nms_carve(ws, batch, make_grid_geom(input_size).N);
  UNIT_TRY(launch_nms_grid(boxes, scores, cls, batch, input_size, num_classes, conf, thr, diou, ob, os, oc, on, keep,
                           w, (cudaStream_t)stream));
  return YNB_OK;
}

YNB_EXPORT int ynb_nms(const float* boxes, const float* scores, const int32_t* cls, int32_t batch, int64_t n,
                       int32_t num_classes, float conf, float thr, int32_t diou, float* ob, float* os, int32_t* oc,
                       int32_t* on, uint8_t* keep, void* ws, int64_t ws_bytes, void* stream) {
  if (!boxes || !scores || !cls || !ob || !os || !oc || !on || !ws || ws_bytes < nms_workspace_bytes(batch, n))
    return fail(nullptr, YNB_ERR_INVALID, "ynb_nms: bad arguments / workspace too small");
  NmsWorkspace w = nms_carve(ws, batch, n);
  UNIT_TRY(launch_nms(boxes, scores, cls, batch, n, num_classes, conf, thr, diou, ob, os, oc, on, keep, w,
                      (cudaStream_t)stream));
  return YNB_OK;
}


namespace {
bool level_geometry(int input_size, int grid[3], int stride[3]) {
  if (input_size <= 0 || input_size % 32) return false;
  const int st[3] = {8, 16, 32};
  for (int l = 0; l < 3; ++l) { stride[l] = st[l]; grid[l] = input_size / st[l]; }
  return true;
}
}

YNB_EXPORT int64_t ynb_train_loss_workspace_bytes(int32_t batch, int32_t input_size) {
  return (int64_t)train_loss_blocks(batch, input_size) * 4 * sizeof(double);
}

YNB_EXPORT int ynb_train_loss(const float* raw_s, const float* raw_m, const float* raw_l, int32_t raw_ld,
                              const float* target, int32_t batch, int32_t input_size, const float* anchors_wh,
                              int32_t num_anchors, int32_t num_classes, float* losses, float* grad_s, float* grad_m,
                              float* grad_l, void* ws, int64_t ws_bytes, void* stream) {
  TrainLossParams p{};
  if (!raw_s || !raw_m || !raw_l || !target || !anchors_wh || !losses || !grad_s || !grad_m || !grad_l || !ws ||
      batch <= 0 || num_anchors <= 0 || num_anchors > kTrainMaxAnchors || num_classes <= 0 ||
      raw_ld < num_anchors * (1 + num_classes + 4) || !level_geometry(input_size, p.grid, p.stride) ||
      ws_bytes < ynb_train_loss_workspace_bytes(batch, input_size))
    return fail(nullptr, YNB_ERR_INVALID, "ynb_train_loss: bad arguments / workspace too small");
  p.raw[0] = raw_s; p.raw[1] = raw_m; p.raw[2] = raw_l;
  p.grad[0] = grad_s; p.grad[1] = grad_m; p.grad[2] = grad_l;
  p.target = target; p.partials = (double*)ws; p.ld = raw_ld; p.B = batch; p.A = num_anchors; p.C = num_classes;
  p.S = input_size;
  int off = 0;
  for (int l = 0; l < 3; ++l) {
    p.cells[l] = p.grid[l] * p.grid[l];
    p.cell_off[l] = off;
    off += p.cells[l];
    for (int a = 0; a < num_anchors; ++a) {
      p.anchors[l][a][0] = anchors_wh[(l * num_anchors + a) * 2];
      p.anchors[l][a][1] = anchors_wh[(l * num_anchors + a) * 2 + 1];
    }
  }
  p.cells_total = off;
  UNIT_TRY(launch_train_loss(p, losses, (cudaStream_t)stream));
  return YNB_OK;
}

YNB_EXPORT int ynb_build_targets(const float* labels, const int32_t* counts, int32_t batch, int32_t max_labels,
                                 int32_t input_size, const float* anchors_wh, int32_t num_anchors, float* target,
                                 void* stream) {
  TargetParams p{};
  if (!labels || !target || !anchors_wh || batch <= 0 || max_labels < 0 || num_anchors <= 0 ||
      num_anchors > kTrainMaxAnchors || !level_geometry(input_size, p.grid, p.stride))
    return fail(nullptr, YNB_ERR_INVALID, "ynb_build_targets: bad arguments");
  p.labels = labels; p.counts = counts; p.target = target; p.B = batch; p.L = max_labels; p.A = num_anchors;
  p.S = input_size;
  long long off = 0;
  for (int l = 0; l < 3; ++l) {
    p.row_off[l] = off;
    off += (long long)p.grid[l] * p.grid[l] * num_anchors;
  }
  p.N = off;
  for (int k = 0; k < 3 * num_anchors; ++k) {
    p.anchors[k][0] = (double)anchors_wh[2 * k];
    p.anchors[k][1] = (double)anchors_wh[2 * k + 1];
  }
  UNIT_TRY(launch_build_targets(p, (cudaStream_t)stream));
  return YNB_OK;
}

YNB_EXPORT int ynb_sgd_step(float* params, const float* grads, float* momentum_buf, int64_t n, float lr,
                            float momentum, float weight_decay, int32_t first_step, float grad_scale, void* stream) {
  if (!params || !grads || !momentum_buf || n <= 0 || ((uintptr_t)params | (uintptr_t)grads | (uintptr_t)momentum_buf) % 16)
    return fail(nullptr, YNB_ERR_INVALID, "ynb_sgd_step: null / unaligned (16 B) buffers");
  UNIT_TRY(launch_sgd_step(params, grads, momentum_buf, n, lr, momentum, weight_decay, first_step, grad_scale,
                           (cudaStream_t)stream));
  return YNB_OK;
}

YNB_EXPORT int32_t ynb_ema_chunk_elems(void) { return kEmaChunk; }

YNB_EXPORT int ynb_ema_update(const uint64_t* ema_ptrs_dev, const uint64_t* model_ptrs_dev, const int64_t* sizes_dev,
                              const int32_t* chunk_tensor_dev, const int32_t* chunk_index_dev, int32_t num_chunks,
                              float d, float one_minus_d, void* stream) {
  if (!ema_ptrs_dev || !model_ptrs_dev || !sizes_dev || !chunk_tensor_dev || !chunk_index_dev || num_chunks < 0)
    return fail(nullptr, YNB_ERR_INVALID, "ynb_ema_update: bad arguments");
  UNIT_TRY(launch_ema_update(reinterpret_cast<const unsigned long long*>(ema_ptrs_dev),
                             reinterpret_cast<const unsigned long long*>(model_ptrs_dev),
                             reinterpret_cast<const long long*>(sizes_dev), chunk_tensor_dev, chunk_index_dev, num_chunks,
                             d, one_minus_d, (cudaStream_t)stream));
  return YNB_OK;
}

YNB_EXPORT int ynb_dwconv3x3_bwd_data(const float* dout, int32_t do_ld, int32_t do_off, float* din, int32_t di_ld,
                                      int32_t di_off, const float* w, int32_t batch, int32_t h_in, int32_t w_in,
                                      int32_t channels, int32_t stride, void* stream) {
  if (!dout || !din || !w || batch <= 0 || h_in <= 0 || w_in <= 0 || channels <= 0 || (stride != 1 && stride != 2))
    return fail(nullptr, YNB_ERR_INVALID, "ynb_dwconv3x3_bwd_data: bad arguments");
  cudaStream_t st = (cudaStream_t)stream;
  const bool vec = channels % 4 == 0 && do_ld % 4 == 0 && do_off % 4 == 0 && di_ld % 4 == 0 && di_off % 4 == 0 &&
                   ((uintptr_t)dout | (uintptr_t)din | (uintptr_t)w) % 16 == 0;
  CUtensorMap tm;
  if (stride == 1 && vec && !getenv("YNB_DW_NO_TMA") &&
      make_tmap_dw(&tm, dout, do_ld, do_off, batch, h_in, w_in, channels, 1)) {
    UNIT_TRY(launch_dwconv3x3_tma(tm, din, di_ld, di_off, w, nullptr, batch, h_in, w_in, channels, 1, YNB_ACT_NONE, st,
                                  true));
    return YNB_OK;
  }
  if (stride == 2 && vec && 9 * channels * 4 <= 48 * 1024) {
    const long long items = (long long)batch * ((h_in + 1) / 2) * ((w_in + 1) / 2) * (channels / 4);
    const int nb = (int)std::min<long long>((items + 255) / 256, (long long)kNumSMs * 8);
    dwconv3x3_s2_bwd_data_kernel<<<nb, 256, 9 * channels * sizeof(float), st>>>(dout, do_ld, do_off, din, di_ld, di_off, w,
                                                                               batch, h_in, w_in, channels);
    YNB_COUNT_LAUNCH();
    UNIT_TRY(cudaGetLastError());
    return YNB_OK;
  }
  const long long total = (long long)batch * h_in * w_in * ((channels + 3) / 4);
  const int blocks = (int)std::min<long long>((total + 255) / 256, (long long)kNumSMs * 16);
  if (vec)
    dwconv3x3_bwd_data_kernel<true><<<blocks, 256, 0, st>>>(dout, do_ld, do_off, din, di_ld, di_off, w, batch, h_in, w_in,
                                                            channels, stride);
  else
    dwconv3x3_bwd_data_kernel<false><<<blocks, 256, 0, st>>>(dout, do_ld, do_off, din, di_ld, di_off, w, batch, h_in, w_in,
                                                             channels, stride);
  YNB_COUNT_LAUNCH();
  UNIT_TRY(cudaGetLastError());
  return YNB_OK;
}

YNB_EXPORT int64_t ynb_dwconv3x3_bwd_weight_workspace_bytes(int32_t batch, int32_t h_in, int32_t w_in, int32_t channels,
                                                            int32_t stride) {
  const int h_out = (h_in - 1) / stride + 1, w_out = (w_in - 1) / stride + 1;
  return (int64_t)dw_bwd_chunks(batch, h_out, w_out) * 10 * channels * sizeof(float);
}

YNB_EXPORT int ynb_dwconv3x3_bwd_weight(const float* dout, int32_t do_ld, int32_t do_off, const float* in, int32_t in_ld,
                                        int32_t in_off, float* dwdb, int32_t batch, int32_t h_in, int32_t w_in,
                                        int32_t channels, int32_t stride, void* ws, int64_t ws_bytes, void* stream) {
  if (!dout || !in || !dwdb || !ws || batch <= 0 || h_in <= 0 || w_in <= 0 || channels <= 0 ||
      (stride != 1 && stride != 2) ||
      ws_bytes < ynb_dwconv3x3_bwd_weight_workspace_bytes(batch, h_in, w_in, channels, stride))
    return fail(nullptr, YNB_ERR_INVALID, "ynb_dwconv3x3_bwd_weight: bad arguments / workspace too small");
  const int h_out = (h_in - 1) / stride + 1, w_out = (w_in - 1) / stride + 1;
  const int chunks = dw_bwd_chunks(batch, h_out, w_out);
  const bool vec = channels % 4 == 0 && do_ld % 4 == 0 && do_off % 4 == 0 && in_ld % 4 == 0 && in_off % 4 == 0 &&
                   ((uintptr_t)dout | (uintptr_t)in) % 16 == 0;
  dim3 grid(chunks, (channels + kDwBwdCg * 4 - 1) / (kDwBwdCg * 4)), block(kDwBwdCg, kDwBwdSlices);
  cudaStream_t st = (cudaStream_t)stream;
  float* part = (float*)ws;
#define YNB_DWBW(S, V) \
  dwconv3x3_bwd_weight_kernel<S, V><<<grid, block, 0, st>>>(dout, do_ld, do_off, in, in_ld, in_off, part, batch, h_in, w_in, channels)
  if (stride == 1) { if (vec) YNB_DWBW(1, true); else YNB_DWBW(1, false); }
  else             { if (vec) YNB_DWBW(2, true); else YNB_DWBW(2, false); }
#undef YNB_DWBW
  YNB_COUNT_LAUNCH();
  launch_reduce_partials(part, chunks, 10LL * channels, dwdb, st);
  UNIT_TRY(cudaGetLastError());
  return YNB_OK;
}

static bool pw_wgrad_use_tc(int cin) { return wgrad_tc_kpad(cin) != 0 && !getenv("YNB_PWBW_FFMA"); }

YNB_EXPORT int64_t ynb_pwconv_bwd_weight_workspace_bytes(int64_t pixels, int32_t cin, int32_t cout) {
  int64_t floats = (int64_t)pw_bwd_chunks(pixels, cin, cout) * ((int64_t)cout * cin + cout);
  if (wgrad_tc_kpad(cin)) floats = std::max<int64_t>(floats, wgrad_tc_partial_floats(pixels, cin, cout));
  return floats * sizeof(float) + 16;
}

YNB_EXPORT int ynb_pwconv_bwd_weight(const float* dout, int32_t do_ld, int32_t do_off, const float* in, int32_t in_ld,
                                     int32_t in_off, float* dw, float* db, int64_t pixels, int32_t cin, int32_t cout,
                                     void* ws, int64_t ws_bytes, void* stream) {
  if (!dout || !in || !dw || !db || !ws || pixels <= 0 || cin <= 0 || cout <= 0 ||
      ws_bytes < ynb_pwconv_bwd_weight_workspace_bytes(pixels, cin, cout))
    return fail(nullptr, YNB_ERR_INVALID, "ynb_pwconv_bwd_weight: bad arguments / workspace too small");
  const bool aligned = cin % 4 == 0 && cout % 4 == 0 && do_ld % 4 == 0 && do_off % 4 == 0 && in_ld % 4 == 0 &&
                       in_off % 4 == 0 && ((uintptr_t)dout | (uintptr_t)in) % 16 == 0;
  if (pw_wgrad_use_tc(cin) && aligned) {
    cudaStream_t st = (cudaStream_t)stream;
    const int chunks = wgrad_tc_chunks(pixels, cout);
    int* err = (int*)((char*)ws + ynb_pwconv_bwd_weight_workspace_bytes(pixels, cin, cout) - 16);
    UNIT_TRY(cudaMemsetAsync(err, 0, 4, st));
    WgradParams p{};
    p.dout = dout; p.do_ld = do_ld; p.do_off = do_off; p.in = in; p.in_ld = in_ld; p.in_off = in_off;
    p.partial = (float*)ws; p.M = pixels; p.K = cin; p.N = cout; p.err = err;
    UNIT_TRY(launch_pw_wgrad_tc(p, chunks, st));
    {
      const int ntiles = (cout + 127) / 128, kpad = wgrad_tc_kpad(cin);
      const long long elems = (long long)ntiles * 128 * kpad;
      launch_wgrad_reduce((const float*)ws, chunks, ntiles, kpad, cout, cin, dw, db, st);
      YNB_COUNT_LAUNCH();
    }
    UNIT_TRY(cudaGetLastError());
    if (getenv("YNB_SYNC_CHECK")) {
      int flag = 0;
      UNIT_TRY(cudaStreamSynchronize(st));
      UNIT_TRY(cudaMemcpy(&flag, err, 4, cudaMemcpyDeviceToHost));
      if (flag) return fail(nullptr, YNB_ERR_CUDA, "ynb_pwconv_bwd_weight: mbarrier timeout code " + std::to_string(flag));
    }
    return YNB_OK;
  }
  const int chunks = pw_bwd_chunks(pixels, cin, cout);
  long long m_per_chunk = (pixels + chunks - 1) / chunks;
  m_per_chunk = (m_per_chunk + kPwBwdSlab - 1) / kPwBwdSlab * kPwBwdSlab;
  float* pw = (float*)ws;
  float* pb = pw + (long long)chunks * cout * cin;
  cudaStream_t st = (cudaStream_t)stream;
  const int vec = cin % 4 == 0 && cout % 4 == 0 && do_ld % 4 == 0 && do_off % 4 == 0 && in_ld % 4 == 0 &&
                  in_off % 4 == 0 && ((uintptr_t)dout | (uintptr_t)in) % 16 == 0;
  dim3 grid(chunks, (cout + kPwBwdTile - 1) / kPwBwdTile, (cin + kPwBwdTile - 1) / kPwBwdTile);
  if (vec && !getenv("YNB_PWBW_NO_ASYNC")) {
    UNIT_TRY(cudaFuncSetAttribute(pwconv_bwd_weight_async_kernel, cudaFuncAttributeMaxDynamicSharedMemorySize,
                                  (int)kPwBwdAsyncSmem));
    pwconv_bwd_weight_async_kernel<<<grid, 256, kPwBwdAsyncSmem, st>>>(dout, do_ld, do_off, in, in_ld, in_off, pw, pb,
                                                                       pixels, cin, cout, m_per_chunk);
  } else {
    pwconv_bwd_weight_kernel<<<grid, 256, 0, st>>>(dout, do_ld, do_off, in, in_ld, in_off, pw, pb, pixels, cin, cout,
                                                   m_per_chunk, vec);
  }
  YNB_COUNT_LAUNCH();
  launch_reduce_partials(pw, chunks, (long long)cout * cin, dw, st);
  launch_reduce_partials(pb, chunks, cout, db, st);
  UNIT_TRY(cudaGetLastError());
  return YNB_OK;
}

YNB_EXPORT int ynb_act_bwd(const float* dout, int32_t do_ld, int32_t do_off, const float* out, int32_t o_ld,
                           int32_t o_off, float* dpre, int32_t dp_ld, int32_t dp_off, int64_t pixels, int32_t channels,
                           int32_t act, void* stream) {
  if (!dout || !out || !dpre || pixels <= 0 || channels <= 0 || (act != YNB_ACT_RELU && act != YNB_ACT_LEAKY))
    return fail(nullptr, YNB_ERR_INVALID, "ynb_act_bwd: bad arguments");
  const long long total = (long long)pixels * channels;
  const int blocks = (int)std::min<long long>((total + 255) / 256, (long long)kNumSMs * 16);
  act_bwd_kernel<<<blocks, 256, 0, (cudaStream_t)stream>>>(dout, do_ld, do_off, out, o_ld, o_off, dpre, dp_ld, dp_off,
                                                           pixels, channels, act == YNB_ACT_RELU ? 0.0f : 0.1f);
  YNB_COUNT_LAUNCH();
  UNIT_TRY(cudaGetLastError());
  return YNB_OK;
}

YNB_EXPORT int ynb_forward_train_loss(ynb_engine* e, const float* x_dev, int32_t batch, const float* target,
                                      float* losses, float* grad_s, float* grad_m, float* grad_l, void* ws,
                                      int64_t ws_bytes, void* stream) {
  if (!e || !x_dev || !target || !losses || !grad_s || !grad_m || !grad_l || !ws)
    return fail(e, YNB_ERR_INVALID, "null argument");
  if (ws_bytes < ynb_train_loss_workspace_bytes(batch, e->S))
    return fail(e, YNB_ERR_INVALID, "ynb_forward_train_loss: workspace too small");
// ... 435 lines not shown
```

Measured before the change: 35410.

## Stream raw fp32 weights and split them to TF32 hi/lo on chip

For non-resident weights in the 3xTF32 GEMM and fused dw+pw kernels, a single raw fp32 weight tile is now loaded by TMA instead of separate pre-split hi and lo tiles. The split into hi and lo happens in shared memory, done by the splitter warps plus warp 15 in the GEMM and by the weight warp in the dw+pw kernel. This halves weight global/L2 traffic per stage. The cost is extra ALU work and an added barrier, and the dw+pw kernel's weight warp is serialized on TMA-then-split, which could stall the MMA.

```diff
diff --git a/yolo_nano_b200/csrc/gemm_tc.cuh b/yolo_nano_b200/csrc/gemm_tc.cuh
--- a/yolo_nano_b200/csrc/gemm_tc.cuh
+++ b/yolo_nano_b200/csrc/gemm_tc.cuh
@@ -37,6 +37,7 @@
   int ksub;
   int presplit;
   int a2_step;
+  int w_f32;
   int stack_b;
   int acc_stages;
   uint32_t tmem_cols;
@@ -101,6 +102,34 @@
 
 __host__ __device__ __forceinline__ uint32_t rn_tf32_bits(uint32_t u) { return (u + 0x1000u) & 0xffffe000u; }
 
+__device__ __forceinline__ void split_tf32_bits(uint32_t u, uint32_t& h, uint32_t& l) {
+  h = rn_tf32_bits(u);
+  l = rn_tf32_bits(__float_as_uint(__uint_as_float(u) - __uint_as_float(h)));
+}
+
+__device__ __forceinline__ void split_tf32_weight_bits(uint32_t u, uint32_t& h, uint32_t& l) {
+  split_tf32_bits(u, h, l);
+  if ((u & 0x7f800000u) == 0x7f800000u) l = rn_tf32_bits((u & 0x007fffffu) ? (u | 0x00400000u) : 0xffc00000u);
+}
+
+template <bool kWeight>
+__device__ __forceinline__ void split_box_tf32(uint4* x, uint4* lo, int n16, int t, int nthreads) {
+#pragma unroll 4
+  for (int i = t; i < n16; i += nthreads) {
+    const uint4 v = x[i];
+    uint4 h, l;
+    if (kWeight) {
+      split_tf32_weight_bits(v.x, h.x, l.x); split_tf32_weight_bits(v.y, h.y, l.y);
+      split_tf32_weight_bits(v.z, h.z, l.z); split_tf32_weight_bits(v.w, h.w, l.w);
+    } else {
+      split_tf32_bits(v.x, h.x, l.x); split_tf32_bits(v.y, h.y, l.y);
+      split_tf32_bits(v.z, h.z, l.z); split_tf32_bits(v.w, h.w, l.w);
+    }
+    x[i] = h;
+    lo[i] = l;
+  }
+}
+
 template <bool kPass, int kDecC>
 __global__ void __launch_bounds__(kTcThreads, 1)
 tc_gemm_kernel(const __grid_constant__ CUtensorMap tmA, const __grid_constant__ CUtensorMap tmAlo,
@@ -113,7 +142,7 @@
   const int kchunk = p.bf16_in ? 64 : kTcBK;
   const int box_alo = p.presplit ? 1 : -1;
   const int box_whi = p.w_resident ? -1 : 1 + (p.presplit ? 1 : 0);
-  const int box_wlo = (p.w_resident || !split) ? -1 : box_whi + 1;
+  const int box_wlo = (p.w_resident || !split || p.w_f32) ? -1 : box_whi + 1;
   const int nboxes = 1 + (box_alo >= 0) + (box_whi >= 0) + (box_wlo >= 0);
   const int nprod = nboxes < kTcProducers ? nboxes : kTcProducers;
   const TcSmemLayout lay = tc_smem_layout(p.Npad, p.num_steps, p.num_stages, p.w_resident != 0, split);
@@ -142,7 +171,7 @@
     if (p.tma_store) ptx::prefetch_tmap(&tmOut);
     for (int s = 0; s < p.num_stages; ++s) {
       ptx::mbar_init(&full[s], nprod);
-      ptx::mbar_init(&ready[s], 4);
+      ptx::mbar_init(&ready[s], p.w_f32 ? 5 : 4);
       ptx::mbar_init(&empty[s], 1);
     }
     for (int a = 0; a < 2; ++a) {
@@ -173,7 +202,6 @@
   auto w_lo_ptr = [&](int s, int step) { return w_hi_ptr(s, step) + w_chunk_bytes; };
 
   const int acc_cols = p.Npad * p.nacc;
-  const uint32_t step_tx = p.a_box_bytes * (p.presplit ? 2 : 1) + (p.w_resident ? 0 : w_chunk_bytes * (split ? 2 : 1));
   const bool splitters_on = split && !p.presplit;
 
   if (warp == kTcProducerWarp && p.w_resident && ptx::elect_one()) {
@@ -185,7 +213,7 @@
   }
   pdl_wait();
 
-  const int prole = warp == kTcProducerWarp ? 0 : (warp == 14 ? 1 : (warp == 15 ? 2 : -1));
+  const int prole = warp == kTcProducerWarp ? 0 : (warp == 14 ? 1 : (warp == 15 && nprod > 2 ? 2 : -1));
   if (prole >= 0) {
     if (prole < nprod && ptx::elect_one()) {
       const bool do_a = 0 % nprod == prole;
@@ -295,9 +323,9 @@
         if (++acc == p.acc_stages) { acc = 0; acc_ph ^= 1; }
       }
     }
-  } else if (warp >= kTcSplitWarp0 && warp < kTcSplitWarp0 + 4) {
-    if (splitters_on) {
-      const int t = threadIdx.x - kTcSplitWarp0 * 32;
+  } else if ((warp >= kTcSplitWarp0 && warp < kTcSplitWarp0 + 4) || warp == 15) {
+    if (splitters_on && (warp != 15 || p.w_f32)) {
+      const int t = warp == 15 ? 128 + lane : threadIdx.x - kTcSplitWarp0 * 32;
       int s = 0;
       uint32_t ph = 0;
       bool ok = true;
@@ -307,17 +335,23 @@
           if (!ok) break;
           uint4* a = reinterpret_cast<uint4*>(stage_a(s));
           uint4* lo = reinterpret_cast<uint4*>(stage_alo(s));
-#pragma unroll
-          for (int i = 0; i < kTcAStageBytes / 16 / 128; ++i) {
-            const uint4 v = a[t + i * 128];
-            uint4 h, l;
-            h.x = rn_tf32_bits(v.x); h.y = rn_tf32_bits(v.y); h.z = rn_tf32_bits(v.z); h.w = rn_tf32_bits(v.w);
-            l.x = rn_tf32_bits(__float_as_uint(__uint_as_float(v.x) - __uint_as_float(h.x)));
-            l.y = rn_tf32_bits(__float_as_uint(__uint_as_float(v.y) - __uint_as_float(h.y)));
-            l.z = rn_tf32_bits(__float_as_uint(__uint_as_float(v.z) - __uint_as_float(h.z)));
-            l.w = rn_tf32_bits(__float_as_uint(__uint_as_float(v.w) - __uint_as_float(h.w)));
-            a[t + i * 128] = h;
-            lo[t + i * 128] = l;
+          if (p.w_f32) {
+            split_box_tf32<false>(a, lo, kTcAStageBytes / 16, t, 160);
+            split_box_tf32<true>(reinterpret_cast<uint4*>(w_hi_ptr(s, st)), reinterpret_cast<uint4*>(w_lo_ptr(s, st)),
+                                 (int)(w_chunk_bytes / 16), t, 160);
+          } else {
+#pragma unroll
+            for (int i = 0; i < kTcAStageBytes / 16 / 128; ++i) {
+              const uint4 v = a[t + i * 128];
+              uint4 h, l;
+              h.x = rn_tf32_bits(v.x); h.y = rn_tf32_bits(v.y); h.z = rn_tf32_bits(v.z); h.w = rn_tf32_bits(v.w);
+              l.x = rn_tf32_bits(__float_as_uint(__uint_as_float(v.x) - __uint_as_float(h.x)));
+              l.y = rn_tf32_bits(__float_as_uint(__uint_as_float(v.y) - __uint_as_float(h.y)));
+              l.z = rn_tf32_bits(__float_as_uint(__uint_as_float(v.z) - __uint_as_float(h.z)));
+              l.w = rn_tf32_bits(__float_as_uint(__uint_as_float(v.w) - __uint_as_float(h.w)));
+              a[t + i * 128] = h;
+              lo[t + i * 128] = l;
+            }
           }
           ptx::fence_proxy_async_smem();
           __syncwarp();
@@ -695,9 +729,10 @@
 struct TcWeights {
   float* hi = nullptr;
   float* lo = nullptr;
+  float* f32 = nullptr;
   bf16* bw = nullptr;
   int N = 0, Npad = 0, Kpad = 0;
-  CUtensorMap tm_hi, tm_lo;
+  CUtensorMap tm_hi, tm_lo, tm_f32;
 };
 
 inline void split_tf32_host(float v, float* hi, float* lo) {
@@ -771,6 +806,8 @@
       if (lay.total <= (uint32_t)kTcSmemBudget && (resident == 0 || stages >= 3 || p.num_steps <= 2 || res2)) {
         p.num_stages = stages;
         p.w_resident = resident;
+        static const bool no_w_f32 = getenv("YNB_TC_NO_W_F32") != nullptr;
+        p.w_f32 = (split && !resident && !p.presplit && L.w->f32 != nullptr && !no_w_f32) ? 1 : 0;
         L.smem = lay.total;
         return true;
       }
@@ -794,8 +831,8 @@
   const CUtensorMap& tmo = L.p.tma_store ? L.tmOut : L.tmA;
   KernelT kern = L.dec_classes == 80 ? kernels[2] : (L.dec_classes == 20 ? kernels[3] : kernels[L.p.pass != nullptr ? 1 : 0]);
   const CUtensorMap& tmalo = (L.p.presplit || L.p.a2_step > 0) ? L.tmAlo : L.tmA;
-  cudaError_t r = launch_pdl(kern, dim3(L.grid), dim3(kTcThreads), (size_t)L.smem, st, L.tmA, tmalo, L.w->tm_hi,
-                             L.w->tm_lo, tmo, L.p);
+  cudaError_t r = launch_pdl(kern, dim3(L.grid), dim3(kTcThreads), (size_t)L.smem, st, L.tmA, tmalo,
+                             L.p.w_f32 ? L.w->tm_f32 : L.w->tm_hi, L.w->tm_lo, tmo, L.p);
   YNB_COUNT_LAUNCH();
   return r;
 }
diff --git a/yolo_nano_b200/csrc/unit_tc.cuh b/yolo_nano_b200/csrc/unit_tc.cuh
--- a/yolo_nano_b200/csrc/unit_tc.cuh
+++ b/yolo_nano_b200/csrc/unit_tc.cuh
@@ -19,6 +19,7 @@
   int N, Npad;
   int mode;
   int w_resident, a_stages, raw_stages;
+  int w_f32;
   int prefetch_tiles;
   int pass_blocks;
   int tma_out;
@@ -97,7 +98,8 @@
   uint64_t* w_full = bars + 16;
   uint64_t* tmem_full = bars + 20;
   uint64_t* tmem_empty = bars + 22;
-  uint32_t* tmem_ptr = reinterpret_cast<uint32_t*>(bars + 24);
+  uint64_t* w_ready = bars + 24;
+  uint32_t* tmem_ptr = reinterpret_cast<uint32_t*>(bars + 28);
 
   const int warp = threadIdx.x >> 5, lane = threadIdx.x & 31;
   pdl_trigger();
@@ -105,7 +107,7 @@
   if (warp == kDpRawWarp && lane == 0) {
     ptx::prefetch_tmap(&tmIn);
     ptx::prefetch_tmap(&tmWhi);
-    if (split) ptx::prefetch_tmap(&tmWlo);
+    if (split && !p.w_f32) ptx::prefetch_tmap(&tmWlo);
     if (p.pass_blocks) ptx::prefetch_tmap(&tmPass);
     if (p.tma_out) ptx::prefetch_tmap(&tmOut);
     for (int s = 0; s < kDpMaxRawStages; ++s) {
@@ -116,6 +118,7 @@
       ptx::mbar_init(&a_ready[s], kBf16 ? kDpDwWarps : kDpDwWarps / 2);
       ptx::mbar_init(&a_empty[s], 1);
       ptx::mbar_init(&w_full[s], 1);
+      ptx::mbar_init(&w_ready[s], 1);
     }
     for (int a = 0; a < 2; ++a) {
       ptx::mbar_init(&tmem_full[a], 1);
@@ -190,7 +193,31 @@
       }
     }
   } else if (warp == kDpWWarp) {
-    if (!p.w_resident && ptx::elect_one()) {
+    if (!p.w_resident && p.w_f32) {
+      int s = 0;
+      uint32_t ph = 0;
+      bool ok = true;
+      for (int64_t tile = blockIdx.x; tile < p.num_tiles && ok; tile += gridDim.x) {
+        for (int kc = 0; kc < p.num_chunks; ++kc) {
+          ok = ptx::mbar_wait(&a_empty[s], ph ^ 1, p.err_flag, 2);
+          if (!ok) break;
+          uint8_t* wh = w_hi_ptr(s, kc);
+          if (ptx::elect_one()) {
+            ptx::mbar_arrive_expect_tx(&w_full[s], w_chunk_bytes);
+            ptx::tma_load_2d(wh, &tmWhi, &w_full[s], kc * CH, 0);
+          }
+          __syncwarp();
+          ok = ptx::mbar_wait(&w_full[s], ph, p.err_flag, 10);
+          if (!ok) break;
+          split_box_tf32<true>(reinterpret_cast<uint4*>(wh), reinterpret_cast<uint4*>(wh + w_chunk_bytes),
+                               (int)(w_chunk_bytes / 16), lane, 32);
+          ptx::fence_proxy_async_smem();
+          __syncwarp();
+          if (lane == 0) ptx::mbar_arrive(&w_ready[s]);
+          if (++s == p.a_stages) { s = 0; ph ^= 1; }
+        }
+      }
+    } else if (!p.w_resident && ptx::elect_one()) {
       int s = 0;
       uint32_t ph = 0;
       bool ok = true;
@@ -222,7 +249,7 @@
         const uint32_t c_tmem = d_tmem + (uint32_t)p.Npad;
         for (int kc = 0; kc < p.num_chunks; ++kc) {
           ok = ptx::mbar_wait(&a_ready[s], ph, p.err_flag, 5);
-          if (ok && !p.w_resident) ok = ptx::mbar_wait(&w_full[s], ph, p.err_flag, 6);
+          if (ok && !p.w_resident) ok = ptx::mbar_wait(p.w_f32 ? &w_ready[s] : &w_full[s], ph, p.err_flag, 6);
           if (!ok) break;
           ptx::tc_fence_after_sync();
           const uint32_t a_hi = ptx::smem_u32(a_stage(s));
@@ -604,6 +631,8 @@
       DpSmemLayout lay = dp_smem_layout(p.Npad, p.num_chunks, p.lgTW, 2, raw, resident != 0, split, chunk_ch);
       if (lay.total <= (uint32_t)kTcSmemBudget) {
         p.a_stages = 2; p.raw_stages = raw; p.w_resident = resident; L.smem = lay.total;
+        static const bool no_w_f32 = getenv("YNB_DP_NO_W_F32") != nullptr;
+        p.w_f32 = (split && !resident && w->f32 != nullptr && !no_w_f32) ? 1 : 0;
         found = true;
       }
     }
@@ -648,7 +677,7 @@
   }
   const int ki = (L.p.mode == YNB_GEMM_TC_BF16 ? 2 : 0) + (L.p.pass != nullptr ? 1 : 0);
   cudaError_t r = launch_pdl(kernels[ki], dim3(L.grid), dim3(kDpThreads), (size_t)L.smem, st,
-                             L.tmIn, L.w->tm_hi, L.w->tm_lo, L.p.pass_blocks ? L.tmPass : L.tmIn,
+                             L.tmIn, L.p.w_f32 ? L.w->tm_f32 : L.w->tm_hi, L.w->tm_lo, L.p.pass_blocks ? L.tmPass : L.tmIn,
                              L.p.tma_out ? L.tmOut : L.tmIn, L.p);
   YNB_COUNT_LAUNCH();
   return r;
diff --git a/yolo_nano_b200/csrc/ynb_api.cu b/yolo_nano_b200/csrc/ynb_api.cu
--- a/yolo_nano_b200/csrc/ynb_api.cu
+++ b/yolo_nano_b200/csrc/ynb_api.cu
@@ -234,8 +234,9 @@
   t.Npad = round_up(n, 16);
   if (t.hi) cudaFree(t.hi);
   if (t.lo) cudaFree(t.lo);
+  if (t.f32) cudaFree(t.f32);
   if (t.bw) cudaFree(t.bw);
-  t.hi = t.lo = nullptr; t.bw = nullptr;
+  t.hi = t.lo = t.f32 = nullptr; t.bw = nullptr;
   if (bf) {
     const int kin = ktot / taps, kin_pad = round_up(kin, 64);
     t.Kpad = taps * kin_pad;
@@ -262,6 +263,12 @@
   CUDA_TRY(e, cudaMemcpy(t.lo, lo.data(), lo.size() * 4, cudaMemcpyHostToDevice));
   if (!make_tmap_2d(&t.tm_hi, t.hi, t.Kpad, t.Npad, t.Kpad, t.Npad) ||
       !make_tmap_2d(&t.tm_lo, t.lo, t.Kpad, t.Npad, t.Kpad, t.Npad))
+    return fail(e, YNB_ERR_CUDA, "cuTensorMapEncodeTiled failed for weights of " + name);
+  std::vector<float> f32((size_t)t.Npad * t.Kpad, 0.f);
+  for (int r = 0; r < n; ++r) memcpy(&f32[(size_t)r * t.Kpad], w + (size_t)r * ktot, (size_t)ktot * 4);
+  CUDA_TRY(e, cudaMalloc(&t.f32, f32.size() * 4));
+  CUDA_TRY(e, cudaMemcpy(t.f32, f32.data(), f32.size() * 4, cudaMemcpyHostToDevice));
+  if (!make_tmap_2d(&t.tm_f32, t.f32, t.Kpad, t.Npad, t.Kpad, t.Npad))
     return fail(e, YNB_ERR_CUDA, "cuTensorMapEncodeTiled failed for weights of " + name);
   return YNB_OK;
 }
@@ -293,6 +300,7 @@
     if (cc.pc.b_dev) cudaFree(cc.pc.b_dev);
     if (cc.pc.tc.hi) cudaFree(cc.pc.tc.hi);
     if (cc.pc.tc.lo) cudaFree(cc.pc.tc.lo);
+    if (cc.pc.tc.f32) cudaFree(cc.pc.tc.f32);
     if (cc.pc.tc.bw) cudaFree(cc.pc.tc.bw);
   }
   e->cat[si].clear();
@@ -1093,6 +1101,7 @@
     if (pc.b_dev) cudaFree(pc.b_dev);
     if (pc.tc.hi) cudaFree(pc.tc.hi);
     if (pc.tc.lo) cudaFree(pc.tc.lo);
+    if (pc.tc.f32) cudaFree(pc.tc.f32);
     if (pc.tc.bw) cudaFree(pc.tc.bw);
   }
   for (int si = 0; si < 3; ++si)
@@ -1100,6 +1109,7 @@
       if (cc.pc.b_dev) cudaFree(cc.pc.b_dev);
       if (cc.pc.tc.hi) cudaFree(cc.pc.tc.hi);
       if (cc.pc.tc.lo) cudaFree(cc.pc.tc.lo);
+      if (cc.pc.tc.f32) cudaFree(cc.pc.tc.f32);
       if (cc.pc.tc.bw) cudaFree(cc.pc.tc.bw);
     }
   if (e->ws) cudaFree(e->ws);
@@ -1540,17 +1550,21 @@
   UNIT_TRY(cudaMemcpy(w.data(), w_dev, w.size() * 4, cudaMemcpyDeviceToHost));
   TcWeights t;
   t.N = cout; t.Npad = round_up(cout, 16); t.Kpad = round_up(cin, kTcBK);
-  std::vector<float> hi((size_t)t.Npad * t.Kpad, 0.f), lo((size_t)t.Npad * t.Kpad, 0.f);
+  std::vector<float> hi((size_t)t.Npad * t.Kpad, 0.f), lo((size_t)t.Npad * t.Kpad, 0.f), f32((size_t)t.Npad * t.Kpad, 0.f);
   for (int n = 0; n < cout; ++n)
-    for (int k = 0; k < cin; ++k)
+    for (int k = 0; k < cin; ++k) {
       split_tf32_host(w[(size_t)n * cin + k], &hi[(size_t)n * t.Kpad + k], &lo[(size_t)n * t.Kpad + k]);
+      f32[(size_t)n * t.Kpad + k] = w[(size_t)n * cin + k];
+    }
   int* d_err = nullptr;
   UNIT_TRY(cudaMalloc(&t.hi, hi.size() * 4));
   UNIT_TRY(cudaMalloc(&t.lo, lo.size() * 4));
+  UNIT_TRY(cudaMalloc(&t.f32, f32.size() * 4));
   UNIT_TRY(cudaMalloc(&d_err, 4));
   UNIT_TRY(cudaMemset(d_err, 0, 4));
   UNIT_TRY(cudaMemcpy(t.hi, hi.data(), hi.size() * 4, cudaMemcpyHostToDevice));
   UNIT_TRY(cudaMemcpy(t.lo, lo.data(), lo.size() * 4, cudaMemcpyHostToDevice));
+  UNIT_TRY(cudaMemcpy(t.f32, f32.data(), f32.size() * 4, cudaMemcpyHostToDevice));
   int rc = YNB_OK;
   TcGemmLaunch L;
   L.w = &t;
@@ -1576,6 +1590,7 @@
   }
   if (!make_tmap_2d(&t.tm_hi, t.hi, t.Kpad, t.Npad, t.Kpad, t.Npad) ||
       !make_tmap_2d(&t.tm_lo, t.lo, t.Kpad, t.Npad, t.Kpad, t.Npad) ||
+      !make_tmap_2d(&t.tm_f32, t.f32, t.Kpad, t.Npad, t.Kpad, t.Npad) ||
       (p.tma_store && !make_tmap_out(&L.tmOut, out + out_off, (uint64_t)round_up(cout, 4), (uint64_t)pixels,
                                      (uint64_t)out_ld)) ||
       !make_tmap_2d(&L.tmA, in + in_off, cin, pixels, in_ld, kTcBM) || !tc_plan_smem(L)) {
@@ -1593,15 +1608,15 @@
       cudaMemcpy(h.data(), d_trace, h.size() * 8, cudaMemcpyDeviceToHost);
       int n = 0;
       for (int i = 0; i < trace_cap; ++i) n += h[4 + 4 * i] != 0;
-      fprintf(stderr, "YNB_TC_TRACE stages=%d resident=%d nmain=%d acc_stages=%d steps=%d grid=%u events=%d\n",
-              p.num_stages, p.w_resident, p.nmain, p.acc_stages, p.num_steps, L.grid, n);
+      fprintf(stderr, "YNB_TC_TRACE stages=%d resident=%d w_f32=%d nmain=%d acc_stages=%d steps=%d grid=%u events=%d\n",
+              p.num_stages, p.w_resident, p.w_f32, p.nmain, p.acc_stages, p.num_steps, L.grid, n);
       for (int i = 0; i < trace_cap; ++i)
         if (h[4 + 4 * i] != 0)
           fprintf(stderr, "TRACE %lld %lld %lld %lld\n", h[1 + 4 * i], h[2 + 4 * i], h[3 + 4 * i], h[4 + 4 * i]);
     }
   }
   if (d_trace) cudaFree(d_trace);
-  cudaFree(t.hi); cudaFree(t.lo); cudaFree(d_err);
+  cudaFree(t.hi); cudaFree(t.lo); cudaFree(t.f32); cudaFree(d_err);
   return rc;
 }
 
@@ -1622,11 +1637,12 @@
   UNIT_TRY(cudaMemcpy(wv.data(), pw_w, wv.size() * 4, cudaMemcpyDeviceToHost));
   TcWeights t;
   t.N = cout; t.Npad = round_up(cout, 16); t.Kpad = round_up(channels, bfm ? 64 : kTcBK);
-  std::vector<float> hi((size_t)t.Npad * t.Kpad, 0.f), lo((size_t)t.Npad * t.Kpad, 0.f);
+  std::vector<float> hi((size_t)t.Npad * t.Kpad, 0.f), lo((size_t)t.Npad * t.Kpad, 0.f), f32((size_t)t.Npad * t.Kpad, 0.f);
   std::vector<bf16> bwv((size_t)t.Npad * t.Kpad, __float2bfloat16(0.0f));
   for (int n = 0; n < cout; ++n)
     for (int k = 0; k < channels; ++k) {
       split_tf32_host(wv[(size_t)n * channels + k], &hi[(size_t)n * t.Kpad + k], &lo[(size_t)n * t.Kpad + k]);
+      f32[(size_t)n * t.Kpad + k] = wv[(size_t)n * channels + k];
       bwv[(size_t)n * t.Kpad + k] = __float2bfloat16_rn(wv[(size_t)n * channels + k]);
     }
   int* d_err = nullptr;
@@ -1636,6 +1652,10 @@
   UNIT_TRY(cudaMemset(d_err, 0, 4));
   UNIT_TRY(cudaMemcpy(t.hi, hi.data(), hi.size() * 4, cudaMemcpyHostToDevice));
   UNIT_TRY(cudaMemcpy(t.lo, lo.data(), lo.size() * 4, cudaMemcpyHostToDevice));
+  if (!bfm) {
+    UNIT_TRY(cudaMalloc(&t.f32, f32.size() * 4));
+    UNIT_TRY(cudaMemcpy(t.f32, f32.data(), f32.size() * 4, cudaMemcpyHostToDevice));
+  }
   if (bfm) UNIT_TRY(cudaMemcpy(t.hi, bwv.data(), bwv.size() * 2, cudaMemcpyHostToDevice));
   int rc = YNB_OK;
   DwPwLaunch L;
@@ -1653,6 +1673,7 @@
   }
   if (!make_tmap_2d(&t.tm_hi, t.hi, t.Kpad, t.Npad, t.Kpad, t.Npad, bfm) ||
       !make_tmap_2d(&t.tm_lo, t.lo, t.Kpad, t.Npad, t.Kpad, t.Npad) ||
+      (t.f32 && !make_tmap_2d(&t.tm_f32, t.f32, t.Kpad, t.Npad, t.Kpad, t.Npad)) ||
       !plan_dwpw(L, in, in_ld, batch, h, w_, channels, channels, &t, mode)) {
     rc = fail(nullptr, YNB_ERR_CUDA, "ynb_dwpw_tc: tensor map / smem planning failed");
   } else {
@@ -1667,8 +1688,9 @@
       cudaMemcpy(h.data(), d_trace, h.size() * 8, cudaMemcpyDeviceToHost);
       long long t0 = 0;
       for (long long v : h) if (v && (!t0 || v < t0)) t0 = v;
-      fprintf(stderr, "YNB_DP_TRACE chunks=%d a_stages=%d raw_stages=%d resident=%d lgTW=%d tiles=%lld grid=%u\n", L.p.num_chunks,
-              L.p.a_stages, L.p.raw_stages, L.p.w_resident, L.p.lgTW, (long long)L.p.num_tiles, L.grid);
+      fprintf(stderr, "YNB_DP_TRACE chunks=%d a_stages=%d raw_stages=%d resident=%d w_f32=%d lgTW=%d tiles=%lld grid=%u\n",
+              L.p.num_chunks, L.p.a_stages, L.p.raw_stages, L.p.w_resident, L.p.w_f32, L.p.lgTW, (long long)L.p.num_tiles,
+              L.grid);
       const char* names[6] = {"raw_issued", "raw_landed", "A_written", "mma_issued", "acc_ready", "epi_done"};
       for (int lt = 0; lt < 16; ++lt)
         for (int role = 0; role < 6; ++role) {
@@ -1680,7 +1702,7 @@
     }
   }
   if (d_trace) cudaFree(d_trace);
-  cudaFree(t.hi); cudaFree(t.lo); cudaFree(d_err);
+  cudaFree(t.hi); cudaFree(t.lo); cudaFree(t.f32); cudaFree(d_err);
   return rc;
 }
 
```

New measurement: 29910, median of 6. -15.5%, worse.
